# seokjuchung/point-cloud-cnn-segmentation

Measured on AMD Instinct MI355X. Metric: M voxels/sec fwd+bwd, 128^3 grid batch=4 (points/s of the PointNet training step: forward + weighted CE + backward + Adam), higher is better.
Workload: dtype bf16; 1 GPU; PointNetSegmentation train step, 4 scenes x 128^3 points per GPU, C=2; global_batch=4, parallelism=dp1

## Files before the change

### include/pcs.h

```cpp
#ifndef PCS_H
#define PCS_H

#include <stdint.h>

#ifdef __cplusplus
extern "C" {
#endif

typedef struct ihipStream_t *pcs_stream_t;

enum { PCS_F32 = 0, PCS_BF16 = 1, PCS_FP8 = 2  };
enum { PCS_OK = 0, PCS_EINVAL = -1000 };
enum {
  PCS_FLAG_GENERIC = 1,
  PCS_FLAG_NO_GLDS = 2,
  PCS_FLAG_AW_FP8 = 4,
  PCS_FLAG_C_FP8 = 8,
  PCS_FLAG_POOL_SIGNED_W = 16,
};

enum {
  PCS_PRO_RAW = 0,
  PCS_PRO_BNRELU = 1,
  PCS_PRO_BWD = 2,
// ... 181 lines not shown
             int32_t C, int32_t dtype, int32_t splits_per_scene, float *workspace, float *G,
             float *colsum, pcs_stream_t stream);

int pcs_sign_rows(const void *W, int32_t dtype, int64_t rows, int64_t cols, const float *sign_of, void *out,
                  pcs_stream_t stream);

int pcs_quant_fp8_rows(const float *W, int64_t rows, int64_t cols, int64_t ldw, uint8_t *Wq, uint8_t *scale,
                       float *deq, pcs_stream_t stream);

int pcs_pool_rows_add(void *dz, int32_t dz_dtype, const void *Yp, int32_t yp_dtype, int64_t num_scenes,
                      int64_t scene_rows, int32_t Ncols, const int32_t *pool_idx, const float *pool_coef,
                      const float *pool_w, int64_t pool_ldw, int32_t pool_c, float *stats, int32_t chunks_per_scene,
                      pcs_stream_t stream);

int64_t pcs_gram_raw_workspace(int64_t M, int32_t C);
int pcs_gram_raw(const void *A, int64_t M, int32_t C, int32_t dtype, float *workspace, int64_t workspace_bytes,
                 float *G, pcs_stream_t stream);

int pcs_gram_wgrad(const float *G, const float *S, const float *W, int64_t ldw_in,
                   const float *beta, const float *gamma, const float *sp, const int32_t *am,
                   const void *Y, const float *s, const float *t, int64_t num_scenes,
                   int32_t Cout, int32_t Cin, int32_t dtype, const float *R, const float *alpha,
                   float *dW, int64_t ldw, pcs_stream_t stream);

int pcs_bn_fold(const float *W, int32_t Cout, int32_t Cin, int64_t ldw, const float *alpha,
                const float *beta, const float *gamma, int32_t dtype, void *WsT, float *c, void *H,
                pcs_stream_t stream);

int pcs_bn_stats_from_gram(const float *G, const float *S, int64_t count, const void *W, int32_t dtype,
                           int64_t ldw, int32_t C, int32_t Cin, int64_t num_scenes, float *stats,
                           pcs_stream_t stream);

int64_t pcs_bn_stats_from_gram_scenes_workspace(int32_t C, int32_t Cin);
int pcs_bn_stats_from_gram_scenes(const float *G, const float *Sb, int64_t scene_rows, const void *W, int32_t dtype,
                                  int64_t ldw, int32_t C, int32_t Cin, int64_t num_scenes, void *workspace,
                                  int64_t workspace_bytes, float *stats, pcs_stream_t stream);

int pcs_bn_s2_from_r(float *stats, int64_t num_chunks, int32_t C, const float *R, const void *W,
                     int32_t dtype, int64_t ldw, int32_t Cin, const float *mean, const float *rstd,
                     pcs_stream_t stream);

int pcs_confusion(const float *logits, int64_t ld, const int64_t *labels, int64_t M, int32_t C,
                  int64_t *cm, pcs_stream_t stream);

int pcs_argmax(const float *logits, int64_t ld, int64_t M, int32_t C, int64_t *out, pcs_stream_t stream);

int pcs_reduce_partials(const float *partial, int64_t nslabs, int64_t len, float scale,
                        float *out, int64_t out_stride_rows, int64_t row_len,
                        pcs_stream_t stream);

int pcs_reduce_partials_grouped(const float *partial, int64_t ngroups, int64_t nslabs, int64_t len,
                                float scale, float *out, pcs_stream_t stream);

int pcs_cast_weight(const float *W, int64_t rows, int64_t cols, int64_t ldw, int32_t dtype,
                    void *Wc, void *WcT, pcs_stream_t stream);

int pcs_adam(float *param, float *grad, float *exp_avg, float *exp_avg_sq, int64_t n,
             const float *grad_scale, float lr, float beta1, float beta2, float eps,
             float weight_decay, int64_t step, pcs_stream_t stream);

int pcs_pad_scatter(const float *points, const void *labels, int32_t label_bytes,
                    const int64_t *offsets, int64_t num_scenes, int64_t scene_rows,
                    float *points_out, int64_t *labels_out, uint8_t *mask_out, pcs_stream_t stream);

int pcs_round_weight(const float *W, int64_t n, int32_t dtype, float *out, pcs_stream_t stream);

typedef struct {
  int64_t num_scenes;
  int64_t scene_rows;
  int32_t chunks_per_scene;
  const void *y2;
  const float *s2, *t2;
  const void *W1;
  const float *sbias;
  void *Y1;
  const float *s1, *t1;
  const uint8_t *keep1;
  float keep_scale;
  const void *W2;
  void *Y2;
  float *stats;
} pcs_seg12_args;
int64_t pcs_fwd_seg12_geometry(pcs_seg12_args *args);
int pcs_fwd_seg12(const pcs_seg12_args *args, pcs_stream_t stream);

int pcs_bn_stats_gram_sbias(const float *G, const float *Sb, int64_t num_scenes, int64_t scene_rows,
                            const float *W, int64_t ldw, int32_t Cin, int32_t C, const float *sbias,
                            float *stats, pcs_stream_t stream);

int pcs_bnrelu_bf16(const float *Y, int64_t M, int32_t K, const float *s, const float *t, int32_t split,
                    void *out, pcs_stream_t stream);

int pcs_voxel_ids(const float *points, int64_t T, int32_t grid, float lo_x, float lo_y, float lo_z,
                  float hi_x, float hi_y, float hi_z, int64_t *ids, pcs_stream_t stream);
int64_t pcs_voxelize_workspace(int64_t T);
int pcs_voxelize(const float *points, const int64_t *labels, const int64_t *offsets, int64_t num_scenes,
                 int64_t T, int32_t grid, float lo_x, float lo_y, float lo_z, float hi_x, float hi_y,
                 float hi_z, int32_t num_classes, void *workspace, int64_t workspace_bytes,
                 int64_t *voxel_of_point, float *vox_points, int64_t *vox_labels, int64_t *vox_counts,
                 int64_t *vox_offsets, int64_t *num_voxels, pcs_stream_t stream);
int pcs_voxel_padded_index(const int64_t *voxel_of_point, int64_t T, const int64_t *vox_offsets,
                           int64_t num_scenes, int64_t scene_rows, int64_t *out, pcs_stream_t stream);
int pcs_gather_rows(const float *src, int64_t ld_src, const int64_t *idx, int64_t n, int32_t C,
                    float *dst, pcs_stream_t stream);

typedef struct {
// ... 124 lines not shown
```

### point-cloud-cnn-segmentation_amd/_lib.py

```python
from __future__ import annotations

import ctypes as ct
import os

import torch

_HERE = os.path.dirname(os.path.abspath(__file__))
LIB_PATH = os.path.join(_HERE, "csrc", "libpcs.so")

F32, BF16, FP8 = 0, 1, 2
PRO_RAW, PRO_BNRELU, PRO_BWD, PRO_CAT = 0, 1, 2, 4
EPI_FWD, EPI_DGRAD, EPI_RAW, EPI_BNRELU = 0, 1, 2, 3
HEAD_FWD, HEAD_CE, HEAD_BWD = 0, 1, 2

_vp = ct.c_void_p
_i64 = ct.c_int64
_i32 = ct.c_int32
_f = ct.c_float


class GemmArgs(ct.Structure):
    _fields_ = [
        ("num_scenes", _i64), ("scene_rows", _i64),
        ("K", _i32), ("Ncols", _i32), ("dtype", _i32), ("prologue", _i32), ("epilogue", _i32),
# ... 22 lines not shown
        ("num_scenes", _i64), ("scene_rows", _i64),
        ("Cout", _i32), ("Cin", _i32), ("dtype", _i32), ("splits_per_scene", _i32),
        ("dy_mode", _i32),
        ("dZ", _vp), ("Y", _vp), ("alpha", _vp), ("beta", _vp), ("gamma", _vp),
        ("reserved0", _vp), ("reserved1", _vp),
        ("x_mode", _i32),
        ("X", _vp), ("s", _vp), ("t", _vp), ("x_mask", _vp), ("x_keep_scale", _f),
        ("partial", _vp), ("dW", _vp), ("ldw", _i64), ("flags", _i32), ("reserved2", _vp),
    ]


class Seg12Args(ct.Structure):
    _fields_ = [
        ("num_scenes", _i64), ("scene_rows", _i64), ("chunks_per_scene", _i32),
        ("y2", _vp), ("s2", _vp), ("t2", _vp), ("W1", _vp), ("sbias", _vp), ("Y1", _vp),
        ("s1", _vp), ("t1", _vp), ("keep1", _vp), ("keep_scale", _f), ("W2", _vp), ("Y2", _vp),
        ("stats", _vp),
    ]


class Conv3dGeom(ct.Structure):
    _fields_ = [
        ("B", _i64), ("Di", _i32), ("Hi", _i32), ("Wi", _i32), ("Do", _i32), ("Ho", _i32), ("Wo", _i32),
        ("Cin", _i32), ("Cout", _i32), ("k", _i32), ("s", _i32), ("p", _i32), ("transposed", _i32),
    ]


class PoolBwdArgs(ct.Structure):
    _fields_ = [
        ("num_scenes", _i64), ("scene_rows", _i64),
        ("Cs", _i32), ("Cg", _i32), ("col_off", _i32),
        ("s1_alpha", _vp), ("s1_beta", _vp), ("s1_gamma", _vp),
        ("s1_scene_s1", _vp), ("s1_scene_sum", _vp),
        ("W_s1", _vp), ("ldw", _i64),
        ("g", _vp), ("ysel", _vp), ("g_mean", _vp), ("g_rstd", _vp), ("g_gamma", _vp),
        ("g_scene_sum", _vp),
        ("dW_s1_global", _vp), ("csum", _vp),
        ("alpha", _vp), ("beta_c", _vp), ("gamma_c", _vp),
        ("dgamma", _vp), ("dbeta", _vp), ("dbias", _vp), ("sp", _vp),
    ]


class HeadArgs(ct.Structure):
    _fields_ = [
        ("num_scenes", _i64), ("scene_rows", _i64),
        ("Cin", _i32), ("num_classes", _i32), ("dtype", _i32), ("mode", _i32),
        ("chunks_per_scene", _i32),
        ("Y", _vp), ("s", _vp), ("t", _vp), ("W", _vp), ("bias", _vp), ("logits", _vp),
        ("labels", _vp), ("class_weight", _vp), ("wsum", _vp),
        ("dlogits", _vp), ("dl_stride_row", _i64), ("dl_stride_col", _i64),
        ("dZ", _vp), ("mean", _vp), ("rstd", _vp), ("stats", _vp), ("wpartial", _vp),
        ("loss_partial", _vp),
    ]


SIGNATURES = [
    ("pcs_gemm_geometry", _i64, [ct.POINTER(GemmArgs)]),
    ("pcs_gemm", ct.c_int, [ct.POINTER(GemmArgs), _vp]),
    ("pcs_conv1_fwd", ct.c_int, [ct.POINTER(GemmArgs), _vp]),
    ("pcs_wgrad_workspace", _i64, [ct.POINTER(WgradArgs)]),
    ("pcs_wgrad", ct.c_int, [ct.POINTER(WgradArgs), _vp]),
    ("pcs_conv1_wgrad", ct.c_int, [ct.POINTER(WgradArgs), _vp]),
    ("pcs_bn_fwd_finalize", ct.c_int, [_vp, _i64, _i64, _i32, _i32, _i64, _vp, _vp, _vp, _vp,
                                       _vp, _f, _f, _i32, _vp, _vp, _vp, _vp, _vp, _vp]),
    ("pcs_bn_eval_coefs", ct.c_int, [_vp, _vp, _vp, _vp, _vp, _f, _i32, _vp, _vp, _vp]),
    ("pcs_bn_bwd_finalize", ct.c_int, [_vp, _i64, _i64, _i32, _i32, _vp, _vp, _vp, _vp, _vp,
                                       _vp, _vp, _vp, _vp, _vp, _vp, _vp]),
    ("pcs_pool_finalize", ct.c_int, [_vp, _i64, _i64, _i32, _i32, _vp, _vp, _vp, _vp, _vp, _vp]),
    ("pcs_scene_gemv", ct.c_int, [_vp, _i64, _i32, _vp, _i64, _i32, _vp, _i32, _vp, _vp, _vp]),
    ("pcs_pool_bwd", ct.c_int, [ct.POINTER(PoolBwdArgs), _vp]),
    ("pcs_head_geometry", _i64, [ct.POINTER(HeadArgs)]),
    ("pcs_head", ct.c_int, [ct.POINTER(HeadArgs), _vp]),
    ("pcs_ce_weight_sum", ct.c_int, [_vp, _i64, _vp, _i32, _vp, _vp, _vp]),
    ("pcs_dropout_bits", ct.c_int, [ct.c_uint64, ct.c_uint64, _i64, _i32, _f, _vp, _vp]),
    ("pcs_dropout_bits_bounded", ct.c_int, [ct.c_uint64, ct.c_uint64, _i64, _i32, _f, _vp, _i32, _vp]),
    ("pcs_dropout_bits_independent", ct.c_int, [ct.c_uint64, ct.c_uint64, _i64, _i32, _f, _vp, _vp]),
    ("pcs_reduce_partials", ct.c_int, [_vp, _i64, _i64, _f, _vp, _i64, _i64, _vp]),
    ("pcs_reduce_partials_grouped", ct.c_int, [_vp, _i64, _i64, _i64, _f, _vp, _vp]),
    ("pcs_cast_weight", ct.c_int, [_vp, _i64, _i64, _i64, _i32, _vp, _vp, _vp]),
    ("pcs_adam", ct.c_int, [_vp, _vp, _vp, _vp, _i64, _vp, _f, _f, _f, _f, _f, _i64, _vp]),
    ("pcs_colstats_geometry", _i64, [_i64, _i64, _i32, ct.POINTER(_i32)]),
    ("pcs_colstats", ct.c_int, [_vp, _i64, _i64, _i32, _i32, _i32, _i64, _vp, _vp, _vp]),
    ("pcs_bnrelu_bwd", ct.c_int, [_vp, _vp, _vp, _vp, _f, _vp, _vp, _vp, _vp, _i64, _i64, _i32, _i32,
                                  _i32, _i64, _vp, _vp]),
    ("pcs_abi_version", ct.c_int, []),
    ("pcs_conv3d", ct.c_int, [ct.POINTER(Conv3dGeom), _vp, _vp, _vp, _vp, _i32, _vp]),
    ("pcs_conv3d_wgrad_workspace", _i64, [ct.POINTER(Conv3dGeom)]),
    ("pcs_conv3d_wgrad", ct.c_int, [ct.POINTER(Conv3dGeom), _vp, _vp, _vp, _i64, _vp, _vp, _vp]),
    ("pcs_conv3d_weight_t", ct.c_int, [_vp, _i32, _i32, _i32, _vp, _vp]),
    ("pcs_sparse_conv", ct.c_int, [_vp, _i64, _i32, _vp, _i32, _vp, _i32, _vp, _vp, _i32, _i32, _vp]),
    ("pcs_sparse_conv_wgrad_workspace", _i64, [_i64, _i32, _i32, _i32]),
    ("pcs_sparse_conv_wgrad", ct.c_int, [_vp, _i64, _i32, _vp, _i32, _vp, _i32, _vp, _i64, _vp, _vp, _vp]),
    ("pcs_sparse_pairs_workspace", _i64, [_i64, _i32]),
    ("pcs_sparse_pairs_count", ct.c_int, [_vp, _i64, _i32, _vp, _vp, _vp]),
    ("pcs_sparse_pairs_build", ct.c_int, [_vp, _i64, _i32, _vp, _vp, _vp, _vp, _vp, _vp]),
    ("pcs_sparse_conv_pairs", ct.c_int, [_vp, _vp, _vp, _i32, _i64, _vp, _i32, _vp, _i32, _vp, _vp, _vp, _i32, _i32,
                                         _vp]),
    ("pcs_sparse_conv_wgrad_pairs_workspace", _i64, [_vp, _i32, _i64, _i32, _i32]),
    ("pcs_sparse_conv_wgrad_pairs", ct.c_int, [_vp, _vp, _vp, _i32, _i64, _vp, _i32, _vp, _i32, _vp, _i64, _vp, _vp,
                                               _vp]),
    ("pcs_sparse_conv_cat", ct.c_int, [_vp, _i64, _i32, _vp, _i32, _vp, _i32, _vp, _i32, _vp, _vp, _i32, _i32, _vp]),
    ("pcs_sparse_conv_cat_dgrad", ct.c_int, [_vp, _i64, _i32, _vp, _i32, _vp, _vp, _i32, _vp, _i32, _i32, _i32, _vp]),
    ("pcs_sparse_conv_cat_wgrad", ct.c_int, [_vp, _i64, _i32, _vp, _i32, _vp, _i32, _vp, _i32, _vp, _i64, _vp, _vp,
                                             _vp]),
    ("pcs_sparse_conv_cat_pairs", ct.c_int, [_vp, _vp, _vp, _i32, _i64, _vp, _i32, _vp, _i32, _vp, _i32, _vp, _vp, _vp,
                                             _i32, _i32, _vp]),
# ... 13 lines not shown
                                       _vp, _vp]),
    ("pcs_rows_interp", ct.c_int, [_vp, _i32, _vp, _vp, _i64, _i32, _i32, _vp, _i32, _vp]),
    ("pcs_rows_segsum", ct.c_int, [_vp, _i32, _vp, _vp, _vp, _vp, _i64, _i32, _vp, _i32, _vp]),
    ("pcs_sparse_bn_geometry", _i64, [_i64, _i32, ct.POINTER(_i32)]),
    ("pcs_sparse_bn_stats", ct.c_int, [_vp, _i32, _i64, _i32, _i32, _i64, _vp, _vp]),
    ("pcs_sparse_bn_apply", ct.c_int, [_vp, _i32, _vp, _vp, _vp, _i32, _i64, _i32, _vp, _i32, _vp]),
    ("pcs_sparse_bn_bwd_reduce", ct.c_int, [_vp, _vp, _i32, _vp, _i32, _vp, _vp, _i32, _i64, _i32, _i32, _i64, _vp,
                                            _vp, _vp]),
    ("pcs_sparse_bn_bwd_apply", ct.c_int, [_vp, _i32, _vp, _i32, _vp, _vp, _vp, _i64, _i32, _vp, _vp]),
    ("pcs_point_lift_mean", ct.c_int, [_vp, _i64, _i32, _vp, _vp, _vp, _vp, _vp, _i64, _i32, _vp, _i32, _vp]),
    ("pcs_point_lift_bwd_workspace", _i64, [_i64, _i32, _i32]),
    ("pcs_point_lift_mean_bwd", ct.c_int, [_vp, _i32, _vp, _i64, _i32, _vp, _vp, _vp, _vp, _vp, _i64, _i32, _vp, _i64,
                                           _vp, _vp, _vp]),
    ("pcs_point_head_project", ct.c_int, [_vp, _i32, _i64, _i32, _vp, _i32, _vp, _vp]),
    ("pcs_point_head_workspace", _i64, [_i64, _i64, _i32, _i32]),
    ("pcs_point_head_logits", ct.c_int, [_vp, _vp, _vp, _i64, _i32, _vp, _vp, _vp, _vp, _vp, _vp, _vp, _i64, _vp, _vp,
                                         _vp]),
    ("pcs_point_head_bwd", ct.c_int, [_vp, _vp, _vp, _vp, _vp, _i32, _i64, _i32, _vp, _i32, _vp, _vp, _vp, _i64, _vp,
                                      _vp]),
    ("pcs_gram_workspace", _i64, [_i64, _i64, _i32, _i32, ct.POINTER(_i32)]),
    ("pcs_gram", ct.c_int, [_vp, _vp, _vp, _i64, _i64, _i32, _i32, _i32, _vp, _vp, _vp, _vp]),
    ("pcs_pool_rows_add", ct.c_int, [_vp, _i32, _vp, _i32, _i64, _i64, _i32, _vp, _vp, _vp, _i64, _i32, _vp, _i32,
                                     _vp]),
    ("pcs_quant_fp8_rows", ct.c_int, [_vp, _i64, _i64, _i64, _vp, _vp, _vp, _vp]),
    ("pcs_gram_raw_workspace", _i64, [_i64, _i32]),
    ("pcs_gram_raw", ct.c_int, [_vp, _i64, _i32, _i32, _vp, _i64, _vp, _vp]),
    ("pcs_gram_wgrad", ct.c_int, [_vp, _vp, _vp, _i64, _vp, _vp, _vp, _vp, _vp, _vp, _vp, _i64, _i32, _i32,
                                  _i32, _vp, _vp, _vp, _i64, _vp]),
    ("pcs_bn_fold", ct.c_int, [_vp, _i32, _i32, _i64, _vp, _vp, _vp, _i32, _vp, _vp, _vp, _vp]),
    ("pcs_bn_s2_from_r", ct.c_int, [_vp, _i64, _i32, _vp, _vp, _i32, _i64, _i32, _vp, _vp, _vp]),
    ("pcs_bn_stats_from_gram", ct.c_int, [_vp, _vp, _i64, _vp, _i32, _i64, _i32, _i32, _i64, _vp, _vp]),
    ("pcs_bn_stats_from_gram_scenes_workspace", _i64, [_i32, _i32]),
    ("pcs_sign_rows", ct.c_int, [_vp, _i32, _i64, _i64, _vp, _vp, _vp]),
    ("pcs_dgrad_wgrad_folded_workspace", _i64, [ct.POINTER(WgradArgs)]),
    ("pcs_dgrad_wgrad_folded", ct.c_int, [ct.POINTER(WgradArgs), _vp, _vp, _vp, _vp, _vp, _vp]),
    ("pcs_bn_stats_from_gram_scenes", ct.c_int, [_vp, _vp, _i64, _vp, _i32, _i64, _i32, _i32, _i64, _vp, _i64, _vp,
                                                 _vp]),
    ("pcs_confusion", ct.c_int, [_vp, _i64, _vp, _i64, _i32, _vp, _vp]),
    ("pcs_argmax", ct.c_int, [_vp, _i64, _i64, _i32, _vp, _vp]),
    ("pcs_dgrad_wgrad_bn_workspace", _i64, [ct.POINTER(GemmArgs)]),
    ("pcs_dgrad_wgrad_bn", ct.c_int, [ct.POINTER(GemmArgs), _vp, _vp, _i64, _vp]),
    ("pcs_round_weight", ct.c_int, [_vp, _i64, _i32, _vp, _vp]),
    ("pcs_bnrelu_bf16", ct.c_int, [_vp, _i64, _i32, _vp, _vp, _i32, _vp, _vp]),
    ("pcs_fwd_seg12_geometry", _i64, [ct.POINTER(Seg12Args)]),
    ("pcs_fwd_seg12", ct.c_int, [ct.POINTER(Seg12Args), _vp]),
    ("pcs_bn_stats_gram_sbias", ct.c_int, [_vp, _vp, _i64, _i64, _vp, _i64, _i32, _i32, _vp, _vp, _vp]),
    ("pcs_voxel_ids", ct.c_int, [_vp, _i64, _i32, _f, _f, _f, _f, _f, _f, _vp, _vp]),
    ("pcs_voxelize_workspace", _i64, [_i64]),
    ("pcs_voxelize", ct.c_int, [_vp, _vp, _vp, _i64, _i64, _i32, _f, _f, _f, _f, _f, _f, _i32, _vp, _i64,
                                _vp, _vp, _vp, _vp, _vp, _vp, _vp]),
    ("pcs_gather_rows", ct.c_int, [_vp, _i64, _vp, _i64, _i32, _vp, _vp]),
    ("pcs_voxel_padded_index", ct.c_int, [_vp, _i64, _vp, _i64, _i64, _vp, _vp]),
    ("pcs_pad_scatter", ct.c_int, [_vp, _vp, _i32, _vp, _i64, _i64, _vp, _vp, _vp, _vp]),
    ("pcs_last_error", ct.c_char_p, []),
]

_lib = None


ABI_VERSION = 3


class PcsError(RuntimeError):
    pass


def load():
    global _lib
    if _lib is not None:
        return _lib
    path = os.environ.get("PCS_LIB", LIB_PATH)
    if not os.path.exists(path):
        raise ImportError(
            f"pcs_amd HIP library not built: {path} is missing. Build it with "
            "`python -c 'import __graft_entry__ as g; g.build()'` or "
            "`make -C point-cloud-cnn-segmentation_amd/csrc`.")
    lib = ct.CDLL(path)
    for name, res, args in SIGNATURES:
        fn = getattr(lib, name)
        fn.restype = res
        fn.argtypes = args
    got = lib.pcs_abi_version()
    if got != ABI_VERSION:
        raise ImportError(f"{path} has C ABI version {got}, this binding expects {ABI_VERSION}: rebuild it "
                          "(`make -C point-cloud-cnn-segmentation_amd/csrc`)")
    _lib = lib
    return lib


def call(name, *args):
    lib = load()
    rc = getattr(lib, name)(*args)
    if rc < 0:
        raise PcsError(f"{name} failed ({rc}): {lib.pcs_last_error().decode()}")
    return rc


def workspace(name, *args) -> int:
    lib = load()
    n = int(getattr(lib, name)(*args))
    if n < 0:
        raise PcsError(lib.pcs_last_error().decode())
    return n


def ptr(t):
# ... 6 lines not shown
```

### point-cloud-cnn-segmentation_amd/csrc/fused_bwd.hip

```cpp
#include "kernel_prims.h"

namespace {

constexpr int THREADS = 512;
constexpr int COUT = 512, CIN = 64, MS = 64;
constexpr int WT_ROWB = COUT * 2;
constexpr int DY_ROWB = COUT * 2 + 32;
constexpr int X_ROWB = CIN * 2 + 32;
constexpr int OFF_DY = CIN * WT_ROWB;
constexpr int OFF_X = OFF_DY + MS * DY_ROWB;
constexpr int OFF_OUT = OFF_X + MS * X_ROWB;
constexpr int OUT_ROWB = CIN * 2 + 8;
constexpr int OFF_COEF = OFF_OUT + MS * OUT_ROWB;
constexpr int OFF_H = OFF_COEF + 3 * CIN * 4;
constexpr int H_ROWB = CIN * 2;
constexpr int LDS_BYTES = OFF_H + CIN * H_ROWB;
static_assert(LDS_BYTES <= 160 * 1024, "LDS budget");
constexpr int SLAB_F = COUT * CIN + CIN * CIN + CIN;
constexpr int DY_CPR = COUT / 8, DY_RP = THREADS / DY_CPR, DY_NCH = MS / DY_RP;
constexpr int X_CPR = CIN / 8, X_RP = THREADS / X_CPR;
static_assert(X_RP == MS, "one x chunk per thread");

PCS_DEV int wt_off(int c, int slot) { return c * WT_ROWB + ((slot ^ (c & 15)) << 4); }

// ... 145 lines not shown
    lds_barrier();
    {
      const int r = tid >> 3, ch = tid & 7;
      if (m0 + r < hi)
        st16(dX + (sbase + m0 + r) * CIN + ch * 8,
             *reinterpret_cast<const u32x4 *>(lds + OFF_OUT + r * OUT_ROWB + ch * 16));
    }
    if (st + 1 < nsteps) {
      store_step(m0 + MS);
      __builtin_amdgcn_sched_barrier(0);
      load_step(m0 + 2 * MS);
    }
    lds_barrier();
  }

  float *out = a.partial + (int64_t)L * SLAB_F;
#pragma unroll
  for (int u = 0; u < 2; ++u)
    *reinterpret_cast<float4 *>(out + COUT * CIN + ((wid >> 1) * 16 + l16) * CIN + (2 * (wid & 1) + u) * 16 + 4 * g) =
        make_float4(accg[u][0], accg[u][1], accg[u][2], accg[u][3]);
  __syncthreads();
  float *red = reinterpret_cast<float *>(lds + OFF_DY);
#pragma unroll
  for (int e = 0; e < 8; ++e) red[xr * CIN + xc * 8 + e] = xsum[e];
  __syncthreads();
  if (tid < CIN) {
    float t = 0.f;
    for (int r = 0; r < X_RP; ++r) t += red[r * CIN + tid];
    out[COUT * CIN + CIN * CIN + tid] = t;
  }
#pragma unroll
  for (int i = 0; i < 4; ++i) {
    const int o = wid * 64 + i * 16 + l16;
#pragma unroll
    for (int j = 0; j < 4; ++j)
      *reinterpret_cast<float4 *>(out + o * CIN + j * 16 + 4 * g) =
          make_float4(accw[i][j][0], accw[i][j][1], accw[i][j][2], accw[i][j][3]);
  }
}

int64_t splits_of(const pcs_wgrad_args &a) {
  int64_t sps = (256 + a.num_scenes - 1) / a.num_scenes;
  const int64_t max_sps = (a.scene_rows + 4 * MS - 1) / (4 * MS);
  if (sps > max_sps) sps = max_sps;
  return sps < 1 ? 1 : sps;
}

}

namespace {

constexpr int RG_LEN = COUT * CIN + CIN * CIN;

__global__ __launch_bounds__(256) void folded_reduce_kernel(const float *__restrict__ part, int nslab, int sps,
                                                            int B, float *__restrict__ red, float *__restrict__ Sb) {
  const int i = blockIdx.x * 256 + threadIdx.x;
  if (i < RG_LEN) {
    float t = 0.f;
    for (int sl = 0; sl < nslab; ++sl) t += part[(int64_t)sl * SLAB_F + i];
    red[i] = t;
  } else if (i < RG_LEN + B * CIN) {
    const int b = (i - RG_LEN) / CIN, j = (i - RG_LEN) % CIN;
    float t = 0.f;
    for (int sl = b * sps; sl < (b + 1) * sps; ++sl) t += part[(int64_t)sl * SLAB_F + RG_LEN + j];
    Sb[b * CIN + j] = t;
  }
}

__global__ __launch_bounds__(CIN) void folded_assemble_kernel(const float *__restrict__ red, const float *__restrict__ Sb,
                                                              int B, const float *__restrict__ W, int64_t ldw,
                                                              const float *__restrict__ alpha,
                                                              const float *__restrict__ beta,
                                                              const float *__restrict__ gamma,
                                                              const float *__restrict__ sbias, float *__restrict__ dW,
                                                              int64_t ldo) {
  __shared__ float wk[CIN];
  const int k = blockIdx.x, j = threadIdx.x;
  wk[j] = W[(int64_t)k * ldw + j];
  __syncthreads();
  const float *G = red + COUT * CIN;
  float wg = 0.f;
  for (int i = 0; i < CIN; ++i) wg = fmaf(wk[i], G[i * CIN + j], wg);
  float S = 0.f, sbs = 0.f;
  for (int b = 0; b < B; ++b) {
    const float sbj = Sb[b * CIN + j];
    S += sbj;
    sbs = fmaf(sbias[(int64_t)b * COUT + k], sbj, sbs);
  }
  dW[(int64_t)k * ldo + j] = fmaf(alpha[k], red[k * CIN + j], fmaf(beta[k], S, gamma[k] * (wg + sbs)));
}

__global__ __launch_bounds__(CIN) void folded_cvec_kernel(const float *__restrict__ W, int64_t ldw,
                                                          const float *__restrict__ beta, const float *__restrict__ gamma,
                                                          const float *__restrict__ sbias, float *__restrict__ cvec) {
  const int b = blockIdx.x, j = threadIdx.x;
  float t = 0.f;
  for (int k = 0; k < COUT; ++k)
    t = fmaf(fmaf(gamma[k], sbias[(int64_t)b * COUT + k], beta[k]), W[(int64_t)k * ldw + j], t);
  cvec[b * CIN + j] = t;
}

bool folded_shapes_ok(const pcs_wgrad_args &a) {
  return a.dtype == PCS_BF16 && a.Cout == COUT && a.Cin == CIN && a.dy_mode == PCS_PRO_RAW &&
         a.x_mode == PCS_PRO_BNRELU && !a.x_mask && !(a.flags & PCS_FLAG_GENERIC);
}

}

extern "C" int64_t pcs_dgrad_wgrad_folded_workspace(pcs_wgrad_args *a) {
  if (!a || a->num_scenes <= 0 || a->scene_rows <= 0)
    return pcs_set_einval("pcs_dgrad_wgrad_folded_workspace", "bad geometry");
  if (!folded_shapes_ok(*a))
    return pcs_set_einval("pcs_dgrad_wgrad_folded_workspace",
                          "bf16, Cout=512, Cin=64, dy_mode PRO_RAW, x_mode PRO_BNRELU, no x_mask only");
  a->splits_per_scene = (int32_t)splits_of(*a);
  const int64_t nb = a->num_scenes * a->splits_per_scene;
  return (nb * SLAB_F + RG_LEN + a->num_scenes * CIN + a->num_scenes * CIN) * 4;
}

extern "C" int pcs_dgrad_wgrad_folded(const pcs_wgrad_args *ap, const void *WaT, const void *H, const float *W,
                                      const float *scene_bias, void *dX, pcs_stream_t stream) {
  if (!ap || !WaT || !H || !W || !scene_bias || !dX) return pcs_set_einval("pcs_dgrad_wgrad_folded", "null argument");
  pcs_wgrad_args a = *ap;
  if (pcs_dgrad_wgrad_folded_workspace(&a) < 0) return PCS_EINVAL;
  if (!a.dZ || !a.alpha || !a.beta || !a.gamma || !a.X || !a.s || !a.t || !a.partial || !a.dW || a.ldw < CIN)
    return pcs_set_einval("pcs_dgrad_wgrad_folded", "missing operand (dZ, alpha, beta, gamma, X, s, t, partial, dW, "
                                                    "ldw >= 64)");
  if (a.scene_rows * a.num_scenes >= (int64_t)1 << 31) return pcs_set_einval("pcs_dgrad_wgrad_folded", "M must be < 2^31");
  const int64_t rps = ((a.scene_rows + a.splits_per_scene - 1) / a.splits_per_scene + MS - 1) / MS * MS;
  const int B = (int)a.num_scenes;
  const int nb = B * a.splits_per_scene;
  float *red = a.partial + (int64_t)nb * SLAB_F;
  float *Sb = red + RG_LEN;
  float *cvec = Sb + B * CIN;
  hipStream_t s = reinterpret_cast<hipStream_t>(stream);
  hipLaunchKernelGGL(folded_cvec_kernel, dim3(B), dim3(CIN), 0, s, W, a.ldw, a.beta, a.gamma, scene_bias, cvec);
  hipLaunchKernelGGL(dgrad_wgrad_s1_kernel, dim3(nb), dim3(THREADS), 0, s, a, static_cast<const bf16_t *>(WaT),
                     static_cast<bf16_t *>(dX), rps, static_cast<const bf16_t *>(H), cvec);
  hipLaunchKernelGGL(folded_reduce_kernel, dim3((RG_LEN + B * CIN + 255) / 256), dim3(256), 0, s, a.partial, nb,
                     a.splits_per_scene, B, red, Sb);
  hipLaunchKernelGGL(folded_assemble_kernel, dim3(COUT), dim3(CIN), 0, s, red, Sb, B, W, a.ldw, a.alpha, a.beta,
                     a.gamma, scene_bias, a.dW, a.ldw);
  PCS_CHECK_LAUNCH();
  return 0;
}

namespace {

template <int COUT, int CIN, int CB, int MS, bool MASK, bool ADD> struct FB {
  static constexpr int NBLK = CIN / CB;
  static constexpr int WT_ROWB = COUT * 2;
  static constexpr int WSW = COUT >= 128 ? 15 : 7;
  static constexpr int DY_ROWB = COUT * 2 + 32;
  static constexpr int X_ROWB = CB * 2 + 32;
  static constexpr int YP_ROWB = CB * 2 + 16;
  static constexpr int OUT_ROWB = CB * 2 + 8;
  static constexpr int OFF_DY = CB * WT_ROWB;
  static constexpr int OFF_X = OFF_DY + MS * DY_ROWB;
  static constexpr int OFF_YP = OFF_X + MS * X_ROWB;
  static constexpr int OFF_AD = OFF_YP + MS * YP_ROWB;
  static constexpr int OFF_MK = OFF_AD + (ADD ? MS * YP_ROWB : 0);
  static constexpr int OFF_OUT = OFF_MK + (MASK ? MS * CB / 8 : 0);
  static constexpr int OFF_COEF = OFF_OUT + MS * OUT_ROWB;
  static constexpr int BYTES = OFF_COEF + (3 * COUT + 2 * CB) * 4;
  static constexpr bool FITS = BYTES <= 160 * 1024;
  static_assert(CIN % CB == 0, "column blocks");
  static constexpr int NCB = CB / 16, NMB = MS / 16, NOB = COUT / 16;
  static constexpr int TPW_D = NMB * NCB / 8, TPW_W = NOB * NCB / 8;
  static constexpr int OBW = TPW_W > NCB ? TPW_W / NCB : 1;
  static_assert(TPW_D >= 1 && TPW_W >= 1 && NCB % TPW_D == 0, "dgrad wave tiling");
  static_assert(TPW_W % NCB == 0 || NCB % TPW_W == 0, "wgrad wave tiling");
  static constexpr int CBW = TPW_W / OBW;
  static constexpr int NCH_D = MS * COUT / 8 / THREADS, NCH_P = MS * CB / 8 / THREADS;
  static_assert(NCH_D >= 1 && NCH_P >= 1 && MS % 32 == 0, "staging");
};

template <int COUT, int CIN, int CB, int MS, bool MASK, bool ADD>
__global__ __launch_bounds__(THREADS) __attribute__((amdgpu_waves_per_eu(COUT == 64 ? 4 : 1, 8))) void dgrad_wgrad_bn_kernel(pcs_gemm_args a, float *__restrict__ wpart,
                                                                 int64_t rows_per_split) {
  typedef FB<COUT, CIN, CB, MS, MASK, ADD> F;
  static_assert(F::FITS, "LDS budget");
  __shared__ __attribute__((aligned(16))) char lds[F::BYTES];
  const int tid = threadIdx.x, lane = tid & 63, wid = tid >> 6;
  const int L = xcd_remap(blockIdx.x, gridDim.x);
  const int chunk = L / F::NBLK, n0 = (L % F::NBLK) * CB;
  const int sps = a.chunks_per_scene;
  const int scene = chunk / sps, sis = chunk % sps;
  const int64_t N = a.scene_rows;
  const int64_t lo = (int64_t)sis * rows_per_split;
  const int64_t hi = pcs_min64(lo + rows_per_split, N);
  const int64_t sbase = (int64_t)scene * N;
  const bf16_t *__restrict__ dZ = reinterpret_cast<const bf16_t *>(a.A);
// ... 200 lines not shown
}

template <int COUT, int CIN, int CB, int MS>
int launch_bn(const pcs_gemm_args &a, float *wpart, int64_t rps, hipStream_t s) {
  const int nb = (int)(a.num_scenes * a.chunks_per_scene) * (CIN / CB);
  if (a.c_mask && a.addend) return pcs_set_einval("pcs_dgrad_wgrad_bn", "mask and addend together");
  if (a.c_mask)
    hipLaunchKernelGGL((dgrad_wgrad_bn_kernel<COUT, CIN, CB, MS, true, false>), dim3(nb), dim3(THREADS), 0, s, a, wpart, rps);
  else if (a.addend) {
    if constexpr (FB<COUT, CIN, CB, MS, false, true>::FITS)
      hipLaunchKernelGGL((dgrad_wgrad_bn_kernel<COUT, CIN, CB, MS, false, true>), dim3(nb), dim3(THREADS), 0, s, a, wpart,
                         rps);
    else
      return pcs_set_einval("pcs_dgrad_wgrad_bn", "no addend variant at this shape (LDS)");
  } else
    hipLaunchKernelGGL((dgrad_wgrad_bn_kernel<COUT, CIN, CB, MS, false, false>), dim3(nb), dim3(THREADS), 0, s, a,
                       wpart, rps);
  PCS_CHECK_LAUNCH();
  return 0;
}

struct BnShape { int cout, cin, cb, ms; };
constexpr BnShape kBnShapes[] = {{64, 64, 64, 64}, {128, 64, 64, 64}};

const BnShape *bn_shape(int K, int Ncols) {
  for (const BnShape &b : kBnShapes)
    if (b.cout == K && b.cin == Ncols) return &b;
  return nullptr;
}

}

extern "C" int64_t pcs_dgrad_wgrad_bn_workspace(pcs_gemm_args *a) {
  if (!a || a->num_scenes <= 0 || a->scene_rows <= 0) return pcs_set_einval("pcs_dgrad_wgrad_bn_workspace", "bad geometry");
  if (pcs_seg4_applicable(*a)) {
    pcs_seg4_geometry(a);
    return (int64_t)a->num_scenes * a->chunks_per_scene * a->K * a->Ncols * 4;
  }
  const BnShape *sh = bn_shape(a->K, a->Ncols);
  if (a->dtype != PCS_BF16 || !sh || (a->flags & PCS_FLAG_GENERIC))
    return pcs_set_einval("pcs_dgrad_wgrad_bn_workspace",
                          "bf16 with (Cout, Cin) = K x Ncols in {64x64, 128x64} only");
  const int nblk = sh->cin / sh->cb;
  const int64_t target = sh->cout == 64 ? 512 : 256;
  int64_t sps = (target + a->num_scenes * nblk - 1) / (a->num_scenes * nblk);
  const int64_t max_sps = (a->scene_rows + 4 * sh->ms - 1) / (4 * sh->ms);
  if (sps > max_sps) sps = max_sps;
  if (sps < 1) sps = 1;
  const int64_t rps = ((a->scene_rows + sps - 1) / sps + sh->ms - 1) / sh->ms * sh->ms;
  a->chunks_per_scene = (int32_t)((a->scene_rows + rps - 1) / rps);
  return (int64_t)a->num_scenes * a->chunks_per_scene * a->K * a->Ncols * 4;
}

extern "C" int pcs_dgrad_wgrad_bn(const pcs_gemm_args *ap, float *partial, float *dW, int64_t ldw,
                                  pcs_stream_t stream) {
  if (!ap || !partial || !dW) return pcs_set_einval("pcs_dgrad_wgrad_bn", "null argument");
  pcs_gemm_args a = *ap;
  if (pcs_dgrad_wgrad_bn_workspace(&a) < 0) return PCS_EINVAL;
  if (a.chunks_per_scene != ap->chunks_per_scene)
    return pcs_set_einval("pcs_dgrad_wgrad_bn", "chunks_per_scene must come from pcs_dgrad_wgrad_bn_workspace");
  if (!a.A || !a.A2 || !a.pa || !a.pb || !a.pc || !a.W || !a.C || !a.Yp || !a.es || !a.et || !a.emean ||
      !a.erstd || !a.stats)
    return pcs_set_einval("pcs_dgrad_wgrad_bn", "missing operand (A, A2, pa, pb, pc, W, C, Yp, es, et, emean, "
                                                "erstd, stats)");
  if (a.scene_rows * a.num_scenes >= (int64_t)1 << 31) return pcs_set_einval("pcs_dgrad_wgrad_bn", "M must be < 2^31");
  if (pcs_seg4_applicable(a)) {
    const int rc = pcs_seg4_launch(a, partial, reinterpret_cast<hipStream_t>(stream));
    if (rc) return rc;
    const int nslab = (int)(a.num_scenes * a.chunks_per_scene);
    return pcs_reduce_partials(partial, nslab, (int64_t)a.K * a.Ncols, 1.0f, dW, ldw ? ldw : a.Ncols, a.Ncols, stream);
  }
  const BnShape *sh = bn_shape(a.K, a.Ncols);
  const int64_t rps = ((a.scene_rows + a.chunks_per_scene - 1) / a.chunks_per_scene + sh->ms - 1) / sh->ms * sh->ms;
  hipStream_t s = reinterpret_cast<hipStream_t>(stream);
  int rc;
  if (a.K == 64) rc = launch_bn<64, 64, 64, 64>(a, partial, rps, s);
  else rc = launch_bn<128, 64, 64, 64>(a, partial, rps, s);
  if (rc) return rc;
  const int nslab = (int)(a.num_scenes * a.chunks_per_scene);
  return pcs_reduce_partials(partial, nslab, (int64_t)a.K * a.Ncols, 1.0f, dW, ldw ? ldw : a.Ncols, a.Ncols, stream);
}
```

### point-cloud-cnn-segmentation_amd/csrc/gemm_glds.hip

```cpp
#include "kernel_prims.h"

#include <type_traits>

namespace {

constexpr int THREADS = 512;
constexpr int BM = 256, BN = 256, BK = 64;
constexpr int REG = 128 * BK * 2;
constexpr int KBUF = 4 * REG;
constexpr int STAGE_BYTES = 2 * KBUF;
constexpr int OFF_RUN = STAGE_BYTES;
constexpr int OFF_BIAS = OFF_RUN + 2 * 256 * 8;
constexpr int OFF_RUNN = OFF_BIAS + 256 * 4;
constexpr int OFF_UNI = OFF_RUNN + 16;
constexpr int OFF_POOL = OFF_UNI;
constexpr int OFF_SGN = OFF_UNI + 2 * 256 * 16;
constexpr int OFF_CUR = OFF_SGN + 256 * 4;
constexpr int OFF_MASK = OFF_UNI;
constexpr int LDS_BYTES = OFF_UNI + 2 * 256 * 8 * 4;
static_assert(LDS_BYTES <= 160 * 1024, "LDS budget");

enum { MODE_FWD = 0, MODE_DGRAD = 1 };


// ... 540 lines not shown
      } else {
        *reinterpret_cast<float2 *>(a.stats + o * 2) = make_float2(h0.x + h1.x, 0.f);
      }
    }
    if (do_pool) {
      float4 p = runp[tid];
      const float4 q = runp[BN + tid];
      const int pi = __float_as_int(p.y), qi = __float_as_int(q.y);
      const int pj = __float_as_int(p.w), qj = __float_as_int(q.w);
      if (pool_max_wins(q.x, qi, p.x, pi)) { p.x = q.x; p.y = q.y; }
      if (pool_min_wins(q.z, qj, p.z, pj)) { p.z = q.z; p.w = q.w; }
      *reinterpret_cast<float4 *>(a.pool + o * 4) = p;
    }
  }
}

}

bool pcs_gemm_glds_applicable(const pcs_gemm_args &a) {
  if (a.dtype != PCS_BF16 || (a.flags & (PCS_FLAG_GENERIC | PCS_FLAG_NO_GLDS))) return false;
  const bool fp8 = a.flags & PCS_FLAG_AW_FP8;
  if (fp8 && !a.w_scale) return false;
  if (a.prologue != PCS_PRO_RAW || a.K % (fp8 ? 256 : 2 * BK) != 0 || a.Ncols % BN != 0) return false;
  if (a.epilogue == PCS_EPI_FWD)
    return a.C == nullptr && a.scene_bias == nullptr && (!a.pool || a.es) &&
           (!(a.flags & PCS_FLAG_POOL_SIGNED_W) || (a.pool && !a.stats));
  if (a.epilogue == PCS_EPI_DGRAD)
    return a.Yp == a.A && a.K == a.Ncols && !a.es && !a.et && !a.erstd && !a.addend && !a.c_mask &&
           !a.pool_w;
  return false;
}

int pcs_gemm_glds_launch(const pcs_gemm_args &g, int tps, int tpc, hipStream_t s) {
  const int ncb = g.Ncols / BN;
  const int nb = ncb * (int)(g.num_scenes * g.chunks_per_scene);
  const bool fp8 = g.flags & PCS_FLAG_AW_FP8;
#define PCS_GL(M, F) hipLaunchKernelGGL((gemm_glds_kernel<M, F>), dim3(nb), dim3(THREADS), 0, s, g, tps, tpc, ncb)
  if (g.epilogue == PCS_EPI_FWD) {
    if (fp8) PCS_GL(MODE_FWD, true); else PCS_GL(MODE_FWD, false);
  } else {
    if (fp8) PCS_GL(MODE_DGRAD, true); else PCS_GL(MODE_DGRAD, false);
  }
#undef PCS_GL
  PCS_CHECK_LAUNCH();
  return 0;
}

namespace {

constexpr int PR_MAXC = 1024;
constexpr int PR_PARTS = 16;

template <typename T, typename TY>
__global__ __launch_bounds__(256) void pool_rows_add_kernel(T *__restrict__ dz, const TY *__restrict__ Yp, int64_t N,
                                                            int Ncols, const int32_t *__restrict__ idx,
                                                            const float *__restrict__ coef, const float *__restrict__ Wp,
                                                            int64_t ldw, int P, float *__restrict__ stats, int cps) {
  __shared__ unsigned long long keys[PR_MAXC];
  const int b = blockIdx.y, part = blockIdx.z, parts = gridDim.z, tid = threadIdx.x;
  const int n = blockIdx.x * 256 + tid;
  int Pp = 1;
  while (Pp < P) Pp <<= 1;
  for (int c = tid; c < Pp; c += 256)
    keys[c] = c < P ? ((unsigned long long)(uint32_t)idx[(int64_t)b * P + c] << 11) | (unsigned)c : ~0ull;
  __syncthreads();
  for (int k = 2; k <= Pp; k <<= 1) {
    for (int j = k >> 1; j > 0; j >>= 1) {
      for (int i = tid; i < Pp; i += 256) {
        const int ixj = i ^ j;
        if (ixj > i) {
          const unsigned long long x = keys[i], y = keys[ixj];
          if ((x > y) == ((i & k) == 0)) { keys[i] = y; keys[ixj] = x; }
        }
      }
      __syncthreads();
    }
  }
  auto srow_at = [&](int q) { return (int)(keys[q] >> 11); };
  auto sch_at = [&](int q) { return (int)(keys[q] & 2047u); };
  auto cut = [&](int j) {
    int p = (int)((int64_t)j * P / parts);
    while (p > 0 && p < P && srow_at(p) == srow_at(p - 1)) ++p;
    return p;
  };
  const int p0 = cut(part), p1 = cut(part + 1);
  if (n >= Ncols || p0 >= p1) return;
  float ds1 = 0.f, v = 0.f;
  constexpr int U = 8;
  for (int p = p0; p < p1; p += U) {
    float cf[U], wv[U];
#pragma unroll
    for (int u = 0; u < U; ++u) {
      cf[u] = 0.f;
      wv[u] = 0.f;
      if (p + u < p1) {
        const int c = sch_at(p + u);
        cf[u] = coef[(int64_t)b * P + c];
        wv[u] = Wp[(int64_t)c * ldw + n];
      }
    }
#pragma unroll
    for (int u = 0; u < U; ++u) {
      const int q = p + u;
      if (q >= p1) break;
      v = fmaf(cf[u], wv[u], v);
      if (q + 1 == p1 || srow_at(q + 1) != srow_at(q)) {
        const int64_t m = (int64_t)srow_at(q);
        const int64_t o = m * Ncols + n;
        if (m >= (int64_t)b * N && m < (int64_t)(b + 1) * N && load_elem(Yp, o) > 0.f) {
          const float d = load_elem(dz, o) + v;
          if constexpr (sizeof(T) == 2) dz[o] = (T)(pack2bf(d, 0.f) & 0xffffu);
          else dz[o] = d;
          ds1 += v;
        }
        v = 0.f;
      }
    }
  }
  if (stats) stats[(((int64_t)b * cps + part) * Ncols + n) * 2] += ds1;
}

}

extern "C" int pcs_pool_rows_add(void *dz, int32_t dz_dtype, const void *Yp, int32_t yp_dtype, int64_t num_scenes,
                                 int64_t scene_rows, int32_t Ncols, const int32_t *pool_idx, const float *pool_coef,
                                 const float *pool_w, int64_t pool_ldw, int32_t pool_c, float *stats,
                                 int32_t chunks_per_scene, pcs_stream_t stream) {
  if (!dz || !Yp || !pool_idx || !pool_coef || !pool_w || num_scenes <= 0 || scene_rows <= 0 || Ncols <= 0 ||
      pool_c <= 0 || pool_c > PR_MAXC || pool_ldw < Ncols || (stats && chunks_per_scene <= 0))
    return pcs_set_einval("pcs_pool_rows_add", "bad arguments (0 < pool_c <= 1024, pool_ldw >= Ncols)");
  hipStream_t s = reinterpret_cast<hipStream_t>(stream);
  const int parts = stats ? (chunks_per_scene < PR_PARTS ? chunks_per_scene : PR_PARTS) : PR_PARTS;
  const dim3 grid((Ncols + 255) / 256, (unsigned)num_scenes, (unsigned)parts);
#define PCS_PRA(T, TY)                                                                                          \
  hipLaunchKernelGGL((pool_rows_add_kernel<T, TY>), grid, dim3(256), 0, s, static_cast<T *>(dz),                 \
                     static_cast<const TY *>(Yp), scene_rows, (int)Ncols, pool_idx, pool_coef, pool_w, pool_ldw, \
                     (int)pool_c, stats, (int)chunks_per_scene)
  if (dz_dtype == PCS_BF16 && yp_dtype == PCS_BF16) PCS_PRA(bf16_t, bf16_t);
  else if (dz_dtype == PCS_BF16 && yp_dtype == PCS_FP8) PCS_PRA(bf16_t, fp8_t);
  else if (dz_dtype == PCS_F32 && yp_dtype == PCS_F32) PCS_PRA(float, float);
  else return pcs_set_einval("pcs_pool_rows_add", "dtypes: (bf16, bf16), (bf16, fp8) or (f32, f32)");
#undef PCS_PRA
  PCS_CHECK_LAUNCH();
  return 0;
}

namespace {
__global__ __launch_bounds__(256) void quant_fp8_rows_kernel(const float *__restrict__ W, int64_t cols, int64_t ldw,
                                                             fp8_t *__restrict__ Wq, uint8_t *__restrict__ scale,
                                                             float *__restrict__ deq) {
  __shared__ float red[4];
  const int64_t r = blockIdx.x;
  const float *w = W + r * ldw;
  float mx = 0.f;
  for (int64_t k = threadIdx.x; k < cols; k += 256) mx = fmaxf(mx, fabsf(w[k]));
  for (int o = 32; o > 0; o >>= 1) mx = fmaxf(mx, __shfl_xor(mx, o));
  if ((threadIdx.x & 63) == 0) red[threadIdx.x >> 6] = mx;
  __syncthreads();
  mx = fmaxf(fmaxf(red[0], red[1]), fmaxf(red[2], red[3]));
  int e = 0;
  if (mx > 0.f) {
    e = (int)ceilf(log2f(mx / 448.f));
    e = e < -126 ? -126 : (e > 127 ? 127 : e);
  }
  if (threadIdx.x == 0) scale[r] = (uint8_t)(127 + e);
  const float inv = ldexpf(1.f, -e);
  for (int64_t k = threadIdx.x * 4; k < cols; k += 1024) {
    float v[4];
#pragma unroll
    for (int q = 0; q < 4; ++q) v[q] = k + q < cols ? w[k + q] * inv : 0.f;
    const uint32_t b = pack4fp8(v[0], v[1], v[2], v[3]);
    for (int q = 0; q < 4 && k + q < cols; ++q) {
      Wq[r * cols + k + q] = (fp8_t)(b >> (8 * q));
      if (deq) deq[r * cols + k + q] = ldexpf(fp82f((b >> (8 * q)) & 255u), e);
    }
  }
}
}

extern "C" int pcs_quant_fp8_rows(const float *W, int64_t rows, int64_t cols, int64_t ldw, uint8_t *Wq, uint8_t *scale,
                                  float *deq, pcs_stream_t stream) {
  if (!W || !Wq || !scale || rows <= 0 || cols <= 0 || ldw < cols) return pcs_set_einval("pcs_quant_fp8_rows", "bad arguments");
  hipLaunchKernelGGL(quant_fp8_rows_kernel, dim3((unsigned)rows), dim3(256), 0, reinterpret_cast<hipStream_t>(stream), W,
                     cols, ldw, Wq, scale, deq);
  PCS_CHECK_LAUNCH();
  return 0;
}

// ... 33 lines not shown
```

### point-cloud-cnn-segmentation_amd/csrc/gemm_tn.hip

```cpp
#include "kernel_prims.h"

namespace {

constexpr int THREADS = 256;

template <typename T> struct TnCfg;
template <> struct TnCfg<bf16_t> {
  static constexpr int MS = 64;
  static constexpr int PADB = 32;
  static PCS_DEV int prow(int r) { return ::prow(r); }
};
template <> struct TnCfg<float> {
  static constexpr int MS = 16;
  static constexpr int PADB = 64;
  static PCS_DEV int prow(int r) { return r; }
};

template <typename T, int COLS, int MODE>
struct Operand {
  static constexpr int EPC = Elem<T>::EPC;
  static constexpr int MS = TnCfg<T>::MS;
  static constexpr int CPR = COLS / EPC;
  static constexpr int RP = THREADS / CPR;
  static constexpr int NCH = MS / RP;
// ... 232 lines not shown

template <typename T, int TM, int TN>
int dispatch_modes(const pcs_wgrad_args &a, int64_t rps, hipStream_t s) {
  if (a.dy_mode == PCS_PRO_BWD) {
    if (a.x_mode == PCS_PRO_BNRELU) return launch<T, TM, TN, PCS_PRO_BWD, PCS_PRO_BNRELU>(a, rps, s);
    if (a.x_mode == PCS_PRO_RAW) return launch<T, TM, TN, PCS_PRO_BWD, PCS_PRO_RAW>(a, rps, s);
  } else if (a.dy_mode == PCS_PRO_RAW) {
    if (a.x_mode == PCS_PRO_BNRELU) return launch<T, TM, TN, PCS_PRO_RAW, PCS_PRO_BNRELU>(a, rps, s);
  } else if (a.dy_mode == PCS_PRO_BNRELU && a.x_mode == PCS_PRO_BNRELU && !a.x_mask) {
    return launch<T, TM, TN, PCS_PRO_BNRELU, PCS_PRO_BNRELU>(a, rps, s);
  }
  return pcs_set_einval("pcs_wgrad", "unsupported dy_mode/x_mode");
}

template <typename T>
int dispatch_tiles(const pcs_wgrad_args &a, int64_t rps, hipStream_t s) {
  const bool m128 = a.Cout % 128 == 0, n128 = a.Cin % 128 == 0;
  if (m128 && n128) return dispatch_modes<T, 128, 128>(a, rps, s);
  if (m128) return dispatch_modes<T, 128, 64>(a, rps, s);
  if (n128) return dispatch_modes<T, 64, 128>(a, rps, s);
  return dispatch_modes<T, 64, 64>(a, rps, s);
}

int64_t rows_per_split_of(const pcs_wgrad_args &a, int ms) {
  const int64_t rps = (a.scene_rows + a.splits_per_scene - 1) / a.splits_per_scene;
  return (rps + ms - 1) / ms * ms;
}

bool reserved_set(const pcs_wgrad_args &a) { return a.reserved0 || a.reserved1 || a.reserved2; }

}

extern "C" int64_t pcs_wgrad_workspace(pcs_wgrad_args *a) {
  if (!a || a->num_scenes <= 0 || a->scene_rows <= 0 || a->Cout <= 0 || a->Cin <= 0)
    return pcs_set_einval("pcs_wgrad_workspace", "bad geometry");
  if (reserved_set(*a)) return pcs_set_einval("pcs_wgrad_workspace", "reserved0..2 must be NULL (removed in ABI 3)");
  const int ms = a->dtype == PCS_BF16 ? TnCfg<bf16_t>::MS : TnCfg<float>::MS;
  if (a->splits_per_scene <= 0 && pcs_wgrad_c5_class(*a)) a->splits_per_scene = pcs_wgrad_c5_splits(*a);
  if (a->splits_per_scene <= 0 && pcs_wgrad_big_applicable(*a)) a->splits_per_scene = pcs_wgrad_big_splits(*a);
  if (a->splits_per_scene <= 0) {
    const int tm = a->Cout % 128 == 0 ? 128 : 64, tn = a->Cin % 128 == 0 ? 128 : 64;
    const int64_t ntiles = a->Cin >= 64 ? (int64_t)(a->Cout / tm) * (a->Cin / tn) : 1;
    const int64_t target = 1024;
    int64_t sps = (target + a->num_scenes * ntiles - 1) / (a->num_scenes * ntiles);
    const int64_t max_sps = (a->scene_rows + 4 * ms - 1) / (4 * ms);
    if (sps > max_sps) sps = max_sps;
    if (sps < 1) sps = 1;
    a->splits_per_scene = (int32_t)sps;
  }
  const int64_t nslabs = (int64_t)a->num_scenes * a->splits_per_scene;
  return nslabs * a->Cout * a->Cin * 4;
}

extern "C" int pcs_wgrad(const pcs_wgrad_args *ap, pcs_stream_t stream) {
  if (!ap) return pcs_set_einval("pcs_wgrad", "null args");
  pcs_wgrad_args a = *ap;
  if (reserved_set(a)) return pcs_set_einval("pcs_wgrad", "reserved0..2 must be NULL (removed in ABI 3)");
  if (a.dy_mode != PCS_PRO_RAW && a.dy_mode != PCS_PRO_BNRELU && a.dy_mode != PCS_PRO_BWD)
    return pcs_set_einval("pcs_wgrad", "unknown dy_mode (PCS_PRO_RAW, PCS_PRO_BNRELU or PCS_PRO_BWD)");
  if (a.Cout % 64 || a.Cin % 64) return pcs_set_einval("pcs_wgrad", "Cout/Cin must be multiples of 64");
  if (!a.X || !a.partial || !a.dW) return pcs_set_einval("pcs_wgrad", "missing operand");
  if (a.dy_mode == PCS_PRO_RAW ? !a.dZ : (!a.Y || !a.beta || !a.gamma))
    return pcs_set_einval("pcs_wgrad", "dy operands missing (RAW: dZ; otherwise: Y, beta, gamma)");
  if (a.dy_mode == PCS_PRO_BWD && (!a.dZ || !a.alpha)) return pcs_set_einval("pcs_wgrad", "PRO_BWD needs dZ, alpha");
  if (a.x_mode == PCS_PRO_BNRELU && (!a.s || !a.t)) return pcs_set_einval("pcs_wgrad", "x BNRELU needs s, t");
  if (pcs_wgrad_workspace(&a) < 0) return PCS_EINVAL;
  const int ms = a.dtype == PCS_BF16 ? TnCfg<bf16_t>::MS : TnCfg<float>::MS;
  const int64_t rps = rows_per_split_of(a, ms);
  hipStream_t s = reinterpret_cast<hipStream_t>(stream);
  int rc;
  if (pcs_wgrad_c5_applicable(a)) rc = pcs_wgrad_c5_launch(a, rps, s);
  else if (pcs_wgrad_big_applicable(a)) rc = pcs_wgrad_big_launch(a, s);
  else if (a.dtype == PCS_BF16) rc = dispatch_tiles<bf16_t>(a, rps, s);
  else if (a.dtype == PCS_F32) rc = dispatch_tiles<float>(a, rps, s);
  else return pcs_set_einval("pcs_wgrad", "bad dtype");
  if (rc) return rc;
  const int64_t nslabs = a.num_scenes * a.splits_per_scene;
  return pcs_reduce_partials(a.partial, nslabs, (int64_t)a.Cout * a.Cin, 1.0f, a.dW,
                             a.ldw ? a.ldw : a.Cin, a.Cin, stream);
}

namespace {

pcs_wgrad_args gram_args(const void *Y, const float *s, const float *t, int64_t num_scenes,
                         int64_t scene_rows, int32_t C, int32_t dtype, int32_t sps) {
  pcs_wgrad_args a = {};
  a.num_scenes = num_scenes; a.scene_rows = scene_rows; a.Cout = C; a.Cin = C; a.dtype = dtype;
  a.splits_per_scene = sps; a.dy_mode = PCS_PRO_BNRELU; a.x_mode = PCS_PRO_BNRELU;
  a.Y = Y; a.X = Y; a.s = s; a.t = t; a.x_keep_scale = 1.f;
  return a;
}

__global__ __launch_bounds__(256) void gram_mirror_kernel(float *__restrict__ G, int C) {
  __shared__ float tile[64][65];
  const int nt = C / 64;
  int t = blockIdx.x, tj = 0;
  while (t >= nt - 1 - tj) { t -= nt - 1 - tj; ++tj; }
  const int tk = tj + 1 + t;
  const int tx = threadIdx.x & 63, ty = threadIdx.x >> 6;
  for (int r = ty; r < 64; r += 4) tile[r][tx] = G[(int64_t)(tj * 64 + r) * C + tk * 64 + tx];
  __syncthreads();
  for (int r = ty; r < 64; r += 4) G[(int64_t)(tk * 64 + r) * C + tj * 64 + tx] = tile[tx][r];
}

}

extern "C" int64_t pcs_gram_workspace(int64_t num_scenes, int64_t scene_rows, int32_t C, int32_t dtype,
                                      int32_t *splits_per_scene) {
  if (num_scenes <= 0 || scene_rows <= 0 || C <= 0 || C % 64 || !splits_per_scene)
    return pcs_set_einval("pcs_gram_workspace", "bad geometry");
  pcs_wgrad_args a = gram_args(nullptr, nullptr, nullptr, num_scenes, scene_rows, C, dtype, 0);
  if (pcs_gram128_class(a)) a.splits_per_scene = pcs_gram128_splits(a);
  const int64_t g = pcs_wgrad_workspace(&a);
  if (g < 0) return g;
  *splits_per_scene = a.splits_per_scene;
  return g + num_scenes * a.splits_per_scene * (int64_t)C * 4;
}

extern "C" int pcs_gram(const void *Y, const float *s, const float *t, int64_t num_scenes, int64_t scene_rows,
                        int32_t C, int32_t dtype, int32_t splits_per_scene, float *workspace, float *G,
                        float *colsum, pcs_stream_t stream) {
  if (!Y || !s != !t || !workspace || !G || !colsum || splits_per_scene <= 0)
    return pcs_set_einval("pcs_gram", "missing operand or splits (s and t both set, or both NULL)");
  if (C % 64) return pcs_set_einval("pcs_gram", "C must be a multiple of 64");
  pcs_wgrad_args a = gram_args(Y, s, t, num_scenes, scene_rows, C, dtype, splits_per_scene);
  a.partial = workspace;
  hipStream_t st = reinterpret_cast<hipStream_t>(stream);
  int rc;
  if (!s && !pcs_wgrad_big_applicable(a))
    return pcs_set_einval("pcs_gram", "s = t = NULL needs the 256x256 kernel (bf16, C % 256 == 0)");
  if (pcs_gram128_applicable(a)) {
    rc = pcs_gram128_launch(a, st);
  } else if (pcs_wgrad_big_applicable(a)) {
// ... 21 lines not shown
```

### point-cloud-cnn-segmentation_amd/csrc/gram.hip

```cpp
#include "common.h"

namespace {

constexpr int TILE = 64, KC = 32, THREADS = 256;

template <typename T, int TL>
__global__ __launch_bounds__(THREADS) void gram_wgrad_kernel(
    const float *__restrict__ G, const float *__restrict__ S, const float *__restrict__ W, int64_t ldwin,
    const float *__restrict__ beta, const float *__restrict__ gamma, const float *__restrict__ sp,
    const int *__restrict__ am, const T *__restrict__ Y, const float *__restrict__ s,
    const float *__restrict__ t, int B, int Cout, int Cin, const float *__restrict__ R,
    const float *__restrict__ alpha, float *__restrict__ dW, int64_t ldw) {
  constexpr int RR = TL / 16, NE = TL * KC / THREADS;
  __shared__ float Ws[TL][KC + 1];
  __shared__ float Gs[KC][TL];
  const int tid = threadIdx.x, tx = tid & 15, ty = tid >> 4;
  const int c0 = blockIdx.y * TL, k0 = blockIdx.x * TL;
  float acc[RR][RR] = {};
  float pw[NE], pg[NE];
  auto load = [&](int j0) {
#pragma unroll
    for (int u = 0; u < NE; ++u) {
      const int e = tid + THREADS * u;
      pw[u] = W[(int64_t)(c0 + e / KC) * ldwin + j0 + e % KC];
// ... 151 lines not shown
      for (int p = 0; p < R; ++p)
#pragma unroll
        for (int q = 0; q < R; ++q) acc[p][q] = fmaf(xa[p], ya[q], acc[p][q]);
    }
    __syncthreads();
  }
#pragma unroll
  for (int p = 0; p < R; ++p)
#pragma unroll
    for (int q = 0; q < R; ++q) {
      const int64_t o = (int64_t)(i0 + ty * R + p) * Cin + j0 + tx * R + q;
      if constexpr (sizeof(T) == 2) H[o] = (T)(pack2bf(acc[p][q], 0.f) & 0xffffu);
      else H[o] = acc[p][q];
    }
}

template <typename T>
__global__ __launch_bounds__(256) void bn_stats_gram_kernel(const float *__restrict__ G, const float *__restrict__ S,
                                                            double n, const T *__restrict__ W, int64_t ldw, int C,
                                                            int Cin, int B, float *__restrict__ stats) {
  __shared__ double w[1024];
  __shared__ double sh[256][2];
  const int c = blockIdx.x, tid = threadIdx.x;
  double dm = 0.0;
  for (int k = tid; k < Cin; k += 256) {
    w[k] = (double)load_elem(W, (int64_t)c * ldw + k);
    dm += w[k] * (double)S[k];
  }
  __syncthreads();
  double q = 0.0;
  for (int j = tid; j < Cin; j += 256) {
    const double sj = (double)S[j] / n;
    double row = 0.0;
    for (int k = 0; k < Cin; ++k) row += ((double)G[(int64_t)j * Cin + k] - sj * (double)S[k]) * w[k];
    q += w[j] * row;
  }
  sh[tid][0] = dm; sh[tid][1] = q;
  __syncthreads();
  for (int st = 128; st > 0; st >>= 1) {
    if (tid < st) { sh[tid][0] += sh[tid + st][0]; sh[tid][1] += sh[tid + st][1]; }
    __syncthreads();
  }
  if (tid < B) {
    const double mean = sh[0][0] / n, m2 = sh[0][1] < 0.0 ? 0.0 : sh[0][1];
    *reinterpret_cast<float2 *>(stats + ((int64_t)tid * C + c) * 2) = make_float2((float)mean, (float)(m2 / B));
  }
}

constexpr int QK_SPLIT = 4;

template <typename T>
__global__ __launch_bounds__(256) void gram_quad_kernel(const float *__restrict__ G, const T *__restrict__ W,
                                                        int64_t ldw, int Cin, double *__restrict__ part) {
  __shared__ double gs[16][64];
  __shared__ double wt[16][65];
  __shared__ double red[16][64];
  const int C = gridDim.x * 64, c0 = blockIdx.x * 64, j0 = blockIdx.y * 64;
  const int tid = threadIdx.x, tx = tid & 15, ty = tid >> 4;
  double acc[4][4];
#pragma unroll
  for (int p = 0; p < 4; ++p)
#pragma unroll
    for (int q = 0; q < 4; ++q) acc[p][q] = 0.0;
  const int kz0 = (int)((int64_t)Cin / 16 * blockIdx.z / QK_SPLIT) * 16;
  const int kz1 = (int)((int64_t)Cin / 16 * (blockIdx.z + 1) / QK_SPLIT) * 16;
  for (int k0 = kz0; k0 < kz1; k0 += 16) {
#pragma unroll
    for (int e = tid; e < 1024; e += 256) {
      gs[e >> 6][e & 63] = (double)G[(int64_t)(k0 + (e >> 6)) * Cin + j0 + (e & 63)];
      wt[e & 15][e >> 4] = (double)load_elem(W, (int64_t)(c0 + (e >> 4)) * ldw + k0 + (e & 15));
    }
    __syncthreads();
#pragma unroll 4
    for (int kk = 0; kk < 16; ++kk) {
      double a[4], b[4];
#pragma unroll
      for (int p = 0; p < 4; ++p) { a[p] = gs[kk][ty * 4 + p]; b[p] = wt[kk][tx * 4 + p]; }
#pragma unroll
      for (int p = 0; p < 4; ++p)
#pragma unroll
        for (int q = 0; q < 4; ++q) acc[p][q] = fma(a[p], b[q], acc[p][q]);
    }
    __syncthreads();
  }
#pragma unroll
  for (int q = 0; q < 4; ++q) {
    const int64_t wr = (int64_t)(c0 + tx * 4 + q) * ldw + j0 + ty * 4;
    double s = 0.0;
#pragma unroll
    for (int p = 0; p < 4; ++p) s = fma((double)load_elem(W, wr + p), acc[p][q], s);
    red[ty][tx * 4 + q] = s;
  }
  __syncthreads();
  if (tid < 64) {
    double s = 0.0;
    for (int r = 0; r < 16; ++r) s += red[r][tid];
    part[((int64_t)blockIdx.z * gridDim.y + blockIdx.y) * C + c0 + tid] = s;
  }
}

template <typename T>
__global__ __launch_bounds__(256) void bn_stats_scenes_kernel(const double *__restrict__ part, int njt,
                                                              const float *__restrict__ Sb, double nb,
                                                              const T *__restrict__ W, int64_t ldw, int C, int Cin,
                                                              int B, float *__restrict__ stats) {
  __shared__ double sh[256];
  __shared__ double d[64];
  const int c = blockIdx.x, tid = threadIdx.x;
  for (int b = 0; b < B; ++b) {
    double x = 0.0;
    for (int k = tid; k < Cin; k += 256)
      x = fma((double)load_elem(W, (int64_t)c * ldw + k), (double)Sb[(int64_t)b * Cin + k], x);
    sh[tid] = x;
    __syncthreads();
    for (int st = 128; st > 0; st >>= 1) {
      if (tid < st) sh[tid] += sh[tid + st];
      __syncthreads();
    }
    if (tid == 0) d[b] = sh[0];
    __syncthreads();
  }
  double qp = 0.0;
  for (int jt = tid; jt < njt; jt += 256) qp += part[(int64_t)jt * C + c];
  sh[tid] = qp;
  __syncthreads();
  for (int st = 128; st > 0; st >>= 1) {
    if (tid < st) sh[tid] += sh[tid + st];
    __syncthreads();
  }
  if (tid == 0) {
// ... 167 lines not shown
```

### point-cloud-cnn-segmentation_amd/csrc/small.hip

```cpp
#include "common.h"

namespace {

constexpr int THREADS = 256;
constexpr int C1_BM = 128;

template <int KD>
PCS_DEV void load_xrow(const float *X, int64_t row, float (&x)[KD]) {
  if constexpr (KD == 4) {
    const float4 v = *reinterpret_cast<const float4 *>(X + row * 4);
    x[0] = v.x; x[1] = v.y; x[2] = v.z; x[3] = v.w;
  } else {
#pragma unroll
    for (int k = 0; k < KD; ++k) x[k] = X[row * KD + k];
  }
}

template <typename T, int KD>
__global__ __launch_bounds__(THREADS) void conv1_fwd_kernel(pcs_gemm_args a, int tiles_per_scene,
                                                            int tiles_per_chunk) {
  constexpr int EPC = Elem<T>::EPC;
  constexpr int COLS = 64;
  constexpr int CPR = COLS / EPC;
  constexpr int RPP = THREADS / CPR;
// ... 73 lines not shown
  const int tid = threadIdx.x;
  const int sps = a.splits_per_scene;
  const int scene = blockIdx.x / sps, sis = blockIdx.x % sps;
  const int64_t N = a.scene_rows;
  const int cc = tid % CPR, r0 = tid / CPR, c0 = cc * EPC;
  const T *dZ = reinterpret_cast<const T *>(a.dZ);
  const T *Y = reinterpret_cast<const T *>(a.Y);
  const float *X = reinterpret_cast<const float *>(a.X);
  float ca[EPC], cb[EPC], cg[EPC];
  load_vec<EPC>(a.alpha, c0, ca); load_vec<EPC>(a.beta, c0, cb); load_vec<EPC>(a.gamma, c0, cg);
  float acc[EPC][KD];
#pragma unroll
  for (int e = 0; e < EPC; ++e)
#pragma unroll
    for (int k = 0; k < KD; ++k) acc[e][k] = 0.f;
  const int64_t lo = (int64_t)sis * rows_per_split, hi = pcs_min64(lo + rows_per_split, N);
  constexpr int U = 4;
  for (int64_t r = lo + r0; r < hi; r += U * RPP) {
    u32x4 dzr[U], yr[U];
    float x[U][KD];
#pragma unroll
    for (int u = 0; u < U; ++u) {
      const int64_t grow = scene * N + pcs_min64(r + u * RPP, hi - 1);
      dzr[u] = *reinterpret_cast<const u32x4 *>(dZ + grow * COLS + c0);
      yr[u] = *reinterpret_cast<const u32x4 *>(Y + grow * COLS + c0);
      load_xrow<KD>(X, grow, x[u]);
    }
#pragma unroll
    for (int u = 0; u < U; ++u) {
      if (r + u * RPP >= hi) break;
      float dz[EPC], y[EPC];
      unpack_chunk(dzr[u], dz);
      unpack_chunk(yr[u], y);
#pragma unroll
      for (int e = 0; e < EPC; ++e) {
        const float dy = fmaf(ca[e], dz[e], fmaf(cg[e], y[e], cb[e]));
#pragma unroll
        for (int k = 0; k < KD; ++k) acc[e][k] = fmaf(dy, x[u][k], acc[e][k]);
      }
    }
  }
#pragma unroll
  for (int e = 0; e < EPC; ++e)
#pragma unroll
    for (int k = 0; k < KD; ++k) red[r0][(c0 + e) * KD + k] = acc[e][k];
  __syncthreads();
  for (int i = tid; i < COLS * KD; i += THREADS) {
    float s = 0.f;
    for (int j = 0; j < RPP; ++j) s += red[j][i];
    a.partial[(int64_t)blockIdx.x * COLS * KD + i] = s;
  }
}

__global__ __launch_bounds__(THREADS) void bn_fwd_finalize_kernel(
    const float *stats, int64_t B, int64_t N, int C, int cps, int64_t rpc, const float *gamma,
    const float *beta, const float *moff, float *rmean, float *rvar, float momentum, float eps, int update,
    float *mean_o, float *rstd_o, float *scale_o, float *shift_o, float *scene_sum) {
  __shared__ double sh[THREADS][3];
  const int c = blockIdx.x, tid = threadIdx.x;
  double gn = 0, gmean = 0, gm2 = 0;
  for (int64_t b = 0; b < B; ++b) {
    double n = 0, mu = 0, q = 0;
    for (int j = tid; j < cps; j += THREADS) {
      const double nb = (double)pcs_min64(rpc, N - (int64_t)j * rpc);
      const float2 p = *reinterpret_cast<const float2 *>(stats + ((b * cps + j) * C + c) * 2);
      const double nn = n + nb, d = (double)p.x - mu;
      mu += d * nb / nn;
      q += (double)p.y + d * d * n * nb / nn;
      n = nn;
    }
    sh[tid][0] = n; sh[tid][1] = mu; sh[tid][2] = q;
    __syncthreads();
    for (int s = THREADS / 2; s > 0; s >>= 1) {
      if (tid < s) {
        const double na = sh[tid][0], nb = sh[tid + s][0];
        if (nb > 0) {
          const double nn = na + nb, d = sh[tid + s][1] - sh[tid][1];
          sh[tid][1] += d * nb / nn;
          sh[tid][2] += sh[tid + s][2] + d * d * na * nb / nn;
          sh[tid][0] = nn;
        }
      }
      __syncthreads();
    }
    if (tid == 0) {
      const double nb = sh[0][0], mb = sh[0][1], qb = sh[0][2];
      if (scene_sum) scene_sum[b * C + c] = (float)(nb * mb);
      const double nn = gn + nb, d = mb - gmean;
      gmean += d * nb / nn;
      gm2 += qb + d * d * gn * nb / nn;
      gn = nn;
    }
    __syncthreads();
  }
  if (tid == 0) {
    const double var = gm2 / gn;
    const double rstd = 1.0 / sqrt(var + (double)eps);
    const double sc = (double)gamma[c] * rstd;
    mean_o[c] = (float)gmean;
    rstd_o[c] = (float)rstd;
    scale_o[c] = (float)sc;
    shift_o[c] = (float)((double)beta[c] - gmean * sc);
    if (update) {
      const double unb = gn > 1 ? gm2 / (gn - 1) : gm2;
      const double tm = gmean + (moff ? (double)moff[c] : 0.0);
      rmean[c] = (float)((1.0 - momentum) * (double)rmean[c] + momentum * tm);
      rvar[c] = (float)((1.0 - momentum) * (double)rvar[c] + momentum * unb);
    }
  }
}

__global__ void bn_eval_kernel(const float *gamma, const float *beta, const float *rm,
                               const float *rv, const float *moff, float eps, int C, float *scale,
                               float *shift) {
  const int c = blockIdx.x * blockDim.x + threadIdx.x;
  if (c >= C) return;
  const double sc = (double)gamma[c] / sqrt((double)rv[c] + (double)eps);
  scale[c] = (float)sc;
  shift[c] = (float)((double)beta[c] - ((double)rm[c] - (moff ? (double)moff[c] : 0.0)) * sc);
}

__global__ __launch_bounds__(THREADS) void bn_bwd_finalize_kernel(
    const float *stats, int64_t B, int64_t N, int C, int cps, const float *mean, const float *rstd,
    const float *gamma, const float *scene_sum, float *alpha, float *beta_c, float *gamma_c,
    float *dgamma, float *dbeta, float *dbias, float *scene_s1) {
  __shared__ double sh[THREADS][2];
  const int c = blockIdx.x, tid = threadIdx.x;
  double S1 = 0, S2 = 0, Sy = 0;
  for (int64_t b = 0; b < B; ++b) {
    double s1 = 0, s2 = 0;
    for (int j = tid; j < cps; j += THREADS) {
      const float2 p = *reinterpret_cast<const float2 *>(stats + ((b * cps + j) * C + c) * 2);
      s1 += p.x; s2 += p.y;
    }
    sh[tid][0] = s1; sh[tid][1] = s2;
    __syncthreads();
    for (int s = THREADS / 2; s > 0; s >>= 1) {
      if (tid < s) { sh[tid][0] += sh[tid + s][0]; sh[tid][1] += sh[tid + s][1]; }
      __syncthreads();
    }
    if (tid == 0) {
      if (scene_s1) scene_s1[b * C + c] = (float)sh[0][0];
      S1 += sh[0][0]; S2 += sh[0][1];
      if (scene_sum) Sy += scene_sum[b * C + c];
    }
    __syncthreads();
  }
  if (tid == 0) {
    const double M = (double)(B * N);
    const double r = rstd[c], g = gamma[c], mu = mean[c];
    const double al = g * r;
    const double ga = -g * r * r * S2 / M;
    const double be = -g * r * S1 / M - ga * mu;
    alpha[c] = (float)al; gamma_c[c] = (float)ga; beta_c[c] = (float)be;
    if (dgamma) dgamma[c] = (float)S2;
    if (dbeta) dbeta[c] = (float)S1;
    if (dbias) dbias[c] = scene_sum ? (float)(al * S1 + M * be + ga * Sy) : 0.f;
  }
}

__global__ void pool_finalize_kernel(const float *pool, int64_t B, int64_t N, int C, int cps,
                                     const float *s, const float *t, float *g, int32_t *am,
                                     float *ysel) {
  const int64_t i = (int64_t)blockIdx.x * blockDim.x + threadIdx.x;
  if (i >= B * C) return;
  const int b = (int)(i / C), c = (int)(i % C);
  float mx = -__builtin_huge_valf(), mn = __builtin_huge_valf();
  int mxi = 0x7fffffff, mni = 0x7fffffff;
  for (int j = 0; j < cps; ++j) {
    const float4 q = *reinterpret_cast<const float4 *>(pool + (((int64_t)b * cps + j) * C + c) * 4);
    const int qi = __float_as_int(q.y), qj = __float_as_int(q.w);
    if (pool_max_wins(q.x, qi, mx, mxi)) { mx = q.x; mxi = qi; }
    if (pool_min_wins(q.z, qj, mn, mni)) { mn = q.z; mni = qj; }
  }
  const float sc = s[c];
  float y; int idx;
  if (sc > 0.f) { y = mx; idx = mxi; }
  else if (sc < 0.f) { y = mn; idx = mni; }
  else { y = mx; idx = (int)(b * N); }
  if ((int64_t)idx < b * N || (int64_t)idx >= (b + 1) * N) idx = (int)(b * N);
  const float z = fmaf(y, sc, t[c]);
  g[i] = (z > 0.f || z != z) ? z : 0.f;
  am[i] = idx;
  ysel[i] = y;
}

__global__ void scene_gemv_kernel(const float *g, int64_t B, int Kg, const float *W, int64_t ldw,
                                  int col_off, const float *bias, int Nout, float *out,
                                  float *offset) {
  const int n = (int)(((int64_t)blockIdx.x * blockDim.x + threadIdx.x) >> 6);
  const int lane = threadIdx.x & 63;
  if (n >= Nout) return;
  const float *w = W + (int64_t)n * ldw + col_off;
  const float bn = bias ? bias[n] : 0.f;
  double mean = 0.0;
  for (int64_t b = 0; b < B; ++b) {
    const float *x = g + b * Kg;
    float acc = 0.f;
    for (int k = lane; k < Kg; k += 64) acc = fmaf(w[k], x[k], acc);
    acc = wave_sum(acc) + bn;
    mean += acc;
    if (lane == 0) out[b * Nout + n] = acc;
  }
  if (!offset) return;
  const float m = (float)(mean / (double)B);
  if (lane == 0) {
    for (int64_t b = 0; b < B; ++b) out[b * Nout + n] -= m;
    offset[n] = m;
  }
}

__global__ void pool_bwd_csum_kernel(pcs_pool_bwd_args a) {
  const int64_t i = (int64_t)blockIdx.x * blockDim.x + threadIdx.x;
  if (i >= a.num_scenes * a.Cs) return;
  const int n = (int)(i % a.Cs);
  a.csum[i] = a.s1_alpha[n] * a.s1_scene_s1[i] + (float)a.scene_rows * a.s1_beta[n] +
              a.s1_gamma[n] * a.s1_scene_sum[i];
}

__global__ void pool_bwd_dw_kernel(pcs_pool_bwd_args a) {
  const int64_t i = (int64_t)blockIdx.x * blockDim.x + threadIdx.x;
  if (i >= (int64_t)a.Cs * a.Cg) return;
  const int n = (int)(i / a.Cg), k = (int)(i % a.Cg);
  float acc = 0.f;
  for (int64_t b = 0; b < a.num_scenes; ++b) acc = fmaf(a.csum[b * a.Cs + n], a.g[b * a.Cg + k], acc);
  a.dW_s1_global[(int64_t)n * a.ldw + a.col_off + k] = acc;
}

constexpr int PBC_MAXB = 64;
constexpr int PBC_PARTS = 16, PBC_SB = 8;
__global__ __launch_bounds__(1024) void pool_bwd_coef_kernel(pcs_pool_bwd_args a) {
  __shared__ float part[PBC_PARTS][PBC_SB][64];
  __shared__ float dgall[PBC_MAXB][64];
  const int kk = threadIdx.x & 63, pr = threadIdx.x >> 6;
  const int k = blockIdx.x * 64 + kk;
  const int B = (int)a.num_scenes;
  const int n0 = (int)((int64_t)a.Cs * pr / PBC_PARTS), n1 = (int)((int64_t)a.Cs * (pr + 1) / PBC_PARTS);
  for (int b0 = 0; b0 < B; b0 += PBC_SB) {
    float dg[PBC_SB];
#pragma unroll
    for (int u = 0; u < PBC_SB; ++u) dg[u] = 0.f;
    if (k < a.Cg) {
      for (int n = n0; n < n1; ++n) {
        const float w = a.W_s1[(int64_t)n * a.ldw + a.col_off + k];
#pragma unroll
        for (int u = 0; u < PBC_SB; ++u)
          if (b0 + u < B) dg[u] = fmaf(w, a.csum[(int64_t)(b0 + u) * a.Cs + n], dg[u]);
      }
    }
#pragma unroll
    for (int u = 0; u < PBC_SB; ++u) part[pr][u][kk] = dg[u];
    __syncthreads();
    if (pr == 0) {
      for (int u = 0; u < PBC_SB && b0 + u < B; ++u) {
        float t = 0.f;
        for (int q = 0; q < PBC_PARTS; ++q) t += part[q][u][kk];
        dgall[b0 + u][kk] = t;
      }
    }
    __syncthreads();
  }
  if (pr != 0 || k >= a.Cg) return;
  const double M = (double)(a.num_scenes * a.scene_rows);
  const double r = a.g_rstd[k], gm = a.g_gamma[k], mu = a.g_mean[k];
  double S1 = 0, S2 = 0, Sy = 0;
  for (int b = 0; b < B; ++b) {
    const float dg = dgall[b][kk];
    const float dz = a.g[(int64_t)b * a.Cg + k] > 0.f ? dg : 0.f;
    a.sp[(int64_t)b * a.Cg + k] = dz;
    S1 += dz;
    S2 += (double)dz * ((double)a.ysel[(int64_t)b * a.Cg + k] - mu) * r;
    Sy += a.g_scene_sum[(int64_t)b * a.Cg + k];
  }
  const double al = gm * r;
  const double ga = -gm * r * r * S2 / M;
  const double be = -gm * r * S1 / M - ga * mu;
  for (int b = 0; b < B; ++b) a.sp[(int64_t)b * a.Cg + k] = (float)(al * a.sp[(int64_t)b * a.Cg + k]);
  a.alpha[k] = (float)al; a.beta_c[k] = (float)be; a.gamma_c[k] = (float)ga;
  a.dgamma[k] = (float)S2; a.dbeta[k] = (float)S1;
  a.dbias[k] = (float)(al * S1 + M * be + ga * Sy);
}

constexpr int HEAD_R = 64;
constexpr int HEAD_CIN = 128;
constexpr int HEAD_MAXC = 64;
constexpr int HEAD_LD = HEAD_CIN + 1;

template <typename T, int MODE, int HEAD_MAXC>
__global__ __launch_bounds__(THREADS) void head_kernel(pcs_head_args a, int tiles_per_scene,
                                                       int tiles_per_chunk) {
  constexpr int EPC = Elem<T>::EPC;
  constexpr int QCH = 32;
  __shared__ float av[HEAD_R * HEAD_LD];
  __shared__ float xh[HEAD_R * HEAD_LD];
  __shared__ float wl[HEAD_MAXC * HEAD_CIN];
// ... 579 lines not shown
  for (int64_t j0 = ((int64_t)blockIdx.x * blockDim.x + threadIdx.x) * 4; j0 < nbytes; j0 += stride) {
  uint32_t word = 0;
#pragma unroll
  for (int q = 0; q < 2; ++q) {
    const int64_t k = (j0 >> 1) + q;
    uint32_t ctr[4] = {(uint32_t)k, (uint32_t)((uint64_t)k >> 32), (uint32_t)offset, (uint32_t)(offset >> 32)};
    philox(ctr, (uint32_t)seed, (uint32_t)(seed >> 32));
#pragma unroll
    for (int i = 0; i < 4; ++i) {
      const uint32_t x = ctr[i];
      const uint32_t sw = __builtin_amdgcn_perm(0u, x, 0x02030001u);
      word |= drop2(sw, thr2, one2) << (8 * q + 2 * i);
      word |= drop2(x, thr2, one2) << (8 * q + 2 * i + 1);
    }
  }
  word = ~word;
  if (j0 + 4 <= nbytes && ((reinterpret_cast<uintptr_t>(bits) & 3) == 0)) {
    *reinterpret_cast<uint32_t *>(bits + j0) = word;
  } else {
    for (int q = 0; q < 4 && j0 + q < nbytes; ++q) bits[j0 + q] = (uint8_t)(word >> (8 * q));
  }
  }
}

__global__ void dropout_bits_indep_kernel(uint64_t seed, uint64_t offset, int64_t nbytes, uint32_t thr,
                                          uint8_t *bits) {
  const uint32_t thr2 = thr | (thr << 16);
  u16x2 one2 = {1, 1};
  asm volatile("" : "+v"(one2));
  const int64_t stride = (int64_t)gridDim.x * blockDim.x * 4;
  for (int64_t j0 = ((int64_t)blockIdx.x * blockDim.x + threadIdx.x) * 4; j0 < nbytes; j0 += stride) {
    uint32_t word = 0;
#pragma unroll
    for (int q = 0; q < 4; ++q) {
      const int64_t k = j0 + q;
      uint32_t ctr[4] = {(uint32_t)k, (uint32_t)((uint64_t)k >> 32), (uint32_t)offset, (uint32_t)(offset >> 32)};
      philox(ctr, (uint32_t)seed, (uint32_t)(seed >> 32));
#pragma unroll
      for (int i = 0; i < 4; ++i) {
        const uint32_t d = drop2(ctr[i], thr2, one2);
        word |= ((d & 1u) | ((d >> 15) & 2u)) << (8 * q + 2 * i);
      }
    }
    word = ~word;
    if (j0 + 4 <= nbytes && ((reinterpret_cast<uintptr_t>(bits) & 3) == 0)) {
      *reinterpret_cast<uint32_t *>(bits + j0) = word;
    } else {
      for (int q = 0; q < 4 && j0 + q < nbytes; ++q) bits[j0 + q] = (uint8_t)(word >> (8 * q));
    }
  }
}

template <int TPO>
__global__ void reduce_partials_kernel(const float *partial, int64_t nslabs, int64_t len, float scale,
                                       float *out, int64_t ldo, int64_t row_len) {
  partial += (int64_t)blockIdx.y * nslabs * len;
  out += (int64_t)blockIdx.y * len;
  const int sub = threadIdx.x % TPO;
  const int64_t i4 = ((int64_t)blockIdx.x * (blockDim.x / TPO) + threadIdx.x / TPO) * 4;
  const bool vec = (row_len & 3) == 0 && i4 + 4 <= len;
  float v[4] = {0.f, 0.f, 0.f, 0.f};
  if (i4 < len) {
    if (vec) {
      for (int64_t k = sub; k < nslabs; k += TPO) {
        const float4 p = *reinterpret_cast<const float4 *>(partial + k * len + i4);
        v[0] += p.x; v[1] += p.y; v[2] += p.z; v[3] += p.w;
      }
    } else {
      for (int64_t k = sub; k < nslabs; k += TPO)
        for (int e = 0; e < 4 && i4 + e < len; ++e) v[e] += partial[k * len + i4 + e];
    }
  }
#pragma unroll
  for (int off = TPO / 2; off > 0; off >>= 1)
#pragma unroll
    for (int e = 0; e < 4; ++e) v[e] += __shfl_xor(v[e], off);
  if (sub != 0 || i4 >= len) return;
  if (vec) {
    const int64_t row = i4 / row_len, col = i4 % row_len;
    *reinterpret_cast<float4 *>(out + row * ldo + col) =
        make_float4(v[0] * scale, v[1] * scale, v[2] * scale, v[3] * scale);
  } else {
    for (int e = 0; e < 4 && i4 + e < len; ++e) {
      const int64_t i = i4 + e;
      out[(i / row_len) * ldo + i % row_len] = v[e] * scale;
    }
  }
}

template <typename T>
__global__ void cast_weight_kernel(const float *W, int64_t rows, int64_t cols, int64_t ldw, T *Wc, T *WcT) {
  const int64_t i = (int64_t)blockIdx.x * blockDim.x + threadIdx.x;
  if (i >= rows * cols) return;
  const float v = W[(i / cols) * ldw + i % cols];
  T o;
  if constexpr (sizeof(T) == 4) o = v;
  else o = (T)(pack2bf(v, 0.f) & 0xffffu);
  if (Wc) Wc[i] = o;
  if (WcT) WcT[(i % cols) * rows + i / cols] = o;
}

__global__ void adam_kernel(float *p, float *g, float *m, float *v, int64_t n,
                            const float *gscale, float lr, float b1, float b2, float eps, float wd,
                            float bc1, float bc2_sqrt) {
  const int64_t i = (int64_t)blockIdx.x * blockDim.x + threadIdx.x;
  if (i >= n) return;
  const float pi = p[i];
  float gr = g[i];
  if (gscale) {
    gr *= *gscale;
    g[i] = gr;
  }
  const float gi = gr + wd * pi;
  const float mi = b1 * m[i] + (1.f - b1) * gi;
  const float vi = b2 * v[i] + (1.f - b2) * gi * gi;
  m[i] = mi;
  v[i] = vi;
  const float denom = sqrtf(vi) / bc2_sqrt + eps;
  p[i] = pi - (lr / bc1) * (mi / denom);
}

int blocks_for(int64_t n, int per) { return (int)((n + per - 1) / per); }

}

static int64_t chunk_geo(int64_t N, int64_t B, int64_t tile, int32_t *cps_io, int64_t target) {
  const int64_t tps = (N + tile - 1) / tile;
  int64_t cps = *cps_io;
  if (cps <= 0) cps = (target + B - 1) / B;
  if (cps > tps) cps = tps;
  if (cps < 1) cps = 1;
  const int64_t tpc = (tps + cps - 1) / cps;
  cps = (tps + tpc - 1) / tpc;
  *cps_io = (int32_t)cps;
  return tpc;
}

namespace {
constexpr int C1_MAXK = 8;
#define PCS_C1_SWITCH(KD_, CALL)                                 \
  switch (KD_) {                                                 \
    case 1: CALL(1); break; case 2: CALL(2); break;              \
    case 3: CALL(3); break; case 4: CALL(4); break;              \
    case 5: CALL(5); break; case 6: CALL(6); break;              \
    case 7: CALL(7); break; default: CALL(8); break;             \
  }
}

extern "C" int pcs_conv1_fwd(const pcs_gemm_args *ap, pcs_stream_t stream) {
  if (!ap || !ap->A || !ap->W || !ap->C) return pcs_set_einval("pcs_conv1_fwd", "missing operand");
  if (ap->K < 1 || ap->K > C1_MAXK || ap->Ncols != 64) return pcs_set_einval("pcs_conv1_fwd", "conv1 is input_dim (1..8) -> 64");
  pcs_gemm_args a = *ap;
  const int64_t tpc = pcs_fill_geometry(&a, C1_BM, 2048, 1) / C1_BM;
  const int tps = (int)((a.scene_rows + C1_BM - 1) / C1_BM);
  const int nb = (int)(a.num_scenes * a.chunks_per_scene);
  hipStream_t s = reinterpret_cast<hipStream_t>(stream);
#define PCS_C1F_BF(KD) hipLaunchKernelGGL((conv1_fwd_kernel<bf16_t, KD>), dim3(nb), dim3(THREADS), 0, s, a, tps, (int)tpc)
#define PCS_C1F_F32(KD) hipLaunchKernelGGL((conv1_fwd_kernel<float, KD>), dim3(nb), dim3(THREADS), 0, s, a, tps, (int)tpc)
  if (a.dtype == PCS_BF16) { PCS_C1_SWITCH(a.K, PCS_C1F_BF) }
  else if (a.dtype == PCS_F32) { PCS_C1_SWITCH(a.K, PCS_C1F_F32) }
  else return pcs_set_einval("pcs_conv1_fwd", "bad dtype");
#undef PCS_C1F_BF
#undef PCS_C1F_F32
  PCS_CHECK_LAUNCH();
  return 0;
}

extern "C" int pcs_conv1_wgrad(const pcs_wgrad_args *ap, pcs_stream_t stream) {
  if (!ap || !ap->dZ || !ap->Y || !ap->X || !ap->partial || !ap->dW)
    return pcs_set_einval("pcs_conv1_wgrad", "missing operand");
  if (ap->Cout != 64 || ap->Cin < 1 || ap->Cin > C1_MAXK)
    return pcs_set_einval("pcs_conv1_wgrad", "conv1 is input_dim (1..8) -> 64");
  pcs_wgrad_args a = *ap;
  if (a.splits_per_scene <= 0) {
    int64_t sps = (1024 + a.num_scenes - 1) / a.num_scenes;
    const int64_t maxs = (a.scene_rows + 255) / 256;
    if (sps > maxs) sps = maxs;
    if (sps < 1) sps = 1;
    a.splits_per_scene = (int32_t)sps;
  }
  const int64_t rps = (a.scene_rows + a.splits_per_scene - 1) / a.splits_per_scene;
  const int nb = (int)(a.num_scenes * a.splits_per_scene);
  hipStream_t s = reinterpret_cast<hipStream_t>(stream);
#define PCS_C1W_BF(KD) hipLaunchKernelGGL((conv1_wgrad_kernel<bf16_t, KD>), dim3(nb), dim3(THREADS), 0, s, a, rps)
#define PCS_C1W_F32(KD) hipLaunchKernelGGL((conv1_wgrad_kernel<float, KD>), dim3(nb), dim3(THREADS), 0, s, a, rps)
  if (a.dtype == PCS_BF16) { PCS_C1_SWITCH(a.Cin, PCS_C1W_BF) }
  else if (a.dtype == PCS_F32) { PCS_C1_SWITCH(a.Cin, PCS_C1W_F32) }
  else return pcs_set_einval("pcs_conv1_wgrad", "bad dtype");
#undef PCS_C1W_BF
#undef PCS_C1W_F32
  PCS_CHECK_LAUNCH();
  return pcs_reduce_partials(a.partial, nb, 64 * a.Cin, 1.f, a.dW, a.ldw ? a.ldw : a.Cin, a.Cin, stream);
}
#undef PCS_C1_SWITCH

extern "C" int pcs_bn_fwd_finalize(const float *stats, int64_t B, int64_t N, int32_t C, int32_t cps,
                                   int64_t rpc, const float *gamma, const float *beta,
                                   const float *mean_offset, float *running_mean,
                                   float *running_var, float momentum,
                                   float eps, int32_t update_running, float *mean, float *rstd,
                                   float *scale, float *shift, float *scene_sum,
                                   pcs_stream_t stream) {
  if (!stats || !gamma || !beta || !mean || !rstd || !scale || !shift || C <= 0 || cps <= 0 || rpc <= 0)
    return pcs_set_einval("pcs_bn_fwd_finalize", "bad arguments");
  if (update_running && (!running_mean || !running_var))
    return pcs_set_einval("pcs_bn_fwd_finalize", "running buffers required");
  hipLaunchKernelGGL(bn_fwd_finalize_kernel, dim3(C), dim3(THREADS), 0, reinterpret_cast<hipStream_t>(stream),
                     stats, B, N, (int)C, (int)cps, rpc, gamma, beta, mean_offset, running_mean, running_var,
                     momentum, eps, (int)update_running, mean, rstd, scale, shift, scene_sum);
  PCS_CHECK_LAUNCH();
  return 0;
}

extern "C" int pcs_bn_eval_coefs(const float *gamma, const float *beta, const float *rm,
                                 const float *rv, const float *mean_offset, float eps, int32_t C,
                                 float *scale, float *shift, pcs_stream_t stream) {
  if (!gamma || !beta || !rm || !rv || !scale || !shift) return pcs_set_einval("pcs_bn_eval_coefs", "null");
  hipLaunchKernelGGL(bn_eval_kernel, dim3(blocks_for(C, 256)), dim3(256), 0,
                     reinterpret_cast<hipStream_t>(stream), gamma, beta, rm, rv, mean_offset, eps, (int)C, scale, shift);
  PCS_CHECK_LAUNCH();
  return 0;
}

extern "C" int pcs_bn_bwd_finalize(const float *stats, int64_t B, int64_t N, int32_t C, int32_t cps,
                                   const float *mean, const float *rstd, const float *gamma,
                                   const float *scene_sum, float *alpha, float *beta_c,
                                   float *gamma_c, float *dgamma, float *dbeta, float *dbias,
                                   float *scene_s1, pcs_stream_t stream) {
  if (!stats || !mean || !rstd || !gamma || !alpha || !beta_c || !gamma_c)
    return pcs_set_einval("pcs_bn_bwd_finalize", "null argument");
  hipLaunchKernelGGL(bn_bwd_finalize_kernel, dim3(C), dim3(THREADS), 0, reinterpret_cast<hipStream_t>(stream),
                     stats, B, N, (int)C, (int)cps, mean, rstd, gamma, scene_sum, alpha, beta_c,
                     gamma_c, dgamma, dbeta, dbias, scene_s1);
  PCS_CHECK_LAUNCH();
  return 0;
}

extern "C" int pcs_pool_finalize(const float *pool, int64_t B, int64_t N, int32_t C, int32_t cps,
                                 const float *s, const float *t, float *g, int32_t *am, float *ysel,
                                 pcs_stream_t stream) {
  if (!pool || !s || !t || !g || !am || !ysel) return pcs_set_einval("pcs_pool_finalize", "null argument");
  hipLaunchKernelGGL(pool_finalize_kernel, dim3(blocks_for(B * C, 256)), dim3(256), 0,
                     reinterpret_cast<hipStream_t>(stream), pool, B, N, (int)C, (int)cps, s, t, g, am, ysel);
  PCS_CHECK_LAUNCH();
  return 0;
}

// ... 158 lines not shown
  if (thr > 65535u) {
    const hipError_t e = hipMemsetAsync(bits, 0, (size_t)nbytes, reinterpret_cast<hipStream_t>(stream));
    return e == hipSuccess ? 0 : pcs_set_error(e, "pcs_dropout_bits_independent");
  }
  hipLaunchKernelGGL(dropout_bits_indep_kernel, dim3((unsigned)blocks_for((nbytes + 3) / 4, 256)), dim3(256), 0,
                     reinterpret_cast<hipStream_t>(stream), seed, offset, nbytes, thr, bits);
  PCS_CHECK_LAUNCH();
  return 0;
}

namespace {
int reduce_partials_launch(const float *partial, int64_t ngroups, int64_t nslabs, int64_t len, float scale,
                           float *out, int64_t ldo, int64_t row_len, hipStream_t st) {
  const int64_t n4 = (len + 3) / 4;
  const dim3 g256(blocks_for(n4, 256 / 32), (unsigned)ngroups), g8(blocks_for(n4, 256 / 8), (unsigned)ngroups),
      g1(blocks_for(n4, 256), (unsigned)ngroups);
  if (nslabs >= 64)
    hipLaunchKernelGGL(reduce_partials_kernel<32>, g256, dim3(256), 0, st, partial, nslabs, len, scale, out, ldo,
                       row_len);
  else if (nslabs >= 8)
    hipLaunchKernelGGL(reduce_partials_kernel<8>, g8, dim3(256), 0, st, partial, nslabs, len, scale, out, ldo, row_len);
  else
    hipLaunchKernelGGL(reduce_partials_kernel<1>, g1, dim3(256), 0, st, partial, nslabs, len, scale, out, ldo, row_len);
  PCS_CHECK_LAUNCH();
  return 0;
}
}

extern "C" int pcs_reduce_partials_grouped(const float *partial, int64_t ngroups, int64_t nslabs, int64_t len,
                                           float scale, float *out, pcs_stream_t stream) {
  if (!partial || !out || len <= 0 || nslabs <= 0 || ngroups <= 0 || ngroups > 65535)
    return pcs_set_einval("pcs_reduce_partials_grouped", "bad arguments (0 < ngroups <= 65535)");
  return reduce_partials_launch(partial, ngroups, nslabs, len, scale, out, len, len, reinterpret_cast<hipStream_t>(stream));
}

extern "C" int pcs_reduce_partials(const float *partial, int64_t nslabs, int64_t len, float scale, float *out,
                                   int64_t ldo, int64_t row_len, pcs_stream_t stream) {
  if (!partial || !out || len <= 0 || nslabs <= 0 || row_len <= 0) return pcs_set_einval("pcs_reduce_partials", "bad arguments");
  hipStream_t st = reinterpret_cast<hipStream_t>(stream);
  const int64_t n4 = (len + 3) / 4;
  if (nslabs >= 64)
    hipLaunchKernelGGL(reduce_partials_kernel<32>, dim3(blocks_for(n4, 256 / 32)), dim3(256), 0, st, partial, nslabs,
                       len, scale, out, ldo, row_len);
  else if (nslabs >= 8)
    hipLaunchKernelGGL(reduce_partials_kernel<8>, dim3(blocks_for(n4, 256 / 8)), dim3(256), 0, st, partial, nslabs,
                       len, scale, out, ldo, row_len);
  else
    hipLaunchKernelGGL(reduce_partials_kernel<1>, dim3(blocks_for(n4, 256)), dim3(256), 0, st, partial, nslabs, len,
                       scale, out, ldo, row_len);
  PCS_CHECK_LAUNCH();
  return 0;
}

extern "C" int pcs_cast_weight(const float *W, int64_t rows, int64_t cols, int64_t ldw, int32_t dtype, void *Wc,
                               void *WcT, pcs_stream_t stream) {
  if (!W) return pcs_set_einval("pcs_cast_weight", "null W");
  hipStream_t s = reinterpret_cast<hipStream_t>(stream);
  const int nb = blocks_for(rows * cols, 256);
  if (dtype == PCS_BF16)
    hipLaunchKernelGGL(cast_weight_kernel<bf16_t>, dim3(nb), dim3(256), 0, s, W, rows, cols, ldw,
                       reinterpret_cast<bf16_t *>(Wc), reinterpret_cast<bf16_t *>(WcT));
  else if (dtype == PCS_F32)
    hipLaunchKernelGGL(cast_weight_kernel<float>, dim3(nb), dim3(256), 0, s, W, rows, cols, ldw,
                       reinterpret_cast<float *>(Wc), reinterpret_cast<float *>(WcT));
  else return pcs_set_einval("pcs_cast_weight", "bad dtype");
  PCS_CHECK_LAUNCH();
  return 0;
}

extern "C" int pcs_adam(float *param, float *grad, float *exp_avg, float *exp_avg_sq, int64_t n,
                        const float *grad_scale, float lr, float beta1, float beta2, float eps,
                        float weight_decay, int64_t step, pcs_stream_t stream) {
  if (!param || !grad || !exp_avg || !exp_avg_sq || step < 1) return pcs_set_einval("pcs_adam", "bad arguments");
  const double bc1 = 1.0 - pow((double)beta1, (double)step);
  const double bc2 = 1.0 - pow((double)beta2, (double)step);
  hipLaunchKernelGGL(adam_kernel, dim3(blocks_for(n, 256)), dim3(256), 0, reinterpret_cast<hipStream_t>(stream),
                     param, grad, exp_avg, exp_avg_sq, n, grad_scale, lr, beta1, beta2, eps,
                     weight_decay, (float)bc1, (float)sqrt(bc2));
  PCS_CHECK_LAUNCH();
  return 0;
}

namespace {
__global__ void round_weight_kernel(const float *__restrict__ W, int64_t n, float *__restrict__ out) {
  for (int64_t i = (int64_t)blockIdx.x * blockDim.x + threadIdx.x; i < n; i += (int64_t)gridDim.x * blockDim.x)
    out[i] = bf2f(pack2bf(W[i], 0.f) & 0xffffu);
}
}

extern "C" int pcs_round_weight(const float *W, int64_t n, int32_t dtype, float *out, pcs_stream_t stream) {
  if (!W || !out || n < 0 || (dtype != PCS_F32 && dtype != PCS_BF16)) return pcs_set_einval("pcs_round_weight", "bad arguments");
  if (n == 0) return 0;
  hipStream_t s = reinterpret_cast<hipStream_t>(stream);
  if (dtype == PCS_F32) return hipMemcpyAsync(out, W, n * 4, hipMemcpyDeviceToDevice, s) == hipSuccess ? 0 : PCS_EINVAL;
  hipLaunchKernelGGL(round_weight_kernel, dim3(blocks_for(n, 256)), dim3(256), 0, s, W, n, out);
  PCS_CHECK_LAUNCH();
  return 0;
}

namespace {
template <bool SPLIT>
__global__ __launch_bounds__(256) void bnrelu_bf16_kernel(const float *__restrict__ Y, int64_t M, int K,
                                                         const float *__restrict__ s, const float *__restrict__ t,
                                                         bf16_t *__restrict__ out) {
  const int K8 = K >> 3;
  const int64_t n = M * K8;
// ... 37 lines not shown
```

### point-cloud-cnn-segmentation_amd/engine.py

```python
from __future__ import annotations

import ctypes as ct
from dataclasses import dataclass, field

import torch

from . import _lib as L

BN_EPS = 1e-5
MAX_INPUT_DIM = 8
MAX_CLASSES = 256
BN_MOMENTUM = 0.1
DROPOUT_P = 0.3

CONVS = [
    ("conv1", None, 64, "bn1"),
    ("conv2", 64, 64, "bn2"),
    ("conv3", 64, 64, "bn3"),
    ("conv4", 64, 128, "bn4"),
    ("conv5", 128, 1024, "bn5"),
    ("global_feat", 1024, 1024, "bn_global"),
    ("seg_conv1", 1088, 512, "bn_seg1"),
    ("seg_conv2", 512, 256, "bn_seg2"),
    ("seg_conv3", 256, 128, "bn_seg3"),
# ... 95 lines not shown
        return dict(pa=self.scale, pb=self.shift)


@dataclass
class Saved:
    B: int
    N: int
    train: bool
    paths: Paths = None
    ys: dict = field(default_factory=dict)
    bn: dict = field(default_factory=dict)
    masks: tuple = (None, None)
    g: torch.Tensor = None
    am: torch.Tensor = None
    ysel: torch.Tensor = None
    x: torch.Tensor = None
    logits: torch.Tensor = None
    head: dict = None
    wc: dict = None
    gram4: tuple = None
    gram2: object = None
    a5_colsum: torch.Tensor = None
    gram5: tuple = None
    wg_eff: torch.Tensor = None
    sbias_s1: torch.Tensor = None
    mask_ready: object = None


def _f32(dev, *shape):
    return torch.empty(*shape, dtype=torch.float32, device=dev)


def _call(name, *args):
    return L.call(name, *(a.data_ptr() if torch.is_tensor(a) else a for a in args))


def _struct(cls, **members):
    a = cls()
    for k, v in members.items():
        setattr(a, k, L.ptr(v) if torch.is_tensor(v) else v)
    return a


class _Bwd:

    def __init__(self, gflat, offsets, bufA):
        self.gflat, self.offsets = gflat, offsets
        self.coefs = {}
        self.bufA = bufA
        self.bufB = None
        self.keep = []
        self.st = None
        self.keep_scale = 1.0 / (1.0 - DROPOUT_P)

    def G(self, name):
        return self.gflat[self.offsets[name]:]


class Engine:

    def __init__(self, num_classes: int, dtype: str = "fp32", input_dim: int = 4, eval_trunk: str = "fp32"):
        check_dims(num_classes, input_dim)
        if eval_trunk not in ("fp32", "bf16"):
            raise ValueError(f"eval_trunk must be 'fp32' or 'bf16', got {eval_trunk!r}")
        self.input_dim = input_dim
        self.C = num_classes
        self.dtype = dtype
        self.dt, self.tdt = _dt(dtype)
        self.fp8 = dtype == "fp8"
        self.a5_dt = L.FP8 if self.fp8 else self.dt
        self.eval_trunk = eval_trunk
        self.layout = param_layout(num_classes, input_dim)
        self.numel = {n: int(torch.Size(s).numel()) for n, s in self.layout}
        self.offsets, self.total_params = flat_offsets(num_classes, input_dim)
        self.buckets = bucket_ranges(num_classes, input_dim)
        self._geo = {}
        self._side = {}
        self.flags = 0
        self.timing = None
        self.timing_tags = None
        self.record_pool_rows = False
        self.last_pool_rows = None
        self.pool_rows_override = None
        self.capture = None
        self.perturb = None
        self.fused_seg12 = True
        self.draw_beside_gram = True
        self.dropout_draw = "paired"
        L.load()

    def _launch(self, tag, name, *args):
        if self.timing is None or tag is None or (self.timing_tags is not None and tag not in self.timing_tags):
            return _call(name, *args)
        st, en = torch.cuda.Event(enable_timing=True), torch.cuda.Event(enable_timing=True)
        st.record()
        r = _call(name, *args)
        en.record()
        self.timing.setdefault(tag, []).append((st, en))
        return r

    def _dims(self, sv):
        return sv.B, sv.N, sv.B * sv.N, sv.x.device, L.stream_ptr()

    def _side_stream(self, dev):
        st = self._side.get(dev)
        if st is None:
            st = self._side.setdefault(dev, torch.cuda.Stream(device=dev))
        return st

    @staticmethod
    def _gemm_args(B, N, K, ncols, dtype, pro=L.PRO_RAW, epi=L.EPI_FWD, cps=0, flags=0, **members):
        return _struct(L.GemmArgs, num_scenes=B, scene_rows=N, K=K, Ncols=ncols, dtype=dtype, prologue=pro,
                       epilogue=epi, chunks_per_scene=cps, flags=flags, **members)

    def geometry(self, B, N, K, ncols, pro=L.PRO_BNRELU, epi=L.EPI_FWD, dtype=None, flags=None):
        dtype = self.dt if dtype is None else dtype
        flags = self.flags if flags is None else flags
        key = (B, N, K, ncols, pro, epi, flags, dtype)
        if key not in self._geo:
            a = self._gemm_args(B, N, K, ncols, dtype, pro, epi, 0, flags)
            rpc = L.workspace("pcs_gemm_geometry", ct.byref(a))
            self._geo[key] = (a.chunks_per_scene, rpc)
        return self._geo[key]

    def _empty(self, *shape, dtype=None, device):
        return torch.empty(*shape, dtype=dtype or self.tdt, device=device)

    def cast_weights(self, P):
        dev = P["conv2.weight"].device
        wc = {}
        s = L.stream_ptr()
        for conv, cin, cout, _ in CONVS:
            if conv in ("conv1", "seg_conv4"):
                continue
            W = P[f"{conv}.weight"]
            rows, ld = W.shape[0], W.shape[1]
            cols = 64 if conv == "seg_conv1" else ld
            Wc = self._empty(rows, cols, device=dev)
            WcT = self._empty(cols, rows, device=dev)
            _call("pcs_cast_weight", W, rows, cols, ld, self.dt, Wc, WcT, s)
            wc[conv] = (Wc, WcT)
        if self.fp8:
            wc["global_feat_fp8"] = self._quant_fp8(P["global_feat.weight"])
        return wc

    def _quant_fp8(self, W):
        W = W.reshape(W.shape[0], -1)
        rows, cols = W.shape
        dev = W.device
        Wq = torch.empty(rows, cols, dtype=torch.uint8, device=dev)
        sc = torch.empty(rows, dtype=torch.uint8, device=dev)
        deq = _f32(dev, rows, cols)
        _call("pcs_quant_fp8_rows", W, rows, cols, W.stride(0), Wq, sc, deq, L.stream_ptr())
        return Wq, sc, deq

    def _bn_finalize(self, P, bufs, sv, bnname, stats, C, cps, rpc, offset=None):
        B, N, _, dev, _ = self._dims(sv)
        coef = BNCoef(*(_f32(dev, C) for _ in range(4)), _f32(dev, B, C))
        g, b = P[f"{bnname}.weight"], P[f"{bnname}.bias"]
        if sv.train:
            rm, rv = bufs.get(f"{bnname}.running_mean"), bufs.get(f"{bnname}.running_var")
            upd = int(rm is not None and rv is not None)
            _call("pcs_bn_fwd_finalize", stats, B, N, C, cps, rpc, g, b, offset, rm, rv, BN_MOMENTUM, BN_EPS, upd,
                  coef.mean, coef.rstd, coef.scale, coef.shift, coef.scene_sum, L.stream_ptr())
        else:
            _call("pcs_bn_eval_coefs", g, b, bufs[f"{bnname}.running_mean"], bufs[f"{bnname}.running_var"], offset,
                  BN_EPS, C, coef.scale, coef.shift, L.stream_ptr())
        return coef

    def _gemm(self, sv, K, ncols, pro, epi, A, W, C, *, tag=None, dtype=None, extra_flags=0, **fields):
        dtype = self.dt if dtype is None else dtype
        flags = sv.paths.flags
        cps, _ = self.geometry(sv.B, sv.N, K, ncols, pro, epi, dtype, flags)
        fields.setdefault("a_keep_scale", 1.0)
        fields.setdefault("c_keep_scale", 1.0)
        a = self._gemm_args(sv.B, sv.N, K, ncols, dtype, pro, epi, cps, flags | extra_flags, A=A, W=W, C=C, **fields)
        self._launch(tag, "pcs_gemm", ct.byref(a), L.stream_ptr())

    def _wgrad_args(self, sv, cout, cin, dy_mode, x_mode, dW, ldw=0, x_keep_scale=1.0, **members):
        return _struct(L.WgradArgs, num_scenes=sv.B, scene_rows=sv.N, Cout=cout, Cin=cin, dtype=self.dt, dy_mode=dy_mode,
                       x_mode=x_mode, x_keep_scale=x_keep_scale, dW=dW, ldw=ldw, flags=sv.paths.flags, **members)

    def _wgrad(self, sv, cout, cin, dy_mode, x_mode, dW, conv1=False, tag=None, **kw):
        a = self._wgrad_args(sv, cout, cin, dy_mode, x_mode, dW, **kw)
        if conv1:
            a.splits_per_scene = max(1, min((1024 + sv.B - 1) // sv.B, (sv.N + 255) // 256))
            nbytes = sv.B * a.splits_per_scene * cout * cin * 4
        else:
            nbytes = L.workspace("pcs_wgrad_workspace", ct.byref(a))
        ws = _f32(dW.device, max(nbytes // 4, 1))
        a.partial = ws.data_ptr()
        self._launch(tag, "pcs_conv1_wgrad" if conv1 else "pcs_wgrad", ct.byref(a), L.stream_ptr())
        return ws

    def _rounded(self, W):
        if self.dt == L.F32:
            return W
        out = torch.empty_like(W)
        _call("pcs_round_weight", W, W.numel(), self.dt, out, L.stream_ptr())
        return out

    def _gram(self, Y, s_, t_, B, N, C, tag=None):
        dev = Y.device
        G, S = _f32(dev, C, C), _f32(dev, C)
        sps = ct.c_int32(0)
        nbytes = L.workspace("pcs_gram_workspace", B, N, C, self.dt, ct.byref(sps))
        ws = _f32(dev, max(nbytes // 4, 1))
        self._launch(tag, "pcs_gram", Y, s_, t_, B, N, C, self.dt, sps.value, ws, G, S, L.stream_ptr())
        return G, S, ws

    def _gram_raw(self, a5, G, beside=None):
        M = a5.shape[0]
        nbytes = L.workspace("pcs_gram_raw_workspace", M, 1024)
        ws = _f32(a5.device, nbytes // 4)
        if beside is not None:
            beside()
        self._launch("wgrad:global_feat", "pcs_gram_raw", a5, M, 1024, self.a5_dt, ws, nbytes, G, L.stream_ptr())
        return ws

    def forward(self, P, bufs, x, *, train, masks=None, seed=0, head_mode=L.HEAD_FWD,
                labels=None, class_weight=None, wsum=None, want_logits=True, saved=None):
        if not x.is_cuda:
            raise RuntimeError("pcs_amd runs on a HIP device only (no CPU fallback)")
        B, N, D = x.shape
        if D != self.input_dim:
            raise ValueError(f"expected x of shape (B, N, {self.input_dim}), got {tuple(x.shape)}")
        x = x.contiguous().float()
        sv = Saved(B=B, N=N, train=train) if saved is None else saved
        sv.B, sv.N, sv.train, sv.x = B, N, train, x
        sv.gram4 = None
        sv.paths = pt = resolve_paths(self.dtype, self.flags, self.eval_trunk, self.fused_seg12, self.draw_beside_gram,
                                      self.dropout_draw, train=train, masks_given=masks is not None)
        live = {}
        if train and masks is None and not pt.draw_beside_gram:
            self._draw_masks(sv, seed)
        sv.wc = self.cast_weights(P)
        self._trunk(P, bufs, sv)
        self._conv5(P, bufs, sv, live)
        self._global_feat(P, bufs, sv, live, seed)
        self._seg(P, bufs, sv, live, masks)
        sv.logits = _f32(x.device, B, N, self.C) if want_logits else None
        if head_mode == L.HEAD_CE:
            sv.head = self._head(P, sv, L.HEAD_CE, labels=labels, class_weight=class_weight, wsum=wsum)
        else:
            self._head(P, sv, L.HEAD_FWD)
        return sv

    def _draw_masks(self, sv, seed, max_wg=0):
        _, _, M, dev, _ = self._dims(sv)
        sv.masks = m1, m2 = tuple(torch.empty(M, w, dtype=torch.uint8, device=dev) for w in (64, 32))
        side = self._side_stream(dev)
        side.wait_stream(torch.cuda.current_stream(dev))
        with torch.cuda.stream(side):
            ss = L.stream_ptr()
            for i, (m, width) in enumerate(((m1, 512), (m2, 256))):
                if self.dropout_draw == "independent":
                    _call("pcs_dropout_bits_independent", seed, i, M, width, DROPOUT_P, m, ss)
                else:
                    _call("pcs_dropout_bits_bounded", seed, i, M, width, DROPOUT_P, m, max_wg, ss)
            sv.mask_ready = torch.cuda.Event()
            sv.mask_ready.record(side)
        m1.record_stream(side)
        m2.record_stream(side)

    def _stats_buf(self, sv, K, ncols):
        cps, rpc = self.geometry(sv.B, sv.N, K, ncols, flags=sv.paths.flags)
        return _f32(sv.x.device, sv.B * cps, ncols, 2), cps, rpc

    def _bridge(self, sv, conv, bn, K, split):
        _, _, M, dev, s = self._dims(sv)
        out = self._empty(M, 2 * K if split else K, device=dev)
        c = sv.bn[bn]
        _call("pcs_bnrelu_bf16", sv.ys[conv], M, K, c.scale, c.shift, int(split), out, s)
        return out

    def _layer(self, P, bufs, sv, conv, src, offset=None, A_raw=None, K=None, **kw):
        M, dev = sv.B * sv.N, sv.x.device
        cin, ncols, bnname = _LAYERS[conv]
        K = K or cin
        st, cps, rpc = self._stats_buf(sv, K, ncols) if sv.train else (None, 0, 0)
        f32 = kw.get("dtype") == L.F32
        y = self._empty(M, ncols, device=dev, dtype=torch.float32 if f32 else None)
        W = P[f"{conv}.weight"] if f32 else sv.wc[conv][0]
        pro, A = L.PRO_RAW, A_raw
        if A_raw is None:
            pro, A = L.PRO_BNRELU, sv.ys[src]
            kw.update(sv.bn[_LAYERS[src][2]].bnrelu())
        self._gemm(sv, K, ncols, pro, L.EPI_FWD, A, W, y, stats=st, tag=f"fwd:{conv}", **kw)
        sv.ys[conv] = y
# ... 8 lines not shown
        rpc, cps = L.workspace("pcs_gemm_geometry", ct.byref(a)), a.chunks_per_scene
        st = _f32(dev, B * cps, 64, 2) if train else None
        a = self._gemm_args(B, N, D, 64, L.F32 if pt.trunk32 else self.dt, cps=cps, A=sv.x,
                            W=P["conv1.weight"], C=y1, bias=None, stats=st)
        self._launch("fwd:conv1", "pcs_conv1_fwd", ct.byref(a), s)
        sv.ys["conv1"] = y1
        sv.bn["bn1"] = self._bn_finalize(P, bufs, sv, "bn1", st, 64, cps, rpc, P["conv1.bias"])
        tkw = {"dtype": L.F32} if pt.trunk32 else {}
        self._layer(P, bufs, sv, "conv2", "conv1", **tkw)
        if pt.fused12:
            sv.gram2 = _f32(dev, B * self.geometry(B, N, 64, 64, flags=pt.flags)[0], 64 * 64 + 64)
        self._layer(P, bufs, sv, "conv3", "conv2", **tkw, **({"gram": sv.gram2} if pt.fused12 else {}))
        self._layer(P, bufs, sv, "conv4", "conv3", **tkw)

    def _conv5(self, P, bufs, sv, live):
        B, N, M, dev, s = self._dims(sv)
        pt, train, W5 = sv.paths, sv.train, sv.wc["conv5"][0]
        st, cps, rpc = (None, 0, 0)
        if pt.gram4_stats:
            c4 = sv.bn["bn4"]
            sv.gram4 = self._gram(sv.ys["conv4"], c4.scale, c4.shift, B, N, 128, tag="fwd_stats:conv5")
            st, cps, rpc = _f32(dev, B, 1024, 2), 1, N
            _call("pcs_bn_stats_from_gram", sv.gram4[0], sv.gram4[1], M, W5, self.dt, 128, 1024, 128, B, st, s)
        elif train:
            st, cps, rpc = self._stats_buf(sv, 128, 1024)
            self._gemm(sv, 128, 1024, L.PRO_BNRELU, L.EPI_FWD, sv.ys["conv4"], W5, None,
                       stats=st, tag="fwd_stats:conv5", **sv.bn["bn4"].bnrelu())
        live["stats"] = st
        sv.bn["bn5"] = c5 = self._bn_finalize(P, bufs, sv, "bn5", st, 1024, cps, rpc, P["conv5.bias"])
        a5 = self._empty(M, 1024, device=dev, dtype=torch.uint8 if pt.fp8 else None)
        sv.a5_colsum = None
        if train and pt.wide_fast:
            cps5c, _ = self.geometry(B, N, 128, 1024, L.PRO_BNRELU, L.EPI_BNRELU, flags=pt.flags)
            sv.a5_colsum = _f32(dev, B * cps5c, 1024, 2)
        kw = dict(es=c5.scale, et=c5.shift, tag="fwd:conv5", extra_flags=L.FLAG_C_FP8 if pt.fp8 else 0)
        if pt.trunk32:
            live["W5s"] = W5s = torch.cat([W5, W5], dim=1)
            self._gemm(sv, 256, 1024, L.PRO_RAW, L.EPI_BNRELU, self._bridge(sv, "conv4", "bn4", 128, True), W5s, a5,
                       **kw)
        else:
            self._gemm(sv, 128, 1024, L.PRO_BNRELU, L.EPI_BNRELU, sv.ys["conv4"], W5, a5, stats=sv.a5_colsum,
                       **kw, **sv.bn["bn4"].bnrelu())
        if self.perturb is not None and "a5" in self.perturb:
            rows, cols, value = self.perturb["a5"]
            if pt.fp8:
                a5[rows, cols] = 0x7f if value != value else int(torch.tensor(value).to(torch.float8_e4m3fn).view(torch.uint8))
            else:
                a5[rows, cols] = value
        sv.ys["a5"] = a5

    def _global_gram_stats(self, P, sv, live, seed):
        B, N, _, dev, s = self._dims(sv)
        pt, a5 = sv.paths, sv.ys["a5"]
        Wg = P["global_feat.weight"].reshape(1024, -1)
        sv.wg_eff = sv.wc["global_feat_fp8"][2] if pt.fp8 else self._rounded(Wg)
        G5 = _f32(dev, 1024, 1024)
        max_wg = 3 * torch.cuda.get_device_properties(dev).multi_processor_count
        gws = self._gram_raw(a5, G5, beside=(lambda: self._draw_masks(sv, seed, max_wg)) if pt.draw_beside_gram else None)
        live["Sb2"] = Sb2 = _f32(dev, B, 1024, 2)
        _call("pcs_reduce_partials_grouped", sv.a5_colsum, B, sv.a5_colsum.shape[0] // B, 2048, 1.0, Sb2, s)
        Sb = Sb2[..., 0].contiguous()
        live["stats"] = st = _f32(dev, B, 1024, 2)
        qbytes = L.workspace("pcs_bn_stats_from_gram_scenes_workspace", 1024, 1024)
        live["qws"] = qws = torch.empty(qbytes // 8, dtype=torch.float64, device=dev)
        self._launch("stats:global_feat", "pcs_bn_stats_from_gram_scenes", G5, Sb, N, sv.wg_eff,
                     L.F32, 1024, 1024, 1024, B, qws, qbytes, st, s)
        sv.gram5 = (G5, Sb, gws)

    def _global_feat(self, P, bufs, sv, live, seed):
        B, N, _, dev, s = self._dims(sv)
        pt, wc, a5 = sv.paths, sv.wc, sv.ys["a5"]
        cps_g, rpc_g = self.geometry(B, N, 1024, 1024, L.PRO_RAW, L.EPI_FWD, flags=pt.flags)
        live["pool"] = pool = _f32(dev, B * cps_g, 1024, 4)
        sv.gram5 = None
        if sv.train and pt.wide_fast:
            self._global_gram_stats(P, sv, live, seed)
            st_g, cps_st, rpc_st = None, 1, N
        else:
            live["stats"] = st_g = _f32(dev, B * cps_g, 1024, 2) if sv.train else None
            cps_st, rpc_st = cps_g, rpc_g
        gamma_g = P["bn_global.weight"]
        Wf, kw = wc["global_feat"][0], dict(extra_flags=0)
        if pt.fp8:
            Wf, kw = wc["global_feat_fp8"][0], dict(w_scale=wc["global_feat_fp8"][1], extra_flags=L.FLAG_AW_FP8)
        if st_g is None and pt.glds:
            live["Wsg"] = Wsg = torch.empty_like(Wf)
            _call("pcs_sign_rows", Wf, self.a5_dt, 1024, 1024, gamma_g, Wsg, s)
            Wf, kw["extra_flags"] = Wsg, kw["extra_flags"] | L.FLAG_POOL_SIGNED_W
        self._gemm(sv, 1024, 1024, L.PRO_RAW, L.EPI_FWD, a5, Wf, None, stats=st_g, pool=pool, es=gamma_g,
                   tag="fwd:global_feat", **kw)
        sv.bn["bn_global"] = cg = self._bn_finalize(P, bufs, sv, "bn_global", live["stats"], 1024, cps_st, rpc_st,
                                                    P["global_feat.bias"])
        sv.g = _f32(dev, B, 1024)
        sv.am = torch.empty(B, 1024, dtype=torch.int32, device=dev)
        sv.ysel = _f32(dev, B, 1024)
        _call("pcs_pool_finalize", pool, B, N, 1024, cps_g, cg.scale, cg.shift, sv.g, sv.am, sv.ysel, s)
        if self.record_pool_rows:
            self.last_pool_rows = sv.am.clone()
        if self.pool_rows_override is not None:
            sv.am.copy_(self.pool_rows_override)

    def _masks(self, sv, masks):
        _, _, M, dev, _ = self._dims(sv)
        m1 = m2 = None
        if sv.train and masks is not None:
            m1, m2 = masks
            if any(tuple(m.shape) != (M, w) or m.dtype != torch.uint8 or m.device != dev for m, w in ((m1, 64), (m2, 32))):
                raise ValueError(f"dropout masks must be uint8 [{M}, 64] and [{M}, 32] on {dev}, got "
                                 f"{tuple(m1.shape)} {m1.dtype} and {tuple(m2.shape)} {m2.dtype}")
            m1, m2 = m1.contiguous(), m2.contiguous()
        elif sv.train:
            m1, m2 = sv.masks
            torch.cuda.current_stream(dev).wait_event(sv.mask_ready)
        sv.masks = (m1, m2)
        return m1, m2, 1.0 / (1.0 - DROPOUT_P) if sv.train else 1.0

    def _seg(self, P, bufs, sv, live, masks):
        B, _, _, dev, s = self._dims(sv)
        pt = sv.paths
        sbias = _f32(dev, B, 512)
        live["soff"] = soff = _f32(dev, 512)
        Ws1 = P["seg_conv1.weight"]
        _call("pcs_scene_gemv", sv.g, B, 1024, Ws1, Ws1.shape[1], 64, P["seg_conv1.bias"], 512, sbias, soff, s)
        sv.sbias_s1 = sbias
        if not pt.fused12:
            self._layer(P, bufs, sv, "seg_conv1", "conv2", soff, K=64, scene_bias=sbias,
                        A_raw=self._bridge(sv, "conv2", "bn2", 64, False) if pt.trunk32 else None)
        m1, m2, keep = self._masks(sv, masks)
        if pt.fused12:
            self._seg12(P, bufs, sv, sv.wc, sbias, soff, m1, keep)
        else:
            self._layer(P, bufs, sv, "seg_conv2", "seg_conv1", a_mask=m1, a_keep_scale=keep)
        self._layer(P, bufs, sv, "seg_conv3", "seg_conv2", a_mask=m2, a_keep_scale=keep)

    def _seg12(self, P, bufs, sv, wc, sbias, soff, m1, keep):
        B, N, M, dev, s = self._dims(sv)
        c2 = sv.bn["bn2"]
        rec = 64 * 64 + 64
        cps3 = sv.gram2.shape[0] // B
        per_scene = _f32(dev, B, rec)
        _call("pcs_reduce_partials_grouped", sv.gram2, B, cps3, rec, 1.0, per_scene, s)
        tot = _f32(dev, rec)
        _call("pcs_reduce_partials", per_scene, B, rec, 1.0, tot, 1, rec, s)
        G2 = tot[:64 * 64]
        Sb = per_scene[:, 64 * 64:].contiguous()
        Ws1 = P["seg_conv1.weight"]
        Ws1_r = self._rounded(Ws1)
        st1 = _f32(dev, B, 512, 2)
        _call("pcs_bn_stats_gram_sbias", G2, Sb, B, N, Ws1_r, Ws1.shape[1], 64, 512, sbias, st1, s)
        sv.bn["bn_seg1"] = c1 = self._bn_finalize(P, bufs, sv, "bn_seg1", st1, 512, 1, N, soff)
        y1, y2 = self._empty(M, 512, device=dev), self._empty(M, 256, device=dev)
        a = _struct(L.Seg12Args, num_scenes=B, scene_rows=N, y2=sv.ys["conv2"], s2=c2.scale, t2=c2.shift,
                    W1=wc["seg_conv1"][0], sbias=sbias, Y1=y1, s1=c1.scale, t1=c1.shift, keep1=m1, keep_scale=keep,
                    W2=wc["seg_conv2"][0], Y2=y2)
        rpc, cps = L.workspace("pcs_fwd_seg12_geometry", ct.byref(a)), a.chunks_per_scene
        st2 = _f32(dev, B * cps, 256, 2)
        a.stats = L.ptr(st2)
        self._launch("fwd:seg_conv1+2", "pcs_fwd_seg12", ct.byref(a), s)
        sv.ys["seg_conv1"], sv.ys["seg_conv2"] = y1, y2
        sv.bn["bn_seg2"] = self._bn_finalize(P, bufs, sv, "bn_seg2", st2, 256, cps, rpc, P["seg_conv2.bias"])

    def _head(self, P, sv, mode, labels=None, class_weight=None, wsum=None, dlogits=None):
        B, N, _, dev, s = self._dims(sv)
        c3 = sv.bn["bn_seg3"]
        ha = _struct(L.HeadArgs, num_scenes=B, scene_rows=N, Cin=128, num_classes=self.C, dtype=self.dt, mode=mode,
                     Y=sv.ys["seg_conv3"], s=c3.scale, t=c3.shift, W=P["seg_conv4.weight"], bias=P["seg_conv4.bias"],
                     logits=sv.logits if mode != L.HEAD_BWD else None)
        hb = None
        if mode != L.HEAD_FWD:
            L.workspace("pcs_head_geometry", ct.byref(ha))
            nch = B * ha.chunks_per_scene
            hb = dict(dZ=torch.empty(B * N * 1024, dtype=self.tdt, device=dev), stats=_f32(dev, nch, 128, 2),
                      wpartial=_f32(dev, nch, self.C * 129), loss_partial=_f32(dev, nch), cps=ha.chunks_per_scene,
                      nch=nch)
            ha.dZ, ha.stats = L.ptr(hb["dZ"]), L.ptr(hb["stats"])
            ha.wpartial, ha.loss_partial = L.ptr(hb["wpartial"]), L.ptr(hb["loss_partial"])
            ha.mean, ha.rstd = L.ptr(c3.mean), L.ptr(c3.rstd)
        if mode == L.HEAD_CE:
            ha.labels, ha.class_weight, ha.wsum = L.ptr(labels), L.ptr(class_weight), L.ptr(wsum)
        if mode == L.HEAD_BWD:
            dl = dlogits.reshape(B * N, self.C) if dlogits.dim() == 3 else dlogits
            if dl.dtype != torch.float32:
                dl = dl.float()
            ha.dlogits = L.ptr(dl)
            ha.dl_stride_row, ha.dl_stride_col = dl.stride(0), dl.stride(1)
            hb["dl"] = dl
        self._launch(f"head:{mode}", "pcs_head", ct.byref(ha), s)
        return hb

    def backward(self, P, sv, gflat, dlogits=None, on_bucket=None):
        bucket = on_bucket or (lambda name: None)
        if not sv.train:
            raise RuntimeError("backward needs a train-mode forward (BatchNorm batch statistics)")
        hb = self._head(P, sv, L.HEAD_BWD, dlogits=dlogits) if dlogits is not None else sv.head
        bw = _Bwd(gflat, self.offsets, hb["dZ"])
        scene_s1 = self._bwd_seg32(P, sv, bw, hb)
        sp = self._bwd_pool(P, sv, bw, scene_s1)
        dA2 = self._bwd_seg1_local(P, sv, bw)
        bucket("seg")
        Wg_r, st5, cps5 = self._bwd_global_dgrad(P, sv, bw, sp)
        self._bwd_global_wgrad(P, sv, bw, sp, Wg_r)
        bucket("global")
        self._bwd_conv5(P, sv, bw, st5, cps5)
        self._bwd_trunk(P, sv, bw, dA2)
        bucket("tail")
        return hb

    def _bn_bwd(self, P, sv, bw, bnname, conv, stats, cps, scene_s1=None):
        B, N, _, dev, s = self._dims(sv)
        fc = sv.bn[bnname]
        C = fc.mean.shape[0]
        al, be, ga = (_f32(dev, C) for _ in range(3))
        _call("pcs_bn_bwd_finalize", stats, B, N, C, cps, fc.mean, fc.rstd, P[f"{bnname}.weight"], fc.scene_sum, al, be,
              ga, bw.G(f"{bnname}.weight"), bw.G(f"{bnname}.bias"), bw.G(f"{conv}.bias"), scene_s1, s)
        bw.coefs[bnname] = (al, be, ga)

    def _wgrad_bn(self, sv, bw, conv, dz, prev, x_mask=None, cin=None, ldw=0):
        al, be, ga = bw.coefs[_LAYERS[conv][2]]
        pc = sv.bn[_LAYERS[prev][2]]
        bw.keep.append(self._wgrad(
            sv, _LAYERS[conv][1], cin or _LAYERS[conv][0], L.PRO_BWD, L.PRO_BNRELU, bw.G(f"{conv}.weight"), ldw=ldw,
            tag=f"wgrad:{conv}", dZ=dz, Y=sv.ys[conv], alpha=al, beta=be, gamma=ga, X=sv.ys[prev], s=pc.scale,
            t=pc.shift, x_mask=x_mask, x_keep_scale=bw.keep_scale if x_mask is not None else 1.0))

    def _bwd_layer(self, P, sv, bw, conv, dz, prev, out, c_mask=None, addend=None, per_scene=False):
        B, N, _, dev, s = self._dims(sv)
        pt, WT = sv.paths, sv.wc[conv][1]
        cin, cout, bn = _LAYERS[conv]
        al, be, ga = bw.coefs[bn]
        pc = sv.bn[_LAYERS[prev][2]]
        f = dict(A2=sv.ys[conv], pa=al, pb=be, pc=ga, Yp=sv.ys[prev], es=pc.scale, et=pc.shift, emean=pc.mean,
                 erstd=pc.rstd, c_mask=c_mask, c_keep_scale=bw.keep_scale if c_mask is not None else 1.0, addend=addend)
        nbytes = -1
        if pt.wide_fast:
            a = self._gemm_args(B, N, cout, cin, self.dt, L.PRO_BWD, L.EPI_DGRAD, 0, pt.flags, A=dz, W=WT, C=out,
                                a_keep_scale=1.0, **f)
            nbytes = L.load().pcs_dgrad_wgrad_bn_workspace(ct.byref(a))
        if nbytes > 0:
            cps = a.chunks_per_scene
            st = _f32(dev, B * cps, cin, 2)
            ws = _f32(dev, nbytes // 4)
            a.stats = L.ptr(st)
            self._launch(f"dgrad+wgrad:{conv}", "pcs_dgrad_wgrad_bn", ct.byref(a), ws, bw.G(f"{conv}.weight"), 0, s)
            bw.keep.append(ws)
        else:
            cps, _ = self.geometry(B, N, cout, cin, L.PRO_BWD, L.EPI_DGRAD, flags=pt.flags)
            st = _f32(dev, B * cps, cin, 2)
            self._gemm(sv, cout, cin, L.PRO_BWD, L.EPI_DGRAD, dz, WT, out, stats=st, tag=f"dgrad:{conv}", **f)
            self._wgrad_bn(sv, bw, conv, dz, prev, x_mask=c_mask)
        bw.st = st
        scene_s1 = _f32(dev, B, pc.mean.shape[0]) if per_scene else None
        self._bn_bwd(P, sv, bw, _LAYERS[prev][2], prev, st, cps, scene_s1)
        return scene_s1

    def _bwd_seg32(self, P, sv, bw, hb):
        _, _, M, dev, s = self._dims(sv)
        m1, m2 = sv.masks
        _call("pcs_reduce_partials", hb["wpartial"], hb["nch"], self.C * 129, 1.0, bw.G("seg_conv4.weight"),
              self.C * 129, self.C * 129, s)
        self._bn_bwd(P, sv, bw, "bn_seg3", "seg_conv3", hb["stats"], hb["cps"])
        bw.bufB = torch.empty(M * 1024, dtype=self.tdt, device=dev)
        self._bwd_layer(P, sv, bw, "seg_conv3", bw.bufA, "seg_conv2", bw.bufB, c_mask=m2)
        return self._bwd_layer(P, sv, bw, "seg_conv2", bw.bufB, "seg_conv1", bw.bufA, c_mask=m1, per_scene=True)

    def _bwd_pool(self, P, sv, bw, scene_s1):
        B, N, _, dev, s = self._dims(sv)
        a1, b1, g1 = bw.coefs["bn_seg1"]
        cg = sv.bn["bn_global"]
        bw.coefs["bn_global"] = ag, bg, gg = tuple(_f32(dev, 1024) for _ in range(3))
        sp = _f32(dev, B, 1024)
        csum = _f32(dev, B, 512)
        Ws1 = P["seg_conv1.weight"]
        pa = _struct(L.PoolBwdArgs, num_scenes=B, scene_rows=N, Cs=512, Cg=1024, col_off=64, s1_alpha=a1, s1_beta=b1,
                     s1_gamma=g1, s1_scene_s1=scene_s1, s1_scene_sum=sv.bn["bn_seg1"].scene_sum, W_s1=Ws1,
                     ldw=Ws1.shape[1], g=sv.g, ysel=sv.ysel, g_mean=cg.mean, g_rstd=cg.rstd,
                     g_gamma=P["bn_global.weight"], g_scene_sum=cg.scene_sum, dW_s1_global=bw.G("seg_conv1.weight"),
                     csum=csum, alpha=ag, beta_c=bg, gamma_c=gg, dgamma=bw.G("bn_global.weight"),
                     dbeta=bw.G("bn_global.bias"), dbias=bw.G("global_feat.bias"), sp=sp)
        _call("pcs_pool_bwd", ct.byref(pa), s)
        bw.keep.append(csum)
        return sp

    def _bwd_seg1_local(self, P, sv, bw):
        B, N, M, dev, s = self._dims(sv)
        a1, b1, g1 = bw.coefs["bn_seg1"]
        dz_s1, ys, Ws1 = bw.bufA, sv.ys, P["seg_conv1.weight"]
        dA2 = torch.empty(M, 64, dtype=self.tdt, device=dev)
        if not sv.paths.wide_fast:
            self._gemm(sv, 512, 64, L.PRO_BWD, L.EPI_RAW, dz_s1, sv.wc["seg_conv1"][1], dA2,
                       A2=ys["seg_conv1"], pa=a1, pb=b1, pc=g1, tag="dgrad:seg_conv1")
            self._wgrad_bn(sv, bw, "seg_conv1", dz_s1, "conv2", cin=64, ldw=Ws1.shape[1])
            return dA2
        p2 = sv.bn["bn2"]
        Ws1_r = self._rounded(Ws1)
        WaT, Hs1 = self._empty(64, 512, device=dev), self._empty(64, 64, device=dev)
        _call("pcs_bn_fold", Ws1_r, 512, 64, Ws1.shape[1], a1, b1, g1, self.dt, WaT, None, Hs1, s)
        fa = self._wgrad_args(sv, 512, 64, L.PRO_RAW, L.PRO_BNRELU, bw.G("seg_conv1.weight"), ldw=Ws1.shape[1],
                              dZ=dz_s1, alpha=a1, beta=b1, gamma=g1, X=ys["conv2"], s=p2.scale, t=p2.shift)
        nbytes = L.workspace("pcs_dgrad_wgrad_folded_workspace", ct.byref(fa))
        ws1 = _f32(dev, nbytes // 4)
        fa.partial = ws1.data_ptr()
        self._launch("dgrad+wgrad:seg_conv1", "pcs_dgrad_wgrad_folded", ct.byref(fa), WaT, Hs1, Ws1_r, sv.sbias_s1, dA2, s)
        bw.keep.append((ws1, Ws1_r, WaT, Hs1))
        return dA2

    def _bwd_global_dgrad(self, P, sv, bw, sp):
        B, N, M, dev, s = self._dims(sv)
        pt, a5, dz5 = sv.paths, sv.ys["a5"], bw.bufB
        bg, gg = bw.coefs["bn_global"][1:]
        Wg_r = sv.wg_eff if sv.gram5 is not None else \
            sv.wc["global_feat_fp8"][2] if pt.fp8 else self._rounded(P["global_feat.weight"])
        cvec = _f32(dev, 1024)
        Hg = _f32(dev, 1024, 1024) if pt.fp8 else self._empty(1024, 1024, device=dev)
        _call("pcs_bn_fold", Wg_r, 1024, 1024, Wg_r.shape[1], None, bg, gg, L.F32 if pt.fp8 else self.dt, None, cvec, Hg, s)
        pool_rows = dict(pool_idx=sv.am, pool_coef=sp, pool_w=Wg_r, pool_ldw=Wg_r.shape[1], pool_c=1024)
        if pt.fp8:
            Hq, hsc, _ = self._quant_fp8(Hg)
            Hg = (Hg, Hq, hsc)
            W, kw = Hq, dict(w_scale=hsc, extra_flags=L.FLAG_AW_FP8)
        else:
            W, kw = Hg, ({} if pt.glds else pool_rows)
        cps5, _ = self.geometry(B, N, 1024, 1024, L.PRO_RAW, L.EPI_DGRAD, flags=pt.flags)
        st5 = _f32(dev, B * cps5, 1024, 2)
        self._gemm(sv, 1024, 1024, L.PRO_RAW, L.EPI_DGRAD, a5, W, dz5, bias=cvec, Yp=a5, stats=st5,
                   tag="dgrad:global_feat", **kw)
        if pt.fp8 or pt.glds:
            _call("pcs_pool_rows_add", dz5, self.dt, a5, self.a5_dt, B, N, 1024, sv.am, sp, Wg_r, Wg_r.shape[1], 1024,
                  st5, cps5, s)
        if self.perturb is not None and "dz5" in self.perturb:
            c0, c1, scale = self.perturb["dz5"]
            dz5.view(M, 1024)[:, c0:c1].mul_(scale)
        if self.capture is not None:
            self.capture.update(dz5=dz5.view(M, 1024).clone(), a5=a5, H=Hg, cvec=cvec, am=sv.am.clone(),
                                sp=sp.clone(), Wg_r=Wg_r)
        bw.keep.append((Hg, cvec))
        return Wg_r, st5, cps5

    def _bwd_global_wgrad(self, P, sv, bw, sp, Wg_r):
        B, N, _, dev, s = self._dims(sv)
        a5 = sv.ys["a5"]
        _, bg, gg = bw.coefs["bn_global"]
        ones = torch.ones(1024, dtype=torch.float32, device=dev)
        zeros = torch.zeros(1024, dtype=torch.float32, device=dev)
        raw = sv.paths.wide_fast and sv.a5_colsum is not None
        gram = _f32(dev, 1024, 1024) if sv.gram5 is not None or raw else None
        if sv.gram5 is not None:
            gram, Sb, ws = sv.gram5
            colsum = _f32(dev, 1024)
            _call("pcs_reduce_partials", Sb, B, 1024, 1.0, colsum, 1024, 1024, s)
        elif raw:
            ws = self._gram_raw(a5, gram)
            cs2 = _f32(dev, 1024, 2)
            _call("pcs_reduce_partials", sv.a5_colsum, sv.a5_colsum.shape[0], 2048, 1.0, cs2, 2048, 2048, s)
            colsum = cs2[:, 0].contiguous()
            bw.keep.append(cs2)
        else:
            gram, colsum, ws = self._gram(a5, ones, zeros, B, N, 1024, tag="wgrad:global_feat")
        self._launch("wgrad_asm:global_feat", "pcs_gram_wgrad", gram, colsum, Wg_r, P["global_feat.weight"].shape[1],
                     bg, gg, sp, sv.am, a5, ones, zeros, B, 1024, 1024, self.a5_dt, None, None,
                     bw.G("global_feat.weight"), 1024, s)
        bw.keep.append((ones, zeros, gram, colsum, ws, Wg_r))

    def _bwd_conv5(self, P, sv, bw, st5, cps5):
        B, N, M, dev, s = self._dims(sv)
        dz5, y4, cap = bw.bufB, sv.ys["conv4"], self.capture
        pc4, pc5 = sv.bn["bn4"], sv.bn["bn5"]
        r5 = _f32(dev, 1024, 128)
        bw.keep.append(self._wgrad(sv, 1024, 128, L.PRO_RAW, L.PRO_BNRELU, r5, tag="wgrad:conv5",
                                   dZ=dz5, X=y4, s=pc4.scale, t=pc4.shift))
        if cap is not None:
            cap.update(r5=r5.clone(), y4=y4, s4=pc4.scale, t4=pc4.shift)
        _call("pcs_bn_s2_from_r", st5, B * cps5, 1024, r5, sv.wc["conv5"][0], self.dt, 128, 128, pc5.mean, pc5.rstd, s)
        self._bn_bwd(P, sv, bw, "bn5", "conv5", st5, cps5)
        al5, be5, ga5 = bw.coefs["bn5"]
        W5_r = self._rounded(P["conv5.weight"])
        ws_t, c5, h4 = self._empty(128, 1024, device=dev), _f32(dev, 128), self._empty(128, 128, device=dev)
        _call("pcs_bn_fold", W5_r, 1024, 128, 128, al5, be5, ga5, self.dt, ws_t, c5, h4, s)
        cps4, _ = self.geometry(B, N, 1024 + 128, 128, L.PRO_CAT, L.EPI_DGRAD, flags=sv.paths.flags)
        bw.st = _f32(dev, B * cps4, 128, 2)
        self._gemm(sv, 1024 + 128, 128, L.PRO_CAT, L.EPI_DGRAD, dz5, ws_t, bw.bufA, K1=1024, A2=y4,
                   W2=h4, pa=pc4.scale, pb=pc4.shift, bias=c5, Yp=y4, es=pc4.scale, et=pc4.shift,
                   emean=pc4.mean, erstd=pc4.rstd, stats=bw.st, tag="dgrad:conv5")
        if cap is not None:
            cap.update(dz4=bw.bufA[:M * 128].view(M, 128).clone(), ws_t=ws_t, h4=h4, c5=c5)
        g4, s4, ws4 = sv.gram4 if sv.gram4 is not None else \
            self._gram(y4, pc4.scale, pc4.shift, B, N, 128, tag="gram:conv4")
        self._launch("wgrad_asm:conv5", "pcs_gram_wgrad", g4, s4, W5_r, 128, be5, ga5, None, None, None, None, None, B,
                     1024, 128, self.dt, r5, al5, bw.G("conv5.weight"), 128, s)
        bw.keep.append((ws_t, c5, h4, r5, g4, s4, ws4, W5_r))
        self._bn_bwd(P, sv, bw, "bn4", "conv4", bw.st, cps4)

    def _bwd_trunk(self, P, sv, bw, dA2):
        self._bwd_layer(P, sv, bw, "conv4", bw.bufA, "conv3", bw.bufB)
        self._bwd_layer(P, sv, bw, "conv3", bw.bufB, "conv2", bw.bufA, addend=dA2)
        self._bwd_layer(P, sv, bw, "conv2", bw.bufA, "conv1", bw.bufB)
        al, be, ga = bw.coefs["bn1"]
        bw.keep.append(self._wgrad(sv, 64, self.input_dim, L.PRO_BWD, L.PRO_RAW, bw.G("conv1.weight"),
                                   ldw=self.input_dim, conv1=True, tag="wgrad:conv1", dZ=bw.bufB, Y=sv.ys["conv1"],
                                   alpha=al, beta=be, gamma=ga, X=sv.x))
```

### point-cloud-cnn-segmentation_amd/model.py

```python
from __future__ import annotations

import threading

import torch
import torch.nn as nn

from . import _lib as L
from .engine import BNS, FLAT_EXTRA, Engine, check_dims, flat_offsets, param_layout


class _DropoutState:

    def __init__(self, seed: int):
        self.lock = threading.Lock()
        self.gen = torch.Generator().manual_seed(seed)
        self.masks = None

    def next_seed(self) -> int:
        with self.lock:
            return int(torch.randint(0, 2 ** 62, (1,), generator=self.gen).item())

    def take_masks(self):
        with self.lock:
            m, self.masks = self.masks, None
            return m


class _PointNetFunction(torch.autograd.Function):
    @staticmethod
    def forward(ctx, x, module, *params):
        eng = module._engine()
        P = module._param_dict()
        bufs = module._buffer_dict()
        train = module.training
        masks = module._take_dropout_masks() if train else None
        seed = module._next_seed() if train and masks is None else 0
        sv = eng.forward(P, bufs, x, train=train, masks=masks, seed=seed)
        if train:
            for bn, _ in BNS:
                getattr(module, bn).num_batches_tracked.add_(1)
        ctx.sv = sv
        ctx.module = module
        return sv.logits

    @staticmethod
    def backward(ctx, dlogits):
        module, sv = ctx.module, ctx.sv
        eng = module._engine()
        P = module._param_dict()
        gflat = torch.empty(eng.total_params, dtype=torch.float32, device=dlogits.device)
        eng.backward(P, sv, gflat, dlogits=dlogits)
        grads = []
        for name, shape in eng.layout:
            off = eng.offsets[name]
            grads.append(gflat[off:off + eng.numel[name]].view(shape))
        ctx.sv = None
        return (None, None, *grads)


class PointNetSegmentation(nn.Module):

    def __init__(self, num_classes, input_dim=4, *, compute_dtype: str = "fp32", eval_trunk: str = "fp32",
                 dropout_draw: str = "paired"):
        super().__init__()
        self.conv1 = nn.Conv1d(input_dim, 64, 1)
        self.conv2 = nn.Conv1d(64, 64, 1)
        self.conv3 = nn.Conv1d(64, 64, 1)
        self.conv4 = nn.Conv1d(64, 128, 1)
        self.conv5 = nn.Conv1d(128, 1024, 1)
        self.global_feat = nn.Conv1d(1024, 1024, 1)
        self.seg_conv1 = nn.Conv1d(1088, 512, 1)
        self.seg_conv2 = nn.Conv1d(512, 256, 1)
        self.seg_conv3 = nn.Conv1d(256, 128, 1)
        self.seg_conv4 = nn.Conv1d(128, num_classes, 1)
        self.bn1 = nn.BatchNorm1d(64)
        self.bn2 = nn.BatchNorm1d(64)
        self.bn3 = nn.BatchNorm1d(64)
        self.bn4 = nn.BatchNorm1d(128)
        self.bn5 = nn.BatchNorm1d(1024)
        self.bn_global = nn.BatchNorm1d(1024)
        self.bn_seg1 = nn.BatchNorm1d(512)
        self.bn_seg2 = nn.BatchNorm1d(256)
        self.bn_seg3 = nn.BatchNorm1d(128)
        self.dropout = nn.Dropout(0.3)
        self.num_classes = num_classes
        self.input_dim = input_dim
        self.compute_dtype = compute_dtype
        self.eval_trunk = eval_trunk
        if dropout_draw not in ("paired", "independent"):
            raise ValueError(f"dropout_draw must be 'paired' or 'independent', got {dropout_draw!r}")
        self.dropout_draw = dropout_draw
        check_dims(num_classes, input_dim)
        self._eng = None
# ... 63 lines not shown
```

### point-cloud-cnn-segmentation_amd/train.py

```python
from __future__ import annotations

import torch
import torch.distributed as dist

from . import _lib as L
from .engine import BNS
from .optim import FusedAdam, flat_buffers


def _all_reduce(t, group=None, async_op=False):
    if t.is_cuda and dist.get_backend(group) == "gloo":
        h = t.cpu()
        dist.all_reduce(h, group=group)
        t.copy_(h)
        return None
    return dist.all_reduce(t, group=group, async_op=async_op)


class GradientBuckets:

    def __init__(self, flat, ranges, group=None):
        self.flat, self.ranges, self.group = flat, ranges, group
        self.works = []
        self.issued = []

    def issue(self, name):
        lo, hi = self.ranges[name]
        w = _all_reduce(self.flat[lo:hi], self.group, async_op=True)
        self.issued.append(name)
        if w is not None:
            self.works.append(w)

    def wait(self):
        if sorted(self.issued) != sorted(self.ranges):
            raise RuntimeError(f"gradient buckets issued {self.issued}, expected {sorted(self.ranges)}")
        for w in self.works:
            w.wait()
        self.works = []


class FusedTrainStep:
    def __init__(self, model, optimizer: FusedAdam | None = None, class_weight=None,
                 process_group=None, lr=1e-3, weight_decay=1e-4):
        self.model = model
        self.opt = optimizer or FusedAdam(model, lr=lr, weight_decay=weight_decay)
        dev = next(model.parameters()).device
        C = model.num_classes
        w = torch.ones(C) if class_weight is None else torch.as_tensor(class_weight, dtype=torch.float32)
        self.class_weight = w.to(dev, torch.float32).contiguous()
        self.pg = process_group
        self.wsum = torch.empty(3, dtype=torch.float32, device=dev)
        self.counts = torch.empty(max(16, C), dtype=torch.int64, device=dev)
        self.inv_wsum = torch.empty(1, dtype=torch.float32, device=dev)
        self.timing = None
        self.timing_tags = None

    def _distributed(self):
        if not (dist.is_available() and dist.is_initialized()):
            return False
        return self.pg is not None or dist.get_world_size() > 1

    def __call__(self, points, labels, masks=None, seed=None):
        model = self.model
        eng = model._engine()
        eng.timing = self.timing
        eng.timing_tags = self.timing_tags
        model.train()
        P = model._param_dict()
        bufs = model._buffer_dict()
        pflat, gflat = flat_buffers(model)
        ext = gflat[eng.total_params:]
        labels = labels.reshape(-1)
        if labels.dtype != torch.int64:
            labels = labels.long()
        s = L.stream_ptr()
        L.call("pcs_ce_weight_sum", L.ptr(labels), labels.numel(), L.ptr(self.class_weight),
               model.num_classes, L.ptr(self.counts), L.ptr(self.wsum), s)
        ddp = self._distributed()
        if seed is None:
            seed = model._next_seed()
        sv = eng.forward(P, bufs, points, train=True, masks=masks, seed=seed,
                         head_mode=L.HEAD_CE, labels=labels, class_weight=self.class_weight,
                         wsum=None if ddp else self.wsum, want_logits=False)
        for bn, _ in BNS:
            getattr(model, bn).num_batches_tracked.add_(1)
        hb = sv.head
        L.call("pcs_reduce_partials", L.ptr(hb["loss_partial"]), hb["nch"], 1, 1.0, L.ptr(ext), 1, 1, s)
        if ddp:
            ext[1:3].copy_(self.wsum[:2])
            buckets = GradientBuckets(gflat, eng.buckets, self.pg)
            eng.backward(P, sv, gflat, on_bucket=buckets.issue)
            buckets.wait()
            torch.reciprocal(ext[1:2], out=self.inv_wsum)
            self.opt.grad_scale = self.inv_wsum
            loss = ext[0] / ext[1]
        else:
            eng.backward(P, sv, gflat)
            self.opt.grad_scale = None
            loss = ext[0] / self.wsum[0]
        del sv, hb
        self.opt.step()
        return loss
```

Baseline: 117.6 M points/s.

## Batch small launches: grouped partial reductions, weight prep, counters, and kernel tweaks

Several changes aim to cut launch count and small-kernel overhead. Partial wgrad reductions are deferred and flushed as batched jobs, weight casting and rounding move into one multi-job prepare kernel, and the num_batches_tracked increments become a single counter kernel. Alongside this, a handful of unrelated kernel tweaks land: pool_rows_add runs with 1024-thread blocks and prefetches loads, the BN finalize does a sub-grouped Welford merge, gram_quad stages its tiles in float LDS, and the folded reduce uses a smaller block with unroll pragmas. These add bookkeeping complexity and carry some precision and ordering risk from the deferred reductions and the float staging.

```diff
diff --git a/include/pcs.h b/include/pcs.h
--- a/include/pcs.h
+++ b/include/pcs.h
@@ -257,6 +257,36 @@
 int pcs_reduce_partials_grouped(const float *partial, int64_t ngroups, int64_t nslabs, int64_t len,
                                 float scale, float *out, pcs_stream_t stream);
 
+#define PCS_REDUCE_MAX_JOBS 16
+typedef struct {
+  const float *partial;
+  int64_t nslabs, len;
+  float scale;
+  float *out;
+  int64_t ldo, row_len;
+} pcs_reduce_job;
+int pcs_reduce_partials_batch(const pcs_reduce_job *jobs, int32_t njobs, pcs_stream_t stream);
+
+int pcs_wgrad_partials(const pcs_wgrad_args *args, pcs_stream_t stream);
+int pcs_conv1_wgrad_partials(const pcs_wgrad_args *args, pcs_stream_t stream);
+int pcs_dgrad_wgrad_bn_partials(const pcs_gemm_args *args, float *workspace, pcs_stream_t stream);
+
+#define PCS_WEIGHT_MAX_JOBS 16
+typedef struct {
+  const float *W;
+  int64_t rows, cols, ldw;
+  int32_t dtype;
+  void *Wc, *WcT;
+  float *Wr;
+  int64_t ldr;
+  const float *sign_of;
+  void *Wsigned;
+} pcs_weight_job;
+int pcs_prepare_weights(const pcs_weight_job *jobs, int32_t njobs, pcs_stream_t stream);
+
+#define PCS_COUNTER_MAX 32
+int pcs_increment_counters(int64_t *const *counters, int32_t n, pcs_stream_t stream);
+
 int pcs_cast_weight(const float *W, int64_t rows, int64_t cols, int64_t ldw, int32_t dtype,
                     void *Wc, void *WcT, pcs_stream_t stream);
 
diff --git a/point-cloud-cnn-segmentation_amd/_lib.py b/point-cloud-cnn-segmentation_amd/_lib.py
--- a/point-cloud-cnn-segmentation_amd/_lib.py
+++ b/point-cloud-cnn-segmentation_amd/_lib.py
@@ -98,6 +98,20 @@
         ("dZ", _vp), ("mean", _vp), ("rstd", _vp), ("stats", _vp), ("wpartial", _vp),
         ("loss_partial", _vp),
     ]
+
+
+class ReduceJob(ct.Structure):
+    _fields_ = [("partial", _vp), ("nslabs", _i64), ("len", _i64), ("scale", _f), ("out", _vp), ("ldo", _i64),
+                ("row_len", _i64)]
+
+
+class WeightJob(ct.Structure):
+    _fields_ = [("W", _vp), ("rows", _i64), ("cols", _i64), ("ldw", _i64), ("dtype", _i32), ("Wc", _vp), ("WcT", _vp),
+                ("Wr", _vp), ("ldr", _i64), ("sign_of", _vp), ("Wsigned", _vp)]
+
+
+REDUCE_MAX_JOBS = WEIGHT_MAX_JOBS = 16
+COUNTER_MAX = 32
 
 
 SIGNATURES = [
@@ -217,6 +231,12 @@
     ("pcs_gather_rows", ct.c_int, [_vp, _i64, _vp, _i64, _i32, _vp, _vp]),
     ("pcs_voxel_padded_index", ct.c_int, [_vp, _i64, _vp, _i64, _i64, _vp, _vp]),
     ("pcs_pad_scatter", ct.c_int, [_vp, _vp, _i32, _vp, _i64, _i64, _vp, _vp, _vp, _vp]),
+    ("pcs_reduce_partials_batch", ct.c_int, [ct.POINTER(ReduceJob), _i32, _vp]),
+    ("pcs_wgrad_partials", ct.c_int, [ct.POINTER(WgradArgs), _vp]),
+    ("pcs_conv1_wgrad_partials", ct.c_int, [ct.POINTER(WgradArgs), _vp]),
+    ("pcs_dgrad_wgrad_bn_partials", ct.c_int, [ct.POINTER(GemmArgs), _vp, _vp]),
+    ("pcs_prepare_weights", ct.c_int, [ct.POINTER(WeightJob), _i32, _vp]),
+    ("pcs_increment_counters", ct.c_int, [ct.POINTER(_vp), _i32, _vp]),
     ("pcs_last_error", ct.c_char_p, []),
 ]
 
diff --git a/point-cloud-cnn-segmentation_amd/csrc/fused_bwd.hip b/point-cloud-cnn-segmentation_amd/csrc/fused_bwd.hip
--- a/point-cloud-cnn-segmentation_amd/csrc/fused_bwd.hip
+++ b/point-cloud-cnn-segmentation_amd/csrc/fused_bwd.hip
@@ -221,11 +221,13 @@
 
 constexpr int RG_LEN = COUT * CIN + CIN * CIN;
 
-__global__ __launch_bounds__(256) void folded_reduce_kernel(const float *__restrict__ part, int nslab, int sps,
-                                                            int B, float *__restrict__ red, float *__restrict__ Sb) {
-  const int i = blockIdx.x * 256 + threadIdx.x;
+constexpr int FR_T = 64;
+__global__ __launch_bounds__(FR_T) void folded_reduce_kernel(const float *__restrict__ part, int nslab, int sps,
+                                                             int B, float *__restrict__ red, float *__restrict__ Sb) {
+  const int i = blockIdx.x * FR_T + threadIdx.x;
   if (i < RG_LEN) {
     float t = 0.f;
+#pragma unroll 16
     for (int sl = 0; sl < nslab; ++sl) t += part[(int64_t)sl * SLAB_F + i];
     red[i] = t;
   } else if (i < RG_LEN + B * CIN) {
@@ -264,6 +266,7 @@
                                                           const float *__restrict__ sbias, float *__restrict__ cvec) {
   const int b = blockIdx.x, j = threadIdx.x;
   float t = 0.f;
+#pragma unroll 16
   for (int k = 0; k < COUT; ++k)
     t = fmaf(fmaf(gamma[k], sbias[(int64_t)b * COUT + k], beta[k]), W[(int64_t)k * ldw + j], t);
   cvec[b * CIN + j] = t;
@@ -306,7 +309,7 @@
   hipLaunchKernelGGL(folded_cvec_kernel, dim3(B), dim3(CIN), 0, s, W, a.ldw, a.beta, a.gamma, scene_bias, cvec);
   hipLaunchKernelGGL(dgrad_wgrad_s1_kernel, dim3(nb), dim3(THREADS), 0, s, a, static_cast<const bf16_t *>(WaT),
                      static_cast<bf16_t *>(dX), rps, static_cast<const bf16_t *>(H), cvec);
-  hipLaunchKernelGGL(folded_reduce_kernel, dim3((RG_LEN + B * CIN + 255) / 256), dim3(256), 0, s, a.partial, nb,
+  hipLaunchKernelGGL(folded_reduce_kernel, dim3((RG_LEN + B * CIN + FR_T - 1) / FR_T), dim3(FR_T), 0, s, a.partial, nb,
                      a.splits_per_scene, B, red, Sb);
   hipLaunchKernelGGL(folded_assemble_kernel, dim3(COUT), dim3(CIN), 0, s, red, Sb, B, W, a.ldw, a.alpha, a.beta,
                      a.gamma, scene_bias, a.dW, a.ldw);
@@ -613,9 +616,8 @@
   return (int64_t)a->num_scenes * a->chunks_per_scene * a->K * a->Ncols * 4;
 }
 
-extern "C" int pcs_dgrad_wgrad_bn(const pcs_gemm_args *ap, float *partial, float *dW, int64_t ldw,
-                                  pcs_stream_t stream) {
-  if (!ap || !partial || !dW) return pcs_set_einval("pcs_dgrad_wgrad_bn", "null argument");
+static int dgrad_wgrad_bn_run(const pcs_gemm_args *ap, float *partial, float *dW, int64_t ldw, pcs_stream_t stream) {
+  if (!ap || !partial) return pcs_set_einval("pcs_dgrad_wgrad_bn", "null argument");
   pcs_gemm_args a = *ap;
   if (pcs_dgrad_wgrad_bn_workspace(&a) < 0) return PCS_EINVAL;
   if (a.chunks_per_scene != ap->chunks_per_scene)
@@ -627,7 +629,7 @@
   if (a.scene_rows * a.num_scenes >= (int64_t)1 << 31) return pcs_set_einval("pcs_dgrad_wgrad_bn", "M must be < 2^31");
   if (pcs_seg4_applicable(a)) {
     const int rc = pcs_seg4_launch(a, partial, reinterpret_cast<hipStream_t>(stream));
-    if (rc) return rc;
+    if (rc || !dW) return rc;
     const int nslab = (int)(a.num_scenes * a.chunks_per_scene);
     return pcs_reduce_partials(partial, nslab, (int64_t)a.K * a.Ncols, 1.0f, dW, ldw ? ldw : a.Ncols, a.Ncols, stream);
   }
@@ -637,7 +639,17 @@
   int rc;
   if (a.K == 64) rc = launch_bn<64, 64, 64, 64>(a, partial, rps, s);
   else rc = launch_bn<128, 64, 64, 64>(a, partial, rps, s);
-  if (rc) return rc;
+  if (rc || !dW) return rc;
   const int nslab = (int)(a.num_scenes * a.chunks_per_scene);
   return pcs_reduce_partials(partial, nslab, (int64_t)a.K * a.Ncols, 1.0f, dW, ldw ? ldw : a.Ncols, a.Ncols, stream);
 }
+
+extern "C" int pcs_dgrad_wgrad_bn(const pcs_gemm_args *ap, float *partial, float *dW, int64_t ldw,
+                                  pcs_stream_t stream) {
+  if (!dW) return pcs_set_einval("pcs_dgrad_wgrad_bn", "null argument");
+  return dgrad_wgrad_bn_run(ap, partial, dW, ldw, stream);
+}
+
+extern "C" int pcs_dgrad_wgrad_bn_partials(const pcs_gemm_args *ap, float *partial, pcs_stream_t stream) {
+  return dgrad_wgrad_bn_run(ap, partial, nullptr, 0, stream);
+}
diff --git a/point-cloud-cnn-segmentation_amd/csrc/gemm_glds.hip b/point-cloud-cnn-segmentation_amd/csrc/gemm_glds.hip
--- a/point-cloud-cnn-segmentation_amd/csrc/gemm_glds.hip
+++ b/point-cloud-cnn-segmentation_amd/csrc/gemm_glds.hip
@@ -616,21 +616,21 @@
 constexpr int PR_PARTS = 16;
 
 template <typename T, typename TY>
-__global__ __launch_bounds__(256) void pool_rows_add_kernel(T *__restrict__ dz, const TY *__restrict__ Yp, int64_t N,
+__global__ __launch_bounds__(1024) void pool_rows_add_kernel(T *__restrict__ dz, const TY *__restrict__ Yp, int64_t N,
                                                             int Ncols, const int32_t *__restrict__ idx,
                                                             const float *__restrict__ coef, const float *__restrict__ Wp,
                                                             int64_t ldw, int P, float *__restrict__ stats, int cps) {
   __shared__ unsigned long long keys[PR_MAXC];
-  const int b = blockIdx.y, part = blockIdx.z, parts = gridDim.z, tid = threadIdx.x;
-  const int n = blockIdx.x * 256 + tid;
+  const int b = blockIdx.y, part = blockIdx.z, parts = gridDim.z, tid = threadIdx.x, nt = blockDim.x;
+  const int n = blockIdx.x * nt + tid;
   int Pp = 1;
   while (Pp < P) Pp <<= 1;
-  for (int c = tid; c < Pp; c += 256)
+  for (int c = tid; c < Pp; c += nt)
     keys[c] = c < P ? ((unsigned long long)(uint32_t)idx[(int64_t)b * P + c] << 11) | (unsigned)c : ~0ull;
   __syncthreads();
   for (int k = 2; k <= Pp; k <<= 1) {
     for (int j = k >> 1; j > 0; j >>= 1) {
-      for (int i = tid; i < Pp; i += 256) {
+      for (int i = tid; i < Pp; i += nt) {
         const int ixj = i ^ j;
         if (ixj > i) {
           const unsigned long long x = keys[i], y = keys[ixj];
@@ -652,15 +652,26 @@
   float ds1 = 0.f, v = 0.f;
   constexpr int U = 8;
   for (int p = p0; p < p1; p += U) {
-    float cf[U], wv[U];
+    float cf[U], wv[U], ypv[U], dzv[U];
+    bool ends[U];
 #pragma unroll
     for (int u = 0; u < U; ++u) {
       cf[u] = 0.f;
       wv[u] = 0.f;
-      if (p + u < p1) {
-        const int c = sch_at(p + u);
+      ypv[u] = 0.f;
+      dzv[u] = 0.f;
+      ends[u] = false;
+      const int q = p + u;
+      if (q < p1) {
+        const int c = sch_at(q);
         cf[u] = coef[(int64_t)b * P + c];
         wv[u] = Wp[(int64_t)c * ldw + n];
+        const int64_t m = (int64_t)srow_at(q);
+        ends[u] = (q + 1 == p1 || srow_at(q + 1) != srow_at(q));
+        if (ends[u] && m >= (int64_t)b * N && m < (int64_t)(b + 1) * N) {
+          ypv[u] = load_elem(Yp, m * Ncols + n);
+          dzv[u] = load_elem(dz, m * Ncols + n);
+        }
       }
     }
 #pragma unroll
@@ -668,11 +679,11 @@
       const int q = p + u;
       if (q >= p1) break;
       v = fmaf(cf[u], wv[u], v);
-      if (q + 1 == p1 || srow_at(q + 1) != srow_at(q)) {
+      if (ends[u]) {
         const int64_t m = (int64_t)srow_at(q);
         const int64_t o = m * Ncols + n;
-        if (m >= (int64_t)b * N && m < (int64_t)(b + 1) * N && load_elem(Yp, o) > 0.f) {
-          const float d = load_elem(dz, o) + v;
+        if (m >= (int64_t)b * N && m < (int64_t)(b + 1) * N && ypv[u] > 0.f) {
+          const float d = dzv[u] + v;
           if constexpr (sizeof(T) == 2) dz[o] = (T)(pack2bf(d, 0.f) & 0xffffu);
           else dz[o] = d;
           ds1 += v;
@@ -695,9 +706,10 @@
     return pcs_set_einval("pcs_pool_rows_add", "bad arguments (0 < pool_c <= 1024, pool_ldw >= Ncols)");
   hipStream_t s = reinterpret_cast<hipStream_t>(stream);
   const int parts = stats ? (chunks_per_scene < PR_PARTS ? chunks_per_scene : PR_PARTS) : PR_PARTS;
-  const dim3 grid((Ncols + 255) / 256, (unsigned)num_scenes, (unsigned)parts);
+  const int nt = Ncols % 1024 == 0 ? 1024 : 256;
+  const dim3 grid((Ncols + nt - 1) / nt, (unsigned)num_scenes, (unsigned)parts);
 #define PCS_PRA(T, TY)                                                                                          \
-  hipLaunchKernelGGL((pool_rows_add_kernel<T, TY>), grid, dim3(256), 0, s, static_cast<T *>(dz),                 \
+  hipLaunchKernelGGL((pool_rows_add_kernel<T, TY>), grid, dim3(nt), 0, s, static_cast<T *>(dz),                  \
                      static_cast<const TY *>(Yp), scene_rows, (int)Ncols, pool_idx, pool_coef, pool_w, pool_ldw, \
                      (int)pool_c, stats, (int)chunks_per_scene)
   if (dz_dtype == PCS_BF16 && yp_dtype == PCS_BF16) PCS_PRA(bf16_t, bf16_t);
diff --git a/point-cloud-cnn-segmentation_amd/csrc/gemm_tn.hip b/point-cloud-cnn-segmentation_amd/csrc/gemm_tn.hip
--- a/point-cloud-cnn-segmentation_amd/csrc/gemm_tn.hip
+++ b/point-cloud-cnn-segmentation_amd/csrc/gemm_tn.hip
@@ -308,14 +308,14 @@
   return nslabs * a->Cout * a->Cin * 4;
 }
 
-extern "C" int pcs_wgrad(const pcs_wgrad_args *ap, pcs_stream_t stream) {
+static int wgrad_run(const pcs_wgrad_args *ap, bool reduce, pcs_stream_t stream) {
   if (!ap) return pcs_set_einval("pcs_wgrad", "null args");
   pcs_wgrad_args a = *ap;
   if (reserved_set(a)) return pcs_set_einval("pcs_wgrad", "reserved0..2 must be NULL (removed in ABI 3)");
   if (a.dy_mode != PCS_PRO_RAW && a.dy_mode != PCS_PRO_BNRELU && a.dy_mode != PCS_PRO_BWD)
     return pcs_set_einval("pcs_wgrad", "unknown dy_mode (PCS_PRO_RAW, PCS_PRO_BNRELU or PCS_PRO_BWD)");
   if (a.Cout % 64 || a.Cin % 64) return pcs_set_einval("pcs_wgrad", "Cout/Cin must be multiples of 64");
-  if (!a.X || !a.partial || !a.dW) return pcs_set_einval("pcs_wgrad", "missing operand");
+  if (!a.X || !a.partial || (reduce && !a.dW)) return pcs_set_einval("pcs_wgrad", "missing operand");
   if (a.dy_mode == PCS_PRO_RAW ? !a.dZ : (!a.Y || !a.beta || !a.gamma))
     return pcs_set_einval("pcs_wgrad", "dy operands missing (RAW: dZ; otherwise: Y, beta, gamma)");
   if (a.dy_mode == PCS_PRO_BWD && (!a.dZ || !a.alpha)) return pcs_set_einval("pcs_wgrad", "PRO_BWD needs dZ, alpha");
@@ -330,11 +330,15 @@
   else if (a.dtype == PCS_BF16) rc = dispatch_tiles<bf16_t>(a, rps, s);
   else if (a.dtype == PCS_F32) rc = dispatch_tiles<float>(a, rps, s);
   else return pcs_set_einval("pcs_wgrad", "bad dtype");
-  if (rc) return rc;
+  if (rc || !reduce) return rc;
   const int64_t nslabs = a.num_scenes * a.splits_per_scene;
   return pcs_reduce_partials(a.partial, nslabs, (int64_t)a.Cout * a.Cin, 1.0f, a.dW,
                              a.ldw ? a.ldw : a.Cin, a.Cin, stream);
 }
+
+extern "C" int pcs_wgrad(const pcs_wgrad_args *ap, pcs_stream_t stream) { return wgrad_run(ap, true, stream); }
+
+extern "C" int pcs_wgrad_partials(const pcs_wgrad_args *ap, pcs_stream_t stream) { return wgrad_run(ap, false, stream); }
 
 namespace {
 
diff --git a/point-cloud-cnn-segmentation_amd/csrc/gram.hip b/point-cloud-cnn-segmentation_amd/csrc/gram.hip
--- a/point-cloud-cnn-segmentation_amd/csrc/gram.hip
+++ b/point-cloud-cnn-segmentation_amd/csrc/gram.hip
@@ -227,8 +227,8 @@
 template <typename T>
 __global__ __launch_bounds__(256) void gram_quad_kernel(const float *__restrict__ G, const T *__restrict__ W,
                                                         int64_t ldw, int Cin, double *__restrict__ part) {
-  __shared__ double gs[16][64];
-  __shared__ double wt[16][65];
+  __shared__ float gs[16][64];
+  __shared__ float wt[16][65];
   __shared__ double red[16][64];
   const int C = gridDim.x * 64, c0 = blockIdx.x * 64, j0 = blockIdx.y * 64;
   const int tid = threadIdx.x, tx = tid & 15, ty = tid >> 4;
@@ -242,15 +242,15 @@
   for (int k0 = kz0; k0 < kz1; k0 += 16) {
 #pragma unroll
     for (int e = tid; e < 1024; e += 256) {
-      gs[e >> 6][e & 63] = (double)G[(int64_t)(k0 + (e >> 6)) * Cin + j0 + (e & 63)];
-      wt[e & 15][e >> 4] = (double)load_elem(W, (int64_t)(c0 + (e >> 4)) * ldw + k0 + (e & 15));
+      gs[e >> 6][e & 63] = G[(int64_t)(k0 + (e >> 6)) * Cin + j0 + (e & 63)];
+      wt[e & 15][e >> 4] = load_elem(W, (int64_t)(c0 + (e >> 4)) * ldw + k0 + (e & 15));
     }
     __syncthreads();
 #pragma unroll 4
     for (int kk = 0; kk < 16; ++kk) {
       double a[4], b[4];
 #pragma unroll
-      for (int p = 0; p < 4; ++p) { a[p] = gs[kk][ty * 4 + p]; b[p] = wt[kk][tx * 4 + p]; }
+      for (int p = 0; p < 4; ++p) { a[p] = (double)gs[kk][ty * 4 + p]; b[p] = (double)wt[kk][tx * 4 + p]; }
 #pragma unroll
       for (int p = 0; p < 4; ++p)
 #pragma unroll
diff --git a/point-cloud-cnn-segmentation_amd/csrc/small.hip b/point-cloud-cnn-segmentation_amd/csrc/small.hip
--- a/point-cloud-cnn-segmentation_amd/csrc/small.hip
+++ b/point-cloud-cnn-segmentation_amd/csrc/small.hip
@@ -149,44 +149,71 @@
   }
 }
 
+constexpr int BN_SG = 4;
+
+__device__ __forceinline__ void welford_merge(double &na, double &ma, double &qa, double nb, double mb, double qb) {
+  if (nb > 0) {
+    const double nn = na + nb, d = mb - ma;
+    ma += d * nb / nn;
+    qa += qb + d * d * na * nb / nn;
+    na = nn;
+  }
+}
+
 __global__ __launch_bounds__(THREADS) void bn_fwd_finalize_kernel(
     const float *stats, int64_t B, int64_t N, int C, int cps, int64_t rpc, const float *gamma,
     const float *beta, const float *moff, float *rmean, float *rvar, float momentum, float eps, int update,
     float *mean_o, float *rstd_o, float *scale_o, float *shift_o, float *scene_sum) {
-  __shared__ double sh[THREADS][3];
+  __shared__ double sh[BN_SG][THREADS][3];
   const int c = blockIdx.x, tid = threadIdx.x;
   double gn = 0, gmean = 0, gm2 = 0;
-  for (int64_t b = 0; b < B; ++b) {
-    double n = 0, mu = 0, q = 0;
-    for (int j = tid; j < cps; j += THREADS) {
-      const double nb = (double)pcs_min64(rpc, N - (int64_t)j * rpc);
-      const float2 p = *reinterpret_cast<const float2 *>(stats + ((b * cps + j) * C + c) * 2);
-      const double nn = n + nb, d = (double)p.x - mu;
-      mu += d * nb / nn;
-      q += (double)p.y + d * d * n * nb / nn;
-      n = nn;
-    }
-    sh[tid][0] = n; sh[tid][1] = mu; sh[tid][2] = q;
-    __syncthreads();
-    for (int s = THREADS / 2; s > 0; s >>= 1) {
-      if (tid < s) {
-        const double na = sh[tid][0], nb = sh[tid + s][0];
-        if (nb > 0) {
-          const double nn = na + nb, d = sh[tid + s][1] - sh[tid][1];
-          sh[tid][1] += d * nb / nn;
-          sh[tid][2] += sh[tid + s][2] + d * d * na * nb / nn;
-          sh[tid][0] = nn;
+  for (int64_t b0 = 0; b0 < B; b0 += BN_SG) {
+    const int nb_s = (int)pcs_min64(BN_SG, B - b0);
+    double n[BN_SG], mu[BN_SG], q[BN_SG];
+#pragma unroll
+    for (int u = 0; u < BN_SG; ++u) {
+      n[u] = 0; mu[u] = 0; q[u] = 0;
+      if (u < nb_s)
+        for (int j = tid; j < cps; j += THREADS) {
+          const double nb = (double)pcs_min64(rpc, N - (int64_t)j * rpc);
+          const float2 p = *reinterpret_cast<const float2 *>(stats + (((b0 + u) * cps + j) * C + c) * 2);
+          const double nn = n[u] + nb, d = (double)p.x - mu[u];
+          mu[u] += d * nb / nn;
+          q[u] += (double)p.y + d * d * n[u] * nb / nn;
+          n[u] = nn;
         }
-      }
+    }
+#pragma unroll
+    for (int s = THREADS / 2; s >= 64; s >>= 1) {
+      if (tid >= s && tid < 2 * s)
+#pragma unroll
+        for (int u = 0; u < BN_SG; ++u) { sh[u][tid][0] = n[u]; sh[u][tid][1] = mu[u]; sh[u][tid][2] = q[u]; }
       __syncthreads();
+      if (tid < s)
+#pragma unroll
+        for (int u = 0; u < BN_SG; ++u)
+          welford_merge(n[u], mu[u], q[u], sh[u][tid + s][0], sh[u][tid + s][1], sh[u][tid + s][2]);
+    }
+    if (tid < 64) {
+#pragma unroll
+      for (int s = 32; s > 0; s >>= 1)
+#pragma unroll
+        for (int u = 0; u < BN_SG; ++u) {
+          const double nb = __shfl_down(n[u], s), mb = __shfl_down(mu[u], s), qb = __shfl_down(q[u], s);
+          welford_merge(n[u], mu[u], q[u], nb, mb, qb);
+        }
     }
     if (tid == 0) {
-      const double nb = sh[0][0], mb = sh[0][1], qb = sh[0][2];
-      if (scene_sum) scene_sum[b * C + c] = (float)(nb * mb);
-      const double nn = gn + nb, d = mb - gmean;
-      gmean += d * nb / nn;
-      gm2 += qb + d * d * gn * nb / nn;
-      gn = nn;
+#pragma unroll
+      for (int u = 0; u < BN_SG; ++u) {
+        if (u >= nb_s) break;
+        const double nb = n[u], mb = mu[u], qb = q[u];
+        if (scene_sum) scene_sum[(b0 + u) * C + c] = (float)(nb * mb);
+        const double nn = gn + nb, d = mb - gmean;
+        gmean += d * nb / nn;
+        gm2 += qb + d * d * gn * nb / nn;
+        gn = nn;
+      }
     }
     __syncthreads();
   }
@@ -221,25 +248,45 @@
     const float *stats, int64_t B, int64_t N, int C, int cps, const float *mean, const float *rstd,
     const float *gamma, const float *scene_sum, float *alpha, float *beta_c, float *gamma_c,
     float *dgamma, float *dbeta, float *dbias, float *scene_s1) {
-  __shared__ double sh[THREADS][2];
+  __shared__ double sh[BN_SG][THREADS][2];
   const int c = blockIdx.x, tid = threadIdx.x;
   double S1 = 0, S2 = 0, Sy = 0;
-  for (int64_t b = 0; b < B; ++b) {
-    double s1 = 0, s2 = 0;
-    for (int j = tid; j < cps; j += THREADS) {
-      const float2 p = *reinterpret_cast<const float2 *>(stats + ((b * cps + j) * C + c) * 2);
-      s1 += p.x; s2 += p.y;
-    }
-    sh[tid][0] = s1; sh[tid][1] = s2;
-    __syncthreads();
-    for (int s = THREADS / 2; s > 0; s >>= 1) {
-      if (tid < s) { sh[tid][0] += sh[tid + s][0]; sh[tid][1] += sh[tid + s][1]; }
+  for (int64_t b0 = 0; b0 < B; b0 += BN_SG) {
+    const int nb_s = (int)pcs_min64(BN_SG, B - b0);
+    double s1[BN_SG], s2[BN_SG];
+#pragma unroll
+    for (int u = 0; u < BN_SG; ++u) {
+      s1[u] = 0; s2[u] = 0;
+      if (u < nb_s)
+        for (int j = tid; j < cps; j += THREADS) {
+          const float2 p = *reinterpret_cast<const float2 *>(stats + (((b0 + u) * cps + j) * C + c) * 2);
+          s1[u] += p.x; s2[u] += p.y;
+        }
+    }
+#pragma unroll
+    for (int s = THREADS / 2; s >= 64; s >>= 1) {
+      if (tid >= s && tid < 2 * s)
+#pragma unroll
+        for (int u = 0; u < BN_SG; ++u) { sh[u][tid][0] = s1[u]; sh[u][tid][1] = s2[u]; }
       __syncthreads();
+      if (tid < s)
+#pragma unroll
+        for (int u = 0; u < BN_SG; ++u) { s1[u] += sh[u][tid + s][0]; s2[u] += sh[u][tid + s][1]; }
+    }
+    if (tid < 64) {
+#pragma unroll
+      for (int s = 32; s > 0; s >>= 1)
+#pragma unroll
+        for (int u = 0; u < BN_SG; ++u) { s1[u] += __shfl_down(s1[u], s); s2[u] += __shfl_down(s2[u], s); }
     }
     if (tid == 0) {
-      if (scene_s1) scene_s1[b * C + c] = (float)sh[0][0];
-      S1 += sh[0][0]; S2 += sh[0][1];
-      if (scene_sum) Sy += scene_sum[b * C + c];
+#pragma unroll
+      for (int u = 0; u < BN_SG; ++u) {
+        if (u >= nb_s) break;
+        if (scene_s1) scene_s1[(b0 + u) * C + c] = (float)s1[u];
+        S1 += s1[u]; S2 += s2[u];
+        if (scene_sum) Sy += scene_sum[(b0 + u) * C + c];
+      }
     }
     __syncthreads();
   }
@@ -338,6 +385,7 @@
 #pragma unroll
     for (int u = 0; u < PBC_SB; ++u) dg[u] = 0.f;
     if (k < a.Cg) {
+#pragma unroll 8
       for (int n = n0; n < n1; ++n) {
         const float w = a.W_s1[(int64_t)n * a.ldw + a.col_off + k];
 #pragma unroll
@@ -1023,12 +1071,10 @@
 }
 
 template <int TPO>
-__global__ void reduce_partials_kernel(const float *partial, int64_t nslabs, int64_t len, float scale,
-                                       float *out, int64_t ldo, int64_t row_len) {
-  partial += (int64_t)blockIdx.y * nslabs * len;
-  out += (int64_t)blockIdx.y * len;
+__device__ __forceinline__ void reduce_partials_block(const float *partial, int64_t nslabs, int64_t len, float scale,
+                                                      float *out, int64_t ldo, int64_t row_len, int64_t block) {
   const int sub = threadIdx.x % TPO;
-  const int64_t i4 = ((int64_t)blockIdx.x * (blockDim.x / TPO) + threadIdx.x / TPO) * 4;
+  const int64_t i4 = (block * (blockDim.x / TPO) + threadIdx.x / TPO) * 4;
   const bool vec = (row_len & 3) == 0 && i4 + 4 <= len;
   float v[4] = {0.f, 0.f, 0.f, 0.f};
   if (i4 < len) {
@@ -1057,6 +1103,74 @@
       out[(i / row_len) * ldo + i % row_len] = v[e] * scale;
     }
   }
+}
+
+template <int TPO>
+__global__ void reduce_partials_kernel(const float *partial, int64_t nslabs, int64_t len, float scale,
+                                       float *out, int64_t ldo, int64_t row_len) {
+  reduce_partials_block<TPO>(partial + (int64_t)blockIdx.y * nslabs * len, nslabs, len, scale,
+                             out + (int64_t)blockIdx.y * len, ldo, row_len, blockIdx.x);
+}
+
+__host__ __device__ inline int reduce_tpo(int64_t nslabs) { return nslabs >= 64 ? 32 : nslabs >= 8 ? 8 : 1; }
+
+struct reduce_batch_table {
+  pcs_reduce_job job[PCS_REDUCE_MAX_JOBS];
+  int32_t first[PCS_REDUCE_MAX_JOBS + 1];
+  int32_t njobs;
+};
+
+__global__ __launch_bounds__(256) void reduce_partials_batch_kernel(reduce_batch_table t) {
+  int j = 0;
+  while (j + 1 < t.njobs && (int)blockIdx.x >= t.first[j + 1]) ++j;
+  const pcs_reduce_job &q = t.job[j];
+  const int64_t block = (int)blockIdx.x - t.first[j];
+  switch (reduce_tpo(q.nslabs)) {
+    case 32: reduce_partials_block<32>(q.partial, q.nslabs, q.len, q.scale, q.out, q.ldo, q.row_len, block); break;
+    case 8: reduce_partials_block<8>(q.partial, q.nslabs, q.len, q.scale, q.out, q.ldo, q.row_len, block); break;
+    default: reduce_partials_block<1>(q.partial, q.nslabs, q.len, q.scale, q.out, q.ldo, q.row_len, block); break;
+  }
+}
+
+struct weight_table {
+  pcs_weight_job job[PCS_WEIGHT_MAX_JOBS];
+  int32_t first[PCS_WEIGHT_MAX_JOBS + 1];
+  int32_t njobs;
+};
+
+template <typename T>
+__device__ __forceinline__ void prepare_weight_elem(const pcs_weight_job &q, int64_t i) {
+  const int64_t r = i / q.cols, c = i % q.cols;
+  const float v = q.W[r * q.ldw + c];
+  T o;
+  float rounded;
+  if constexpr (sizeof(T) == 4) { o = v; rounded = v; }
+  else { o = (T)(pack2bf(v, 0.f) & 0xffffu); rounded = bf2f(o); }
+  if (q.Wc) static_cast<T *>(q.Wc)[i] = o;
+  if (q.WcT) static_cast<T *>(q.WcT)[c * q.rows + r] = o;
+  if (q.Wr) q.Wr[r * q.ldr + c] = rounded;
+  if (q.Wsigned) {
+    const bool flip = q.sign_of[r] < 0.f;
+    if constexpr (sizeof(T) == 4)
+      static_cast<uint32_t *>(q.Wsigned)[i] = flip ? __float_as_uint(o) ^ 0x80000000u : __float_as_uint(o);
+    else
+      static_cast<uint16_t *>(q.Wsigned)[i] = flip ? (uint16_t)(o ^ 0x8000u) : o;
+  }
+}
+
+__global__ __launch_bounds__(256) void prepare_weights_kernel(weight_table t) {
+  int j = 0;
+  while (j + 1 < t.njobs && (int)blockIdx.x >= t.first[j + 1]) ++j;
+  const pcs_weight_job &q = t.job[j];
+  const int64_t i = (int64_t)((int)blockIdx.x - t.first[j]) * 256 + threadIdx.x;
+  if (i >= q.rows * q.cols) return;
+  if (q.dtype == PCS_BF16) prepare_weight_elem<bf16_t>(q, i);
+  else prepare_weight_elem<float>(q, i);
+}
+
+struct counter_table { int64_t *p[PCS_COUNTER_MAX]; };
+__global__ void increment_counters_kernel(counter_table t, int n) {
+  if ((int)threadIdx.x < n) *t.p[threadIdx.x] += 1;
 }
 
 template <typename T>
@@ -1137,8 +1251,8 @@
   return 0;
 }
 
-extern "C" int pcs_conv1_wgrad(const pcs_wgrad_args *ap, pcs_stream_t stream) {
-  if (!ap || !ap->dZ || !ap->Y || !ap->X || !ap->partial || !ap->dW)
+static int conv1_wgrad_run(const pcs_wgrad_args *ap, bool reduce, pcs_stream_t stream) {
+  if (!ap || !ap->dZ || !ap->Y || !ap->X || !ap->partial || (reduce && !ap->dW))
     return pcs_set_einval("pcs_conv1_wgrad", "missing operand");
   if (ap->Cout != 64 || ap->Cin < 1 || ap->Cin > C1_MAXK)
     return pcs_set_einval("pcs_conv1_wgrad", "conv1 is input_dim (1..8) -> 64");
@@ -1161,9 +1275,16 @@
 #undef PCS_C1W_BF
 #undef PCS_C1W_F32
   PCS_CHECK_LAUNCH();
+  if (!reduce) return 0;
   return pcs_reduce_partials(a.partial, nb, 64 * a.Cin, 1.f, a.dW, a.ldw ? a.ldw : a.Cin, a.Cin, stream);
 }
 #undef PCS_C1_SWITCH
+
+extern "C" int pcs_conv1_wgrad(const pcs_wgrad_args *ap, pcs_stream_t stream) { return conv1_wgrad_run(ap, true, stream); }
+
+extern "C" int pcs_conv1_wgrad_partials(const pcs_wgrad_args *ap, pcs_stream_t stream) {
+  return conv1_wgrad_run(ap, false, stream);
+}
 
 extern "C" int pcs_bn_fwd_finalize(const float *stats, int64_t B, int64_t N, int32_t C, int32_t cps,
                                    int64_t rpc, const float *gamma, const float *beta,
@@ -1428,6 +1549,68 @@
   return 0;
 }
 
+extern "C" int pcs_reduce_partials_batch(const pcs_reduce_job *jobs, int32_t njobs, pcs_stream_t stream) {
+  if (!jobs) return pcs_set_einval("pcs_reduce_partials_batch", "null job table");
+  if (njobs < 1 || njobs > PCS_REDUCE_MAX_JOBS)
+    return pcs_set_einval("pcs_reduce_partials_batch", "1 <= njobs <= PCS_REDUCE_MAX_JOBS (16)");
+  reduce_batch_table t = {};
+  int64_t nblocks = 0;
+  for (int j = 0; j < njobs; ++j) {
+    const pcs_reduce_job &q = jobs[j];
+    if (!q.partial || !q.out || q.len <= 0 || q.nslabs <= 0 || q.row_len <= 0)
+      return pcs_set_einval("pcs_reduce_partials_batch", "bad job (as pcs_reduce_partials)");
+    t.job[j] = q;
+    t.first[j] = (int32_t)nblocks;
+    const int64_t per = 256 / reduce_tpo(q.nslabs);
+    nblocks += ((q.len + 3) / 4 + per - 1) / per;
+    if (nblocks > INT32_MAX) return pcs_set_einval("pcs_reduce_partials_batch", "too many outputs for one launch");
+  }
+  t.first[njobs] = (int32_t)nblocks;
+  t.njobs = njobs;
+  hipLaunchKernelGGL(reduce_partials_batch_kernel, dim3((unsigned)nblocks), dim3(256), 0,
+                     reinterpret_cast<hipStream_t>(stream), t);
+  PCS_CHECK_LAUNCH();
+  return 0;
+}
+
+extern "C" int pcs_prepare_weights(const pcs_weight_job *jobs, int32_t njobs, pcs_stream_t stream) {
+  if (!jobs) return pcs_set_einval("pcs_prepare_weights", "null job table");
+  if (njobs < 1 || njobs > PCS_WEIGHT_MAX_JOBS)
+    return pcs_set_einval("pcs_prepare_weights", "1 <= njobs <= PCS_WEIGHT_MAX_JOBS (16)");
+  weight_table t = {};
+  int64_t nblocks = 0;
+  for (int j = 0; j < njobs; ++j) {
+    const pcs_weight_job &q = jobs[j];
+    if (!q.W || q.rows <= 0 || q.cols <= 0 || q.ldw < q.cols || (q.dtype != PCS_F32 && q.dtype != PCS_BF16) ||
+        (q.Wr && q.ldr < q.cols) || (q.Wsigned && !q.sign_of))
+      return pcs_set_einval("pcs_prepare_weights", "bad job (W, rows, cols > 0, ldw >= cols, dtype F32 or BF16, "
+                                                   "ldr >= cols with Wr, sign_of with Wsigned)");
+    t.job[j] = q;
+    t.first[j] = (int32_t)nblocks;
+    nblocks += (q.rows * q.cols + 255) / 256;
+    if (nblocks > INT32_MAX) return pcs_set_einval("pcs_prepare_weights", "too many elements for one launch");
+  }
+  t.first[njobs] = (int32_t)nblocks;
+  t.njobs = njobs;
+  hipLaunchKernelGGL(prepare_weights_kernel, dim3((unsigned)nblocks), dim3(256), 0,
+                     reinterpret_cast<hipStream_t>(stream), t);
+  PCS_CHECK_LAUNCH();
+  return 0;
+}
+
+extern "C" int pcs_increment_counters(int64_t *const *counters, int32_t n, pcs_stream_t stream) {
+  if (!counters || n < 1 || n > PCS_COUNTER_MAX)
+    return pcs_set_einval("pcs_increment_counters", "1 <= n <= PCS_COUNTER_MAX (32) device pointers");
+  counter_table t = {};
+  for (int i = 0; i < n; ++i) {
+    if (!counters[i]) return pcs_set_einval("pcs_increment_counters", "null counter");
+    t.p[i] = counters[i];
+  }
+  hipLaunchKernelGGL(increment_counters_kernel, dim3(1), dim3(64), 0, reinterpret_cast<hipStream_t>(stream), t, (int)n);
+  PCS_CHECK_LAUNCH();
+  return 0;
+}
+
 extern "C" int pcs_cast_weight(const float *W, int64_t rows, int64_t cols, int64_t ldw, int32_t dtype, void *Wc,
                                void *WcT, pcs_stream_t stream) {
   if (!W) return pcs_set_einval("pcs_cast_weight", "null W");
diff --git a/point-cloud-cnn-segmentation_amd/engine.py b/point-cloud-cnn-segmentation_amd/engine.py
--- a/point-cloud-cnn-segmentation_amd/engine.py
+++ b/point-cloud-cnn-segmentation_amd/engine.py
@@ -171,9 +171,20 @@
         self.keep = []
         self.st = None
         self.keep_scale = 1.0 / (1.0 - DROPOUT_P)
+        self.sums = []
 
     def G(self, name):
         return self.gflat[self.offsets[name]:]
+
+    def defer_sum(self, partial, nslabs, rows, cols, out, ldo=0):
+        self.sums.append(_struct(L.ReduceJob, partial=partial, nslabs=nslabs, len=rows * cols, scale=1.0, out=out,
+                                 ldo=ldo or cols, row_len=cols))
+
+    def flush_sums(self):
+        for i in range(0, len(self.sums), L.REDUCE_MAX_JOBS):
+            jobs = self.sums[i:i + L.REDUCE_MAX_JOBS]
+            L.call("pcs_reduce_partials_batch", (L.ReduceJob * len(jobs))(*jobs), len(jobs), L.stream_ptr())
+        self.sums = []
 
 
 class Engine:
@@ -195,6 +206,7 @@
         self.buckets = bucket_ranges(num_classes, input_dim)
         self._geo = {}
         self._side = {}
+        self._unit = {}
         self.flags = 0
         self.timing = None
         self.timing_tags = None
@@ -221,6 +233,12 @@
     def _dims(self, sv):
         return sv.B, sv.N, sv.B * sv.N, sv.x.device, L.stream_ptr()
 
+    def _unit_coefs(self, dev):
+        if dev not in self._unit:
+            self._unit[dev] = (torch.ones(1024, dtype=torch.float32, device=dev),
+                               torch.zeros(1024, dtype=torch.float32, device=dev))
+        return self._unit[dev]
+
     def _side_stream(self, dev):
         st = self._side.get(dev)
         if st is None:
@@ -245,10 +263,13 @@
     def _empty(self, *shape, dtype=None, device):
         return torch.empty(*shape, dtype=dtype or self.tdt, device=device)
 
-    def cast_weights(self, P):
+    def cast_weights(self, P, sv=None):
         dev = P["conv2.weight"].device
-        wc = {}
-        s = L.stream_ptr()
+        wc, jobs = {}, []
+        pt = sv.paths if sv is not None and sv.train else None
+        rounded = ()
+        if pt is not None and pt.bf16:
+            rounded = ("global_feat", "conv5") + (("seg_conv1",) if pt.wide_fast else ())
         for conv, cin, cout, _ in CONVS:
             if conv in ("conv1", "seg_conv4"):
                 continue
@@ -257,11 +278,27 @@
             cols = 64 if conv == "seg_conv1" else ld
             Wc = self._empty(rows, cols, device=dev)
             WcT = self._empty(cols, rows, device=dev)
-            _call("pcs_cast_weight", W, rows, cols, ld, self.dt, Wc, WcT, s)
             wc[conv] = (Wc, WcT)
+            job = dict(W=W, rows=rows, cols=cols, ldw=ld, dtype=self.dt, Wc=Wc, WcT=WcT)
+            if conv in rounded and not (conv == "global_feat" and self.fp8):
+                wc[f"{conv}.rounded"] = Wr = torch.empty_like(W.reshape(rows, ld))
+                job.update(Wr=Wr, ldr=ld)
+            if conv == "global_feat" and pt is not None and pt.wide_fast and pt.glds and not self.fp8:
+                wc["global_feat.signed"] = Ws = torch.empty_like(Wc)
+                job.update(sign_of=P["bn_global.weight"], Wsigned=Ws)
+            jobs.append(job)
+        table = (L.WeightJob * len(jobs))(*(_struct(L.WeightJob, **j) for j in jobs))
+        L.call("pcs_prepare_weights", table, len(jobs), L.stream_ptr())
         if self.fp8:
             wc["global_feat_fp8"] = self._quant_fp8(P["global_feat.weight"])
         return wc
+
+    @staticmethod
+    def count_batches(bufs):
+        cs = [bufs[f"{bn}.num_batches_tracked"] for bn, _ in BNS if f"{bn}.num_batches_tracked" in bufs]
+        if cs:
+            L.call("pcs_increment_counters", (ct.c_void_p * len(cs))(*(c.data_ptr() for c in cs)), len(cs),
+                   L.stream_ptr())
 
     def _quant_fp8(self, W):
         W = W.reshape(W.shape[0], -1)
@@ -300,7 +337,7 @@
         return _struct(L.WgradArgs, num_scenes=sv.B, scene_rows=sv.N, Cout=cout, Cin=cin, dtype=self.dt, dy_mode=dy_mode,
                        x_mode=x_mode, x_keep_scale=x_keep_scale, dW=dW, ldw=ldw, flags=sv.paths.flags, **members)
 
-    def _wgrad(self, sv, cout, cin, dy_mode, x_mode, dW, conv1=False, tag=None, **kw):
+    def _wgrad(self, sv, cout, cin, dy_mode, x_mode, dW, conv1=False, tag=None, bw=None, **kw):
         a = self._wgrad_args(sv, cout, cin, dy_mode, x_mode, dW, **kw)
         if conv1:
             a.splits_per_scene = max(1, min((1024 + sv.B - 1) // sv.B, (sv.N + 255) // 256))
@@ -309,15 +346,15 @@
             nbytes = L.workspace("pcs_wgrad_workspace", ct.byref(a))
         ws = _f32(dW.device, max(nbytes // 4, 1))
         a.partial = ws.data_ptr()
-        self._launch(tag, "pcs_conv1_wgrad" if conv1 else "pcs_wgrad", ct.byref(a), L.stream_ptr())
+        name = "pcs_conv1_wgrad" if conv1 else "pcs_wgrad"
+        self._launch(tag, name if bw is None else name + "_partials", ct.byref(a), L.stream_ptr())
+        if bw is not None:
+            bw.defer_sum(ws, sv.B * a.splits_per_scene, cout, cin, dW, a.ldw)
         return ws
 
-    def _rounded(self, W):
-        if self.dt == L.F32:
-            return W
-        out = torch.empty_like(W)
-        _call("pcs_round_weight", W, W.numel(), self.dt, out, L.stream_ptr())
-        return out
+    @staticmethod
+    def _rounded(P, sv, conv):
+        return sv.wc[f"{conv}.rounded"] if sv.paths.bf16 else P[f"{conv}.weight"]
 
     def _gram(self, Y, s_, t_, B, N, C, tag=None):
         dev = Y.device
@@ -353,7 +390,7 @@
         live = {}
         if train and masks is None and not pt.draw_beside_gram:
             self._draw_masks(sv, seed)
-        sv.wc = self.cast_weights(P)
+        sv.wc = self.cast_weights(P, sv)
         self._trunk(P, bufs, sv)
         self._conv5(P, bufs, sv, live)
         self._global_feat(P, bufs, sv, live, seed)
@@ -468,8 +505,7 @@
     def _global_gram_stats(self, P, sv, live, seed):
         B, N, _, dev, s = self._dims(sv)
         pt, a5 = sv.paths, sv.ys["a5"]
-        Wg = P["global_feat.weight"].reshape(1024, -1)
-        sv.wg_eff = sv.wc["global_feat_fp8"][2] if pt.fp8 else self._rounded(Wg)
+        sv.wg_eff = sv.wc["global_feat_fp8"][2] if pt.fp8 else self._rounded(P, sv, "global_feat")
         G5 = _f32(dev, 1024, 1024)
         max_wg = 3 * torch.cuda.get_device_properties(dev).multi_processor_count
         gws = self._gram_raw(a5, G5, beside=(lambda: self._draw_masks(sv, seed, max_wg)) if pt.draw_beside_gram else None)
@@ -500,8 +536,10 @@
         if pt.fp8:
             Wf, kw = wc["global_feat_fp8"][0], dict(w_scale=wc["global_feat_fp8"][1], extra_flags=L.FLAG_AW_FP8)
         if st_g is None and pt.glds:
-            live["Wsg"] = Wsg = torch.empty_like(Wf)
-            _call("pcs_sign_rows", Wf, self.a5_dt, 1024, 1024, gamma_g, Wsg, s)
+            Wsg = wc.get("global_feat.signed")
+            if Wsg is None:
+                live["Wsg"] = Wsg = torch.empty_like(Wf)
+                _call("pcs_sign_rows", Wf, self.a5_dt, 1024, 1024, gamma_g, Wsg, s)
             Wf, kw["extra_flags"] = Wsg, kw["extra_flags"] | L.FLAG_POOL_SIGNED_W
         self._gemm(sv, 1024, 1024, L.PRO_RAW, L.EPI_FWD, a5, Wf, None, stats=st_g, pool=pool, es=gamma_g,
                    tag="fwd:global_feat", **kw)
@@ -561,7 +599,7 @@
         G2 = tot[:64 * 64]
         Sb = per_scene[:, 64 * 64:].contiguous()
         Ws1 = P["seg_conv1.weight"]
-        Ws1_r = self._rounded(Ws1)
+        Ws1_r = self._rounded(P, sv, "seg_conv1")
         st1 = _f32(dev, B, 512, 2)
         _call("pcs_bn_stats_gram_sbias", G2, Sb, B, N, Ws1_r, Ws1.shape[1], 64, 512, sbias, st1, s)
         sv.bn["bn_seg1"] = c1 = self._bn_finalize(P, bufs, sv, "bn_seg1", st1, 512, 1, N, soff)
@@ -613,12 +651,15 @@
         scene_s1 = self._bwd_seg32(P, sv, bw, hb)
         sp = self._bwd_pool(P, sv, bw, scene_s1)
         dA2 = self._bwd_seg1_local(P, sv, bw)
+        bw.flush_sums()
         bucket("seg")
         Wg_r, st5, cps5 = self._bwd_global_dgrad(P, sv, bw, sp)
         self._bwd_global_wgrad(P, sv, bw, sp, Wg_r)
+        bw.flush_sums()
         bucket("global")
         self._bwd_conv5(P, sv, bw, st5, cps5)
         self._bwd_trunk(P, sv, bw, dA2)
+        bw.flush_sums()
         bucket("tail")
         return hb
 
@@ -636,7 +677,7 @@
         pc = sv.bn[_LAYERS[prev][2]]
         bw.keep.append(self._wgrad(
             sv, _LAYERS[conv][1], cin or _LAYERS[conv][0], L.PRO_BWD, L.PRO_BNRELU, bw.G(f"{conv}.weight"), ldw=ldw,
-            tag=f"wgrad:{conv}", dZ=dz, Y=sv.ys[conv], alpha=al, beta=be, gamma=ga, X=sv.ys[prev], s=pc.scale,
+            tag=f"wgrad:{conv}", bw=bw, dZ=dz, Y=sv.ys[conv], alpha=al, beta=be, gamma=ga, X=sv.ys[prev], s=pc.scale,
             t=pc.shift, x_mask=x_mask, x_keep_scale=bw.keep_scale if x_mask is not None else 1.0))
 
     def _bwd_layer(self, P, sv, bw, conv, dz, prev, out, c_mask=None, addend=None, per_scene=False):
@@ -657,7 +698,8 @@
             st = _f32(dev, B * cps, cin, 2)
             ws = _f32(dev, nbytes // 4)
             a.stats = L.ptr(st)
-            self._launch(f"dgrad+wgrad:{conv}", "pcs_dgrad_wgrad_bn", ct.byref(a), ws, bw.G(f"{conv}.weight"), 0, s)
+            self._launch(f"dgrad+wgrad:{conv}", "pcs_dgrad_wgrad_bn_partials", ct.byref(a), ws, s)
+            bw.defer_sum(ws, B * cps, cout, cin, bw.G(f"{conv}.weight"))
             bw.keep.append(ws)
         else:
             cps, _ = self.geometry(B, N, cout, cin, L.PRO_BWD, L.EPI_DGRAD, flags=pt.flags)
@@ -672,8 +714,7 @@
     def _bwd_seg32(self, P, sv, bw, hb):
         _, _, M, dev, s = self._dims(sv)
         m1, m2 = sv.masks
-        _call("pcs_reduce_partials", hb["wpartial"], hb["nch"], self.C * 129, 1.0, bw.G("seg_conv4.weight"),
-              self.C * 129, self.C * 129, s)
+        bw.defer_sum(hb["wpartial"], hb["nch"], 1, self.C * 129, bw.G("seg_conv4.weight"))
         self._bn_bwd(P, sv, bw, "bn_seg3", "seg_conv3", hb["stats"], hb["cps"])
         bw.bufB = torch.empty(M * 1024, dtype=self.tdt, device=dev)
         self._bwd_layer(P, sv, bw, "seg_conv3", bw.bufA, "seg_conv2", bw.bufB, c_mask=m2)
@@ -708,7 +749,7 @@
             self._wgrad_bn(sv, bw, "seg_conv1", dz_s1, "conv2", cin=64, ldw=Ws1.shape[1])
             return dA2
         p2 = sv.bn["bn2"]
-        Ws1_r = self._rounded(Ws1)
+        Ws1_r = self._rounded(P, sv, "seg_conv1")
         WaT, Hs1 = self._empty(64, 512, device=dev), self._empty(64, 64, device=dev)
         _call("pcs_bn_fold", Ws1_r, 512, 64, Ws1.shape[1], a1, b1, g1, self.dt, WaT, None, Hs1, s)
         fa = self._wgrad_args(sv, 512, 64, L.PRO_RAW, L.PRO_BNRELU, bw.G("seg_conv1.weight"), ldw=Ws1.shape[1],
@@ -725,7 +766,7 @@
         pt, a5, dz5 = sv.paths, sv.ys["a5"], bw.bufB
         bg, gg = bw.coefs["bn_global"][1:]
         Wg_r = sv.wg_eff if sv.gram5 is not None else \
-            sv.wc["global_feat_fp8"][2] if pt.fp8 else self._rounded(P["global_feat.weight"])
+            sv.wc["global_feat_fp8"][2] if pt.fp8 else self._rounded(P, sv, "global_feat")
         cvec = _f32(dev, 1024)
         Hg = _f32(dev, 1024, 1024) if pt.fp8 else self._empty(1024, 1024, device=dev)
         _call("pcs_bn_fold", Wg_r, 1024, 1024, Wg_r.shape[1], None, bg, gg, L.F32 if pt.fp8 else self.dt, None, cvec, Hg, s)
@@ -756,8 +797,7 @@
         B, N, _, dev, s = self._dims(sv)
         a5 = sv.ys["a5"]
         _, bg, gg = bw.coefs["bn_global"]
-        ones = torch.ones(1024, dtype=torch.float32, device=dev)
-        zeros = torch.zeros(1024, dtype=torch.float32, device=dev)
+        ones, zeros = self._unit_coefs(dev)
         raw = sv.paths.wide_fast and sv.a5_colsum is not None
         gram = _f32(dev, 1024, 1024) if sv.gram5 is not None or raw else None
         if sv.gram5 is not None:
@@ -789,7 +829,7 @@
         _call("pcs_bn_s2_from_r", st5, B * cps5, 1024, r5, sv.wc["conv5"][0], self.dt, 128, 128, pc5.mean, pc5.rstd, s)
         self._bn_bwd(P, sv, bw, "bn5", "conv5", st5, cps5)
         al5, be5, ga5 = bw.coefs["bn5"]
-        W5_r = self._rounded(P["conv5.weight"])
+        W5_r = self._rounded(P, sv, "conv5")
         ws_t, c5, h4 = self._empty(128, 1024, device=dev), _f32(dev, 128), self._empty(128, 128, device=dev)
         _call("pcs_bn_fold", W5_r, 1024, 128, 128, al5, be5, ga5, self.dt, ws_t, c5, h4, s)
         cps4, _ = self.geometry(B, N, 1024 + 128, 128, L.PRO_CAT, L.EPI_DGRAD, flags=sv.paths.flags)
@@ -812,5 +852,5 @@
         self._bwd_layer(P, sv, bw, "conv2", bw.bufA, "conv1", bw.bufB)
         al, be, ga = bw.coefs["bn1"]
         bw.keep.append(self._wgrad(sv, 64, self.input_dim, L.PRO_BWD, L.PRO_RAW, bw.G("conv1.weight"),
-                                   ldw=self.input_dim, conv1=True, tag="wgrad:conv1", dZ=bw.bufB, Y=sv.ys["conv1"],
+                                   ldw=self.input_dim, conv1=True, tag="wgrad:conv1", bw=bw, dZ=bw.bufB, Y=sv.ys["conv1"],
                                    alpha=al, beta=be, gamma=ga, X=sv.x))
diff --git a/point-cloud-cnn-segmentation_amd/model.py b/point-cloud-cnn-segmentation_amd/model.py
--- a/point-cloud-cnn-segmentation_amd/model.py
+++ b/point-cloud-cnn-segmentation_amd/model.py
@@ -6,7 +6,7 @@
 import torch.nn as nn
 
 from . import _lib as L
-from .engine import BNS, FLAT_EXTRA, Engine, check_dims, flat_offsets, param_layout
+from .engine import FLAT_EXTRA, Engine, check_dims, flat_offsets, param_layout
 
 
 class _DropoutState:
@@ -37,8 +37,7 @@
         seed = module._next_seed() if train and masks is None else 0
         sv = eng.forward(P, bufs, x, train=train, masks=masks, seed=seed)
         if train:
-            for bn, _ in BNS:
-                getattr(module, bn).num_batches_tracked.add_(1)
+            eng.count_batches(bufs)
         ctx.sv = sv
         ctx.module = module
         return sv.logits
diff --git a/point-cloud-cnn-segmentation_amd/train.py b/point-cloud-cnn-segmentation_amd/train.py
--- a/point-cloud-cnn-segmentation_amd/train.py
+++ b/point-cloud-cnn-segmentation_amd/train.py
@@ -4,7 +4,6 @@
 import torch.distributed as dist
 
 from . import _lib as L
-from .engine import BNS
 from .optim import FusedAdam, flat_buffers
 
 
@@ -82,8 +81,7 @@
         sv = eng.forward(P, bufs, points, train=True, masks=masks, seed=seed,
                          head_mode=L.HEAD_CE, labels=labels, class_weight=self.class_weight,
                          wsum=None if ddp else self.wsum, want_logits=False)
-        for bn, _ in BNS:
-            getattr(model, bn).num_batches_tracked.add_(1)
+        eng.count_batches(bufs)
         hb = sv.head
         L.call("pcs_reduce_partials", L.ptr(hb["loss_partial"]), hb["nch"], 1, 1.0, L.ptr(ext), 1, 1, s)
         if ddp:
```

Measured after the change: 118.0 M points/s (median of 6 runs). No clear change (+0.3%).
